# mgaido91/FBK-fairseq-ST

Measured on AMD Instinct MI355X. Metric: audio-frames/sec (train fwd+bwd) s2t_transformer_m, 80-mel, higher is better.
Workload: dtype bf16

## Files before the change

### fbk_fairseq_st_amd/csrc/attention.hip

```cpp
#include "common.hpp"
#include "prof.hpp"
#include <cstdlib>
#include <type_traits>

template <typename T, int DH> struct ACfg {
    static constexpr int E = Elem<T>::PER16;
    static constexpr int ROWB = DH * (int)sizeof(T);
    static constexpr int NCH = ROWB / 16;
    static constexpr int KG = NCH / 4;
    static constexpr int PROWB = 64 * (int)sizeof(T);
    static constexpr int PCH = PROWB / 16;
    static constexpr int PKG = PCH / 4;
    static constexpr int ND = DH / 16;
    static constexpr int TILE = 64 * ROWB;
    static constexpr int TTILE = DH * PROWB;
    static constexpr int PTILE = 16 * PROWB;
};

__device__ __forceinline__ int swz(int row, int c, int nch) { return c ^ (row & ((nch < 8 ? nch : 8) - 1)); }

template <typename T, int DH>
__device__ __forceinline__ void stage_rows(char* lds, const T* g, long stride, int row0, int nvalid) {
    typedef ACfg<T, DH> C;
    for (int cid = threadIdx.x; cid < 64 * C::NCH; cid += 256) {
        const int row = cid / C::NCH, c = cid % C::NCH;
        u32x4 v = {0, 0, 0, 0};
        if (row0 + row < nvalid) v = *reinterpret_cast<const u32x4*>(g + (long)(row0 + row) * stride + c * C::E);
        *reinterpret_cast<u32x4*>(lds + row * C::ROWB + (swz(row, c, C::NCH) << 4)) = v;
    }
}

template <typename T, int DH>
__device__ __forceinline__ void stage_cols(char* lds, const T* g, long stride, int row0, int nvalid) {
    typedef ACfg<T, DH> C;
    if constexpr (sizeof(T) == 2) {
        for (int it = threadIdx.x; it < 32 * C::NCH; it += 256) {
            const int rp = it & 31, dc = it >> 5;
            u32x4 v0 = {0, 0, 0, 0}, v1 = {0, 0, 0, 0};
            const int r0 = row0 + 2 * rp;
            if (r0 < nvalid) v0 = *reinterpret_cast<const u32x4*>(g + (long)r0 * stride + dc * 8);
            if (r0 + 1 < nvalid) v1 = *reinterpret_cast<const u32x4*>(g + (long)(r0 + 1) * stride + dc * 8);
            const uint16_t* a = reinterpret_cast<const uint16_t*>(&v0);
            const uint16_t* b = reinterpret_cast<const uint16_t*>(&v1);
#pragma unroll
            for (int e = 0; e < 8; ++e) {
                const int d = dc * 8 + e;
                const uint32_t w = (uint32_t)a[e] | ((uint32_t)b[e] << 16);
                *reinterpret_cast<uint32_t*>(lds + d * C::PROWB + (swz(d, rp >> 2, C::PCH) << 4) + ((rp & 3) << 2)) = w;
            }
        }
    } else {
        for (int it = threadIdx.x; it < 64 * C::NCH; it += 256) {
            const int r = it & 63, dc = it >> 6;
            u32x4 v = {0, 0, 0, 0};
            if (row0 + r < nvalid) v = *reinterpret_cast<const u32x4*>(g + (long)(row0 + r) * stride + dc * 4);
#pragma unroll
            for (int e = 0; e < 4; ++e) {
                const int d = dc * 4 + e;
                *reinterpret_cast<uint32_t*>(lds + d * C::PROWB + (swz(d, r >> 2, C::PCH) << 4) + ((r & 3) << 2)) = v[e];
            }
        }
    }
}

__device__ __forceinline__ u32x4 frag(const char* lds, int row, int chunk, int rowb, int nch) {
    return *reinterpret_cast<const u32x4*>(lds + row * rowb + (swz(row, chunk, nch) << 4));
}

template <typename T>
__device__ __forceinline__ void put_tile(char* lds, const f32x4 (&acc)[4], int q, int r16) {
    constexpr int PROWB = 64 * (int)sizeof(T), PCH = PROWB / 16;
#pragma unroll
    for (int j = 0; j < 4; ++j)
#pragma unroll
        for (int r = 0; r < 4; ++r) {
            const int row = 4 * q + r, byte = (16 * j + r16) * (int)sizeof(T);
            *reinterpret_cast<T*>(lds + row * PROWB + (swz(row, byte >> 4, PCH) << 4) + (byte & 15)) = from_f32<T>(acc[j][r]);
        }
}

#define S2T_ATTN_V2_MIN_TQ g_s2t_opt_attn_v2_min_tq

struct AttnArgs {
    const void *Q, *K, *V; void* O; float* LSE;
    const void *dO; void *dQ, *dK, *dV; const float* Delta;
    long q_st, q_sb, k_st, k_sb, v_st, v_sb, o_st, o_sb;
    long dq_st, dq_sb, dk_st, dk_sb, dv_st, dv_sb, do_st, do_sb;
    const int* klen;
    int B, H, Tq, Tk, causal;
    int dist_pen;
    float scale, p_drop; unsigned long long seed;
};

__device__ __forceinline__ uint64_t drop_index(const AttnArgs& p, int b, int h, int qrow, int key) {
    return (((uint64_t)b * p.H + h) * p.Tq + qrow) * (uint64_t)((p.Tk + 3) & ~3) + key;
}
__device__ __forceinline__ float drop_scale(const AttnArgs& p, int b, int h, int qrow, int key) {
    if (p.p_drop <= 0.f) return 1.f;
    const uint32_t th = (uint32_t)fminf(p.p_drop * 4294967296.f, 4294967295.f);
    return dropout_keep(p.seed, drop_index(p, b, h, qrow, key), th) ? 1.f / (1.f - p.p_drop) : 0.f;
}

__device__ __forceinline__ uint32_t drop_pair(uint32_t pair, uint32_t fields, uint32_t thm1x2) {
    uint32_t d, k, r;
    asm("v_pk_sub_u16 %0, %1, %2 clamp" : "=v"(d) : "v"(fields), "v"(thm1x2));
    asm("v_pk_min_u16 %0, %1, %2" : "=v"(k) : "v"(d), "v"(0x00010001u));
    asm("v_pk_mul_lo_u16 %0, %1, %2" : "=v"(r) : "v"(pair), "v"(k));
    return r;
}

__device__ __forceinline__ float dist_pen_ln(int qrow, int key) {
    const int d = qrow > key ? qrow - key : key - qrow;
    return d > 1 ? __logf((float)d) : 0.f;
}
__device__ __forceinline__ float dist_pen_log2(int qrow, int key) {
    const int d = qrow > key ? qrow - key : key - qrow;
    return d > 1 ? __builtin_amdgcn_logf((float)d) : 0.f;
}

template <typename T, int DH>
__global__ __launch_bounds__(256) void attn_fwd_kernel(AttnArgs p) {
    typedef ACfg<T, DH> C;
    extern __shared__ __attribute__((aligned(16))) char smem[];
    char* ldsK = smem;
    char* ldsVt = smem + C::TILE;
    const int lane = threadIdx.x & 63, wave = threadIdx.x >> 6, r16 = lane & 15, q = lane >> 4;
    char* ldsP = smem + 2 * C::TILE + wave * C::PTILE;
    const int b = blockIdx.z, h = blockIdx.y, q0 = blockIdx.x * 64 + wave * 16;
    const int klen = p.klen ? min(p.klen[b], p.Tk) : p.Tk;
    const T* Qg = reinterpret_cast<const T*>(p.Q) + (long)b * p.q_sb + (long)h * DH;
    const T* Kg = reinterpret_cast<const T*>(p.K) + (long)b * p.k_sb + (long)h * DH;
    const T* Vg = reinterpret_cast<const T*>(p.V) + (long)b * p.v_sb + (long)h * DH;

    u32x4 qf[C::KG];
#pragma unroll
    for (int g = 0; g < C::KG; ++g) {
        qf[g] = (u32x4){0, 0, 0, 0};
        if (q0 + r16 < p.Tq) qf[g] = *reinterpret_cast<const u32x4*>(Qg + (long)(q0 + r16) * p.q_st + (4 * g + q) * C::E);
    }
    f32x4 o[C::ND];
#pragma unroll
    for (int n = 0; n < C::ND; ++n) o[n] = (f32x4){0.f, 0.f, 0.f, 0.f};
    float m[4] = {-INFINITY, -INFINITY, -INFINITY, -INFINITY}, l[4] = {0.f, 0.f, 0.f, 0.f};

    int kv_end = klen;
    if (p.causal) kv_end = min(kv_end, blockIdx.x * 64 + 64);
    for (int kv0 = 0; kv0 < kv_end; kv0 += 64) {
        __syncthreads();
        stage_rows<T, DH>(ldsK, Kg, p.k_st, kv0, klen);
        stage_cols<T, DH>(ldsVt, Vg, p.v_st, kv0, klen);
        __syncthreads();
        f32x4 s[4];
#pragma unroll
        for (int j = 0; j < 4; ++j) {
            s[j] = (f32x4){0.f, 0.f, 0.f, 0.f};
#pragma unroll
            for (int g = 0; g < C::KG; ++g)
                s[j] = mma16<T>(qf[g], frag(ldsK, 16 * j + r16, 4 * g + q, C::ROWB, C::NCH), s[j]);
        }
        float mx[4] = {-INFINITY, -INFINITY, -INFINITY, -INFINITY};
#pragma unroll
        for (int j = 0; j < 4; ++j) {
            const int key = kv0 + 16 * j + r16;
#pragma unroll
            for (int r = 0; r < 4; ++r) {
                const int qrow = q0 + 4 * q + r;
                const bool ok = key < klen && (!p.causal || key <= qrow);
                s[j][r] = ok ? s[j][r] * p.scale - (p.dist_pen ? dist_pen_ln(qrow, key) : 0.f) : -INFINITY;
                mx[r] = fmaxf(mx[r], s[j][r]);
            }
        }
        float alpha[4], rs[4];
#pragma unroll
        for (int r = 0; r < 4; ++r) {
            float v = mx[r];
            v = fmaxf(v, __shfl_xor(v, 1)); v = fmaxf(v, __shfl_xor(v, 2));
            v = fmaxf(v, __shfl_xor(v, 4)); v = fmaxf(v, __shfl_xor(v, 8));
            const float mn = fmaxf(m[r], v);
            const float mu = (mn == -INFINITY) ? 0.f : mn;
            alpha[r] = __expf(m[r] - mu);
            m[r] = mn;
            mx[r] = mu;
            rs[r] = 0.f;
        }
#pragma unroll
        for (int j = 0; j < 4; ++j)
#pragma unroll
            for (int r = 0; r < 4; ++r) {
                const float pv = __expf(s[j][r] - mx[r]);
                rs[r] += pv;
                s[j][r] = pv * drop_scale(p, b, h, q0 + 4 * q + r, kv0 + 16 * j + r16);
            }
#pragma unroll
        for (int r = 0; r < 4; ++r) {
            float v = rs[r];
            v += __shfl_xor(v, 1); v += __shfl_xor(v, 2); v += __shfl_xor(v, 4); v += __shfl_xor(v, 8);
            l[r] = l[r] * alpha[r] + v;
        }
#pragma unroll
        for (int n = 0; n < C::ND; ++n)
#pragma unroll
            for (int r = 0; r < 4; ++r) o[n][r] *= alpha[r];
        put_tile<T>(ldsP, s, q, r16);
        __builtin_amdgcn_s_waitcnt(0xC07F);
        __builtin_amdgcn_wave_barrier();
#pragma unroll
        for (int g = 0; g < C::PKG; ++g) {
            const u32x4 pa = frag(ldsP, r16, 4 * g + q, C::PROWB, C::PCH);
#pragma unroll
            for (int n = 0; n < C::ND; ++n)
                o[n] = mma16<T>(pa, frag(ldsVt, 16 * n + r16, 4 * g + q, C::PROWB, C::PCH), o[n]);
        }
    }
    T* Og = reinterpret_cast<T*>(p.O) + (long)b * p.o_sb + (long)h * DH;
#pragma unroll
    for (int r = 0; r < 4; ++r) {
        const int qrow = q0 + 4 * q + r;
        if (qrow >= p.Tq) continue;
        const float inv = l[r] > 0.f ? 1.f / l[r] : 0.f;
#pragma unroll
        for (int n = 0; n < C::ND; ++n) Og[(long)qrow * p.o_st + 16 * n + r16] = from_f32<T>(o[n][r] * inv);
        if (r16 == 0 && p.LSE) p.LSE[((long)b * p.H + h) * p.Tq + qrow] = m[r] + logf(l[r]);
    }
}

__device__ __forceinline__ int head_xcd_remap(int& head, int nheads, int ntile) {
    const int L = ((int)blockIdx.z * gridDim.y + blockIdx.y) * gridDim.x + blockIdx.x;
    if (nheads & 7) { head = (int)blockIdx.z * gridDim.y + blockIdx.y; return blockIdx.x; }
    const int slot = L >> 3;
    head = (L & 7) + 8 * (slot / ntile);
    return slot % ntile;
}
typedef short s16x4_t __attribute__((ext_vector_type(4)));
typedef __bf16 bf16x2_t __attribute__((ext_vector_type(2)));
typedef float f32x2_t __attribute__((ext_vector_type(2)));
__device__ __forceinline__ uint32_t pack_bf16(float lo, float hi) {
    return __builtin_bit_cast(uint32_t, __builtin_convertvector((f32x2_t){lo, hi}, bf16x2_t));
}
__device__ __forceinline__ float max_over_rows(float v) {
    uint32_t x = __builtin_bit_cast(uint32_t, v);
    auto r = __builtin_amdgcn_permlane16_swap(x, x, false, false);
    v = fmaxf(__builtin_bit_cast(float, (uint32_t)r[0]), __builtin_bit_cast(float, (uint32_t)r[1]));
    x = __builtin_bit_cast(uint32_t, v);
    r = __builtin_amdgcn_permlane32_swap(x, x, false, false);
    return fmaxf(__builtin_bit_cast(float, (uint32_t)r[0]), __builtin_bit_cast(float, (uint32_t)r[1]));
}
#ifdef S2T_ATTN_STAMPS
__device__ unsigned long long* g_attn_stamps = nullptr;
extern "C" int s2t_dbg_attn_stamps(void* buf) {
    return hipMemcpyToSymbol(HIP_SYMBOL(g_attn_stamps), &buf, sizeof(buf)) == hipSuccess ? 0 : -1;
}
#define ASTAMP_INIT(KID)                                                                                         \
    const int lin_ = ((int)blockIdx.z * gridDim.y + blockIdx.y) * gridDim.x + blockIdx.x;                        \
    const int slot_ = lin_ == 0 ? 0 : (lin_ == 700 ? 1 : (lin_ == 1100 ? 2 : (lin_ == 1500 ? 3 : -1)));                                                    \
    unsigned long long* const stp_ = (g_attn_stamps && slot_ >= 0) ? g_attn_stamps + (((KID) * 4 + slot_) * 4 + (threadIdx.x >> 6)) * 64 : nullptr;
#define ASTAMP(T, K)                                                                                             \
    if (stp_ && (T) < 8) {                                                                                       \
        unsigned long long t_;                                                                                   \
        asm volatile("s_memtime %0\n\ts_waitcnt lgkmcnt(0)" : "=s"(t_) :: "memory");                             \
        if ((threadIdx.x & 63) == 0) stp_[(T) * 8 + (K)] = t_;                                                   \
    }
#define ASTAMP_EARLY(KID)                  \
    ASTAMP_INIT(KID) ASTAMP(7, 0)
#else
#define ASTAMP_INIT(KID)
#define ASTAMP(T, K)
#define ASTAMP_EARLY(KID)
#endif
__global__ __launch_bounds__(256, 3) void attn_fwd2_kernel(AttnArgs p) {
    constexpr int DH = 64;
    ASTAMP_EARLY(0)
    extern __shared__ __attribute__((aligned(16))) char smem[];
    const int lane = threadIdx.x & 63, wave = threadIdx.x >> 6, r16 = lane & 15, q = lane >> 4;
    int head;
    const int bx = head_xcd_remap(head, p.B * p.H, gridDim.x);
    const int b = head / p.H, h = head % p.H, qw = bx * 128 + wave * 32;
    const int klen = p.klen ? min(p.klen[b], p.Tk) : p.Tk;
    const bf16* Qg = reinterpret_cast<const bf16*>(p.Q) + (long)b * p.q_sb + (long)h * DH;
    const bf16* Kg = reinterpret_cast<const bf16*>(p.K) + (long)b * p.k_sb + (long)h * DH;
    const bf16* Vg = reinterpret_cast<const bf16*>(p.V) + (long)b * p.v_sb + (long)h * DH;

    f32x4 o[2][4];
#pragma unroll
    for (int qb = 0; qb < 2; ++qb)
#pragma unroll
        for (int n = 0; n < 4; ++n) o[qb][n] = (f32x4){0.f, 0.f, 0.f, 0.f};
    float m[2] = {-INFINITY, -INFINITY}, l[2] = {0.f, 0.f};

    int kv_end = klen;
    if (p.causal) kv_end = min(kv_end, bx * 128 + 128);
    const int ntile = (kv_end + 63) / 64;

    const uint32_t kst2 = (uint32_t)p.k_st * 2u, vst2 = (uint32_t)p.v_st * 2u;
    auto stage = [&](int kv0, char* st) {
#pragma unroll
        for (int i = 0; i < 2; ++i) {
            const int r8 = 8 * (wave + 4 * i), row = r8 + (lane >> 3), pos = lane & 7;
            const uint32_t r = (uint32_t)min(kv0 + row, p.Tk - 1);
            char* dst = st + __builtin_amdgcn_readfirstlane(r8 * 128);
            const char* ka = reinterpret_cast<const char*>(Kg) + (__umul24(r, kst2) + (uint32_t)((pos ^ (row & 7)) << 4));
            const char* va = reinterpret_cast<const char*>(Vg) + (__umul24(r, vst2) + (uint32_t)((pos ^ (row & 6)) << 4));
            __builtin_amdgcn_global_load_lds((__attribute__((address_space(1))) const void*)ka, (__attribute__((address_space(3))) void*)dst, 16, 0, 0);
            __builtin_amdgcn_global_load_lds((__attribute__((address_space(1))) const void*)va, (__attribute__((address_space(3))) void*)(dst + 8192), 16, 0, 0);
        }
    };
    const uint32_t drop_th16 = (uint32_t)fminf(p.p_drop * 4294967296.f, 4294967295.f) >> 16;
    const uint32_t drop_thm1x2 = (drop_th16 - 1u) * 0x00010001u;
    const bool has_drop = drop_th16 > 0;
    const float drop_inv = 1.f / (1.f - p.p_drop);
    const uint32_t drop_ks = drop_seed_key(p.seed);
    const float sc2 = p.scale * 1.44269504088896f;
    const bool plain = !p.causal && !p.dist_pen && (uint64_t)p.B * p.H * p.Tq * (uint64_t)((p.Tk + 3) & ~3) < (1ull << 34);

    float* sInit = reinterpret_cast<float*>(smem + 32768);
    if (threadIdx.x < 128) {
        const int i = threadIdx.x & 63;
        sInit[threadIdx.x] = (threadIdx.x < 64 || (ntile - 1) * 64 + i < klen) ? 0.f : -INFINITY;
    }
    if (ntile > 0) stage(0, smem);
    char* sQ = smem + 32768 + 512;
#pragma unroll
    for (int i = 0; i < 4; ++i) {
        const int r8 = 8 * (wave + 4 * i), row = r8 + (lane >> 3), pos = lane & 7;
        const long r = min(bx * 128 + row, p.Tq - 1);
        char* dst = sQ + __builtin_amdgcn_readfirstlane(r8 * 128);
        __builtin_amdgcn_global_load_lds((__attribute__((address_space(1))) const void*)(Qg + r * p.q_st + ((pos ^ (row & 7)) << 3)),
                                         (__attribute__((address_space(3))) void*)dst, 16, 0, 0);
    }
    __builtin_amdgcn_s_waitcnt(0x0F70);
    __syncthreads();
    ASTAMP(7, 1)
    for (int t = 0; t < ntile; ++t) {
        const int kv0 = t * 64;
        const char* sK = smem + (t & 1) * 16384;
        const char* sV = sK + 8192;
        ASTAMP(t, 0)
        if (t + 1 < ntile) stage(kv0 + 64, smem + ((t + 1) & 1) * 16384);
        ASTAMP(t, 1)
        f32x4 s[2][4];
        const float* sInit0 = sInit + ((plain && t == ntile - 1) ? 64 : 0) + 4 * q;
        u32x4 qf[2][2];
#pragma unroll
        for (int qb = 0; qb < 2; ++qb)
#pragma unroll
            for (int g = 0; g < 2; ++g) {
                const int row = wave * 32 + 16 * qb + r16;
                qf[qb][g] = *reinterpret_cast<const u32x4*>(sQ + row * 128 + (((4 * g + q) ^ (row & 7)) << 4));
            }
#pragma unroll
        for (int j = 0; j < 4; ++j) {
            u32x4 kf[2];
#pragma unroll
            for (int g = 0; g < 2; ++g) {
                const int row = 16 * j + r16;
                kf[g] = *reinterpret_cast<const u32x4*>(sK + row * 128 + (((4 * g + q) ^ (row & 7)) << 4));
            }
#pragma unroll
            for (int qb = 0; qb < 2; ++qb) {
                s[qb][j] = *reinterpret_cast<const f32x4*>(sInit0 + 16 * j);
#pragma unroll
                for (int g = 0; g < 2; ++g) s[qb][j] = mma16<bf16>(kf[g], qf[qb][g], s[qb][j]);
            }
        }
        u32x4 pf[2][2];
        auto softmax_tile = [&](auto fast_tag, auto drop_tag) {
            constexpr bool FAST = decltype(fast_tag)::value, DROP = decltype(drop_tag)::value;
            const bool pen = !FAST && p.dist_pen;
            const float k2 = pen ? 1.f : sc2;
#pragma unroll
            for (int qb = 0; qb < 2; ++qb) {
                const int qrow = qw + 16 * qb + r16;
                float mx = -INFINITY;
#pragma unroll
                for (int j = 0; j < 4; ++j) {
                    if constexpr (!FAST) {
#pragma unroll
                        for (int r = 0; r < 4; ++r) {
                            float v = s[qb][j][r];
                            const int key = kv0 + 16 * j + 4 * q + r;
                            if (pen) v = v * sc2 - dist_pen_log2(qrow, key);
                            v = (key < klen && (!p.causal || key <= qrow)) ? v : -INFINITY;
                            s[qb][j][r] = v;
                        }
                    }
                    mx = fmaxf(fmaxf(mx, s[qb][j][0]), s[qb][j][1]);
                    mx = fmaxf(fmaxf(mx, s[qb][j][2]), s[qb][j][3]);
                }
                mx = max_over_rows(mx);
                const float mn = fmaxf(m[qb], mx * k2);
                const float mu = (mn == -INFINITY) ? 0.f : mn;
                const float alpha = __builtin_amdgcn_exp2f(m[qb] - mu);
                m[qb] = mn;
                f32x2_t rs2 = {0.f, 0.f};
                const bool drop = FAST ? DROP : has_drop;
                const uint64_t quad0 = drop ? drop_index(p, b, h, qrow, kv0 + 4 * q) >> 2 : 0;
                const uint32_t qlo = (uint32_t)quad0, hwm0 = drop_high_mix(p.seed, quad0);
#pragma unroll
                for (int j = 0; j < 4; ++j) {
                    float pv[4];
#pragma unroll
                    for (int r = 0; r < 4; ++r) pv[r] = __builtin_amdgcn_exp2f(__builtin_fmaf(s[qb][j][r], k2, -mu));
                    rs2 += (f32x2_t){pv[0], pv[1]};
                    rs2 += (f32x2_t){pv[2], pv[3]};
                    uint32_t p01 = pack_bf16(pv[0], pv[1]), p23 = pack_bf16(pv[2], pv[3]);
                    if (drop) {
                        const u32x2 hq = FAST ? drop_hash4_lo(drop_ks, hwm0, qlo + 4u * j) : drop_hash4(p.seed, quad0 + 4 * j);
                        p01 = drop_pair(p01, hq[1], drop_thm1x2); p23 = drop_pair(p23, hq[0], drop_thm1x2);
                    }
                    pf[qb][j >> 1][2 * (j & 1)] = p01;
                    pf[qb][j >> 1][2 * (j & 1) + 1] = p23;
                }
                l[qb] = l[qb] * alpha + (rs2[0] + rs2[1]);
#pragma unroll
                for (int n = 0; n < 4; ++n) o[qb][n] *= alpha;
            }
        };
        if (!plain) softmax_tile(std::false_type{}, std::false_type{});
        else if (has_drop) softmax_tile(std::true_type{}, std::true_type{});
        else softmax_tile(std::true_type{}, std::false_type{});
        ASTAMP(t, 2)
#pragma unroll
        for (int kb = 0; kb < 2; ++kb)
#pragma unroll
            for (int n = 0; n < 4; ++n) {
                u32x4 vf;
#pragma unroll
                for (int hh = 0; hh < 2; ++hh) {
                    const int row = 32 * kb + 16 * hh + 4 * q + (r16 >> 2);
                    const int ch = 2 * n + ((r16 & 3) >> 1);
                    const char* a = sV + row * 128 + ((ch ^ (row & 6)) << 4) + ((r16 & 1) << 3);
                    const s16x4_t v = __builtin_amdgcn_ds_read_tr16_b64_v4i16((__attribute__((address_space(3))) s16x4_t*)a);
                    const u32x2 w = __builtin_bit_cast(u32x2, v);
                    vf[2 * hh] = w[0]; vf[2 * hh + 1] = w[1];
                }
#pragma unroll
                for (int qb = 0; qb < 2; ++qb) o[qb][n] = mma16<bf16>(vf, pf[qb][kb], o[qb][n]);
            }
        ASTAMP(t, 3)
        __builtin_amdgcn_s_waitcnt(0x0F70);
        ASTAMP(t, 4)
        __syncthreads();
        ASTAMP(t, 5)
    }
    ASTAMP(7, 2)
    bf16* Og = reinterpret_cast<bf16*>(p.O) + (long)b * p.o_sb + (long)h * DH;
#pragma unroll
    for (int qb = 0; qb < 2; ++qb) {
        const int qrow = qw + 16 * qb + r16;
        float lt = l[qb];
        lt += __shfl_xor(lt, 16); lt += __shfl_xor(lt, 32);
        if (qrow >= p.Tq) continue;
        const float inv = lt > 0.f ? drop_inv / lt : 0.f;
#pragma unroll
        for (int n = 0; n < 4; ++n) {
            u32x2 w;
            w[0] = pack_bf16(o[qb][n][0] * inv, o[qb][n][1] * inv);
            w[1] = pack_bf16(o[qb][n][2] * inv, o[qb][n][3] * inv);
            *reinterpret_cast<u32x2*>(Og + (long)qrow * p.o_st + 16 * n + 4 * q) = w;
        }
        if (q == 0 && p.LSE) p.LSE[((long)b * p.H + h) * p.Tq + qrow] = m[qb] * 0.693147180559945f + logf(lt);
    }
    ASTAMP(7, 3)
}

template <typename T, int DH>
__global__ __launch_bounds__(256) void attn_delta_kernel(AttnArgs p) {
    const int g = (blockIdx.x * 256 + threadIdx.x) >> 4, li = threadIdx.x & 15;
    const long total = (long)p.B * p.H * p.Tq;
    float s = 0.f;
    if (g < total) {
        const int t = g % p.Tq, h = (g / p.Tq) % p.H, b = g / (p.Tq * p.H);
        const T* o = reinterpret_cast<const T*>(p.O) + (long)t * p.o_st + (long)b * p.o_sb + (long)h * DH;
        const T* d = reinterpret_cast<const T*>(p.dO) + (long)t * p.do_st + (long)b * p.do_sb + (long)h * DH;
        for (int j = li; j < DH; j += 16) s += to_f32(o[j]) * to_f32(d[j]);
    }
    s += __shfl_xor(s, 1); s += __shfl_xor(s, 2); s += __shfl_xor(s, 4); s += __shfl_xor(s, 8);
    if (g < total && li == 0) {
        const int t = g % p.Tq, h = (g / p.Tq) % p.H, b = g / (p.Tq * p.H);
        const_cast<float*>(p.Delta)[((long)b * p.H + h) * p.Tq + t] = s;
    }
}

template <typename T, int DH>
__global__ __launch_bounds__(256) void attn_bwd_dkv_kernel(AttnArgs p) {
    typedef ACfg<T, DH> C;
    extern __shared__ __attribute__((aligned(16))) char smem[];
    char* ldsQ = smem;
    char* ldsDO = smem + C::TILE;
    char* ldsQt = smem + 2 * C::TILE;
    char* ldsDOt = smem + 3 * C::TILE;
    const int lane = threadIdx.x & 63, wave = threadIdx.x >> 6, r16 = lane & 15, q = lane >> 4;
    char* ldsP = smem + 4 * C::TILE + wave * 2 * C::PTILE;
    char* ldsS = ldsP + C::PTILE;
    const int b = blockIdx.z, h = blockIdx.y, k0 = blockIdx.x * 64 + wave * 16;
    const int klen = p.klen ? min(p.klen[b], p.Tk) : p.Tk;
    const T* Qg = reinterpret_cast<const T*>(p.Q) + (long)b * p.q_sb + (long)h * DH;
    const T* Kg = reinterpret_cast<const T*>(p.K) + (long)b * p.k_sb + (long)h * DH;
    const T* Vg = reinterpret_cast<const T*>(p.V) + (long)b * p.v_sb + (long)h * DH;
    const T* dOg = reinterpret_cast<const T*>(p.dO) + (long)b * p.do_sb + (long)h * DH;
    const float* lse = p.LSE + ((long)b * p.H + h) * p.Tq;
    const float* dlt = p.Delta + ((long)b * p.H + h) * p.Tq;

    u32x4 kf[C::KG], vf[C::KG];
#pragma unroll
    for (int g = 0; g < C::KG; ++g) {
        kf[g] = vf[g] = (u32x4){0, 0, 0, 0};
        if (k0 + r16 < klen) {
            kf[g] = *reinterpret_cast<const u32x4*>(Kg + (long)(k0 + r16) * p.k_st + (4 * g + q) * C::E);
            vf[g] = *reinterpret_cast<const u32x4*>(Vg + (long)(k0 + r16) * p.v_st + (4 * g + q) * C::E);
        }
    }
    f32x4 dk[C::ND], dv[C::ND];
#pragma unroll
    for (int n = 0; n < C::ND; ++n) { dk[n] = (f32x4){0.f, 0.f, 0.f, 0.f}; dv[n] = dk[n]; }

    const int qstart = p.causal ? (blockIdx.x * 64) : 0;
    for (int qt = qstart; qt < p.Tq; qt += 64) {
        __syncthreads();
        stage_rows<T, DH>(ldsQ, Qg, p.q_st, qt, p.Tq);
        stage_rows<T, DH>(ldsDO, dOg, p.do_st, qt, p.Tq);
        stage_cols<T, DH>(ldsQt, Qg, p.q_st, qt, p.Tq);
        stage_cols<T, DH>(ldsDOt, dOg, p.do_st, qt, p.Tq);
        __syncthreads();
        f32x4 st[4], dp[4];
#pragma unroll
        for (int j = 0; j < 4; ++j) {
            st[j] = (f32x4){0.f, 0.f, 0.f, 0.f}; dp[j] = st[j];
#pragma unroll
            for (int g = 0; g < C::KG; ++g) {
                st[j] = mma16<T>(kf[g], frag(ldsQ, 16 * j + r16, 4 * g + q, C::ROWB, C::NCH), st[j]);
                dp[j] = mma16<T>(vf[g], frag(ldsDO, 16 * j + r16, 4 * g + q, C::ROWB, C::NCH), dp[j]);
            }
        }
#pragma unroll
        for (int j = 0; j < 4; ++j) {
            const int qrow = qt + 16 * j + r16;
            const bool qok = qrow < p.Tq;
            const float L = qok ? lse[qrow] : 0.f, Dl = qok ? dlt[qrow] : 0.f;
#pragma unroll
            for (int r = 0; r < 4; ++r) {
                const int key = k0 + 4 * q + r;
                const bool ok = qok && key < klen && (!p.causal || key <= qrow);
                const float pv = ok ? __expf(st[j][r] * p.scale - (p.dist_pen ? dist_pen_ln(qrow, key) : 0.f) - L) : 0.f;
                const float ds = ok ? drop_scale(p, b, h, qrow, key) : 0.f;
                st[j][r] = pv * ds;
                dp[j][r] = pv * (ds * dp[j][r] - Dl) * p.scale;
            }
        }
        put_tile<T>(ldsP, st, q, r16);
        put_tile<T>(ldsS, dp, q, r16);
        __builtin_amdgcn_s_waitcnt(0xC07F);
        __builtin_amdgcn_wave_barrier();
#pragma unroll
        for (int g = 0; g < C::PKG; ++g) {
            const u32x4 pa = frag(ldsP, r16, 4 * g + q, C::PROWB, C::PCH);
            const u32x4 sa = frag(ldsS, r16, 4 * g + q, C::PROWB, C::PCH);
#pragma unroll
            for (int n = 0; n < C::ND; ++n) {
                dv[n] = mma16<T>(pa, frag(ldsDOt, 16 * n + r16, 4 * g + q, C::PROWB, C::PCH), dv[n]);
                dk[n] = mma16<T>(sa, frag(ldsQt, 16 * n + r16, 4 * g + q, C::PROWB, C::PCH), dk[n]);
            }
        }
    }
    T* dKg = reinterpret_cast<T*>(p.dK) + (long)b * p.dk_sb + (long)h * DH;
    T* dVg = reinterpret_cast<T*>(p.dV) + (long)b * p.dv_sb + (long)h * DH;
#pragma unroll
    for (int r = 0; r < 4; ++r) {
        const int key = k0 + 4 * q + r;
        if (key >= p.Tk) continue;
#pragma unroll
        for (int n = 0; n < C::ND; ++n) {
            dKg[(long)key * p.dk_st + 16 * n + r16] = from_f32<T>(dk[n][r]);
            dVg[(long)key * p.dv_st + 16 * n + r16] = from_f32<T>(dv[n][r]);
        }
    }
}

template <typename T, int DH>
__global__ __launch_bounds__(256) void attn_bwd_dq_kernel(AttnArgs p) {
    typedef ACfg<T, DH> C;
    extern __shared__ __attribute__((aligned(16))) char smem[];
    char* ldsK = smem;
    char* ldsV = smem + C::TILE;
    char* ldsKt = smem + 2 * C::TILE;
    const int lane = threadIdx.x & 63, wave = threadIdx.x >> 6, r16 = lane & 15, q = lane >> 4;
    char* ldsS = smem + 3 * C::TILE + wave * C::PTILE;
    const int b = blockIdx.z, h = blockIdx.y, q0 = blockIdx.x * 64 + wave * 16;
    const int klen = p.klen ? min(p.klen[b], p.Tk) : p.Tk;
    const T* Qg = reinterpret_cast<const T*>(p.Q) + (long)b * p.q_sb + (long)h * DH;
    const T* Kg = reinterpret_cast<const T*>(p.K) + (long)b * p.k_sb + (long)h * DH;
    const T* Vg = reinterpret_cast<const T*>(p.V) + (long)b * p.v_sb + (long)h * DH;
    const T* dOg = reinterpret_cast<const T*>(p.dO) + (long)b * p.do_sb + (long)h * DH;
    const float* lse = p.LSE + ((long)b * p.H + h) * p.Tq;
    const float* dlt = p.Delta + ((long)b * p.H + h) * p.Tq;

    u32x4 qf[C::KG], dof[C::KG];
#pragma unroll
    for (int g = 0; g < C::KG; ++g) {
        qf[g] = dof[g] = (u32x4){0, 0, 0, 0};
        if (q0 + r16 < p.Tq) {
            qf[g] = *reinterpret_cast<const u32x4*>(Qg + (long)(q0 + r16) * p.q_st + (4 * g + q) * C::E);
            dof[g] = *reinterpret_cast<const u32x4*>(dOg + (long)(q0 + r16) * p.do_st + (4 * g + q) * C::E);
        }
    }
    float L[4], Dl[4];
#pragma unroll
    for (int r = 0; r < 4; ++r) {
        const int qrow = q0 + 4 * q + r;
        L[r] = qrow < p.Tq ? lse[qrow] : 0.f;
        Dl[r] = qrow < p.Tq ? dlt[qrow] : 0.f;
    }
    f32x4 dq[C::ND];
#pragma unroll
    for (int n = 0; n < C::ND; ++n) dq[n] = (f32x4){0.f, 0.f, 0.f, 0.f};

    int kv_end = klen;
    if (p.causal) kv_end = min(kv_end, blockIdx.x * 64 + 64);
    for (int kv0 = 0; kv0 < kv_end; kv0 += 64) {
        __syncthreads();
        stage_rows<T, DH>(ldsK, Kg, p.k_st, kv0, klen);
        stage_rows<T, DH>(ldsV, Vg, p.v_st, kv0, klen);
        stage_cols<T, DH>(ldsKt, Kg, p.k_st, kv0, klen);
        __syncthreads();
        f32x4 s[4], dp[4];
#pragma unroll
        for (int j = 0; j < 4; ++j) {
            s[j] = (f32x4){0.f, 0.f, 0.f, 0.f}; dp[j] = s[j];
#pragma unroll
            for (int g = 0; g < C::KG; ++g) {
                s[j] = mma16<T>(qf[g], frag(ldsK, 16 * j + r16, 4 * g + q, C::ROWB, C::NCH), s[j]);
                dp[j] = mma16<T>(dof[g], frag(ldsV, 16 * j + r16, 4 * g + q, C::ROWB, C::NCH), dp[j]);
            }
        }
#pragma unroll
        for (int j = 0; j < 4; ++j) {
            const int key = kv0 + 16 * j + r16;
#pragma unroll
            for (int r = 0; r < 4; ++r) {
                const int qrow = q0 + 4 * q + r;
                const bool ok = qrow < p.Tq && key < klen && (!p.causal || key <= qrow);
                const float pv = ok ? __expf(s[j][r] * p.scale - (p.dist_pen ? dist_pen_ln(qrow, key) : 0.f) - L[r]) : 0.f;
                const float ds = ok ? drop_scale(p, b, h, qrow, key) : 0.f;
                dp[j][r] = pv * (ds * dp[j][r] - Dl[r]) * p.scale;
            }
        }
        put_tile<T>(ldsS, dp, q, r16);
        __builtin_amdgcn_s_waitcnt(0xC07F);
        __builtin_amdgcn_wave_barrier();
#pragma unroll
        for (int g = 0; g < C::PKG; ++g) {
            const u32x4 sa = frag(ldsS, r16, 4 * g + q, C::PROWB, C::PCH);
#pragma unroll
            for (int n = 0; n < C::ND; ++n)
                dq[n] = mma16<T>(sa, frag(ldsKt, 16 * n + r16, 4 * g + q, C::PROWB, C::PCH), dq[n]);
        }
    }
    T* dQg = reinterpret_cast<T*>(p.dQ) + (long)b * p.dq_sb + (long)h * DH;
#pragma unroll
    for (int r = 0; r < 4; ++r) {
        const int qrow = q0 + 4 * q + r;
        if (qrow >= p.Tq) continue;
#pragma unroll
        for (int n = 0; n < C::ND; ++n) dQg[(long)qrow * p.dq_st + 16 * n + r16] = from_f32<T>(dq[n][r]);
    }
}

__device__ __forceinline__ u32x4 row_frag128(const char* tile, int row, int chunk) {
    return *reinterpret_cast<const u32x4*>(tile + row * 128 + ((chunk ^ (row & 7)) << 4));
}
__device__ __forceinline__ u32x4 tr_frag128(const char* tile, int blk, int n, int r16, int q) {
    u32x4 f;
#pragma unroll
    for (int hh = 0; hh < 2; ++hh) {
        const int row = 32 * blk + 16 * hh + 4 * q + (r16 >> 2);
        const int ch = 2 * n + ((r16 & 3) >> 1);
        const char* a = tile + row * 128 + ((ch ^ (row & 7)) << 4) + ((r16 & 1) << 3);
        const s16x4_t v = __builtin_amdgcn_ds_read_tr16_b64_v4i16((__attribute__((address_space(3))) s16x4_t*)a);
        const u32x2 w = __builtin_bit_cast(u32x2, v);
        f[2 * hh] = w[0]; f[2 * hh + 1] = w[1];
    }
    return f;
}
__device__ __forceinline__ uint32_t quad_bcast(uint32_t v, int r) {
    switch (r) {
        case 0: return (uint32_t)__builtin_amdgcn_mov_dpp((int)v, 0x00, 0xf, 0xf, true);
        case 1: return (uint32_t)__builtin_amdgcn_mov_dpp((int)v, 0x55, 0xf, 0xf, true);
        case 2: return (uint32_t)__builtin_amdgcn_mov_dpp((int)v, 0xAA, 0xf, 0xf, true);
        default: return (uint32_t)__builtin_amdgcn_mov_dpp((int)v, 0xFF, 0xf, 0xf, true);
    }
}
__device__ __forceinline__ void stage2_dma(const bf16* A, long a_st, const bf16* B, long b_st, int r0, int nrows, char* st, int wave, int lane) {
#pragma unroll
    for (int i = 0; i < 2; ++i) {
        const int r8 = 8 * (wave + 4 * i), row = r8 + (lane >> 3), pos = lane & 7;
        const uint32_t r = (uint32_t)min(r0 + row, nrows - 1);
        const uint32_t ch = (uint32_t)((pos ^ (row & 7)) << 4);
        char* dst = st + __builtin_amdgcn_readfirstlane(r8 * 128);
        const char* aa = reinterpret_cast<const char*>(A) + (__umul24(r, (uint32_t)a_st * 2u) + ch);
        const char* ba = reinterpret_cast<const char*>(B) + (__umul24(r, (uint32_t)b_st * 2u) + ch);
        __builtin_amdgcn_global_load_lds((__attribute__((address_space(1))) const void*)aa, (__attribute__((address_space(3))) void*)dst, 16, 0, 0);
        __builtin_amdgcn_global_load_lds((__attribute__((address_space(1))) const void*)ba, (__attribute__((address_space(3))) void*)(dst + 8192), 16, 0, 0);
    }
}
#define S2T_WAIT_VM0() __builtin_amdgcn_s_waitcnt(0x0F70)

__global__ __launch_bounds__(256, 2) void attn_bwd_dkv2_kernel(AttnArgs p) {
    constexpr int DH = 64;
    ASTAMP_EARLY(2)
    extern __shared__ __attribute__((aligned(16))) char smem[];
    const int lane = threadIdx.x & 63, wave = __builtin_amdgcn_readfirstlane(threadIdx.x >> 6), r16 = lane & 15, q = lane >> 4;
    int head;
    const int bx = head_xcd_remap(head, p.B * p.H, gridDim.x);
    const int b = head / p.H, h = head % p.H, kw = bx * 128 + wave * 32;
    const int klen = p.klen ? min(p.klen[b], p.Tk) : p.Tk;
    const bf16* Qg = reinterpret_cast<const bf16*>(p.Q) + (long)b * p.q_sb + (long)h * DH;
    const bf16* Kg = reinterpret_cast<const bf16*>(p.K) + (long)b * p.k_sb + (long)h * DH;
    const bf16* Vg = reinterpret_cast<const bf16*>(p.V) + (long)b * p.v_sb + (long)h * DH;
    const bf16* dOg = reinterpret_cast<const bf16*>(p.dO) + (long)b * p.do_sb + (long)h * DH;
    const float* lse = p.LSE + ((long)b * p.H + h) * p.Tq;
    const float* dlt = p.Delta + ((long)b * p.H + h) * p.Tq;

    char* sKown = smem + 32768 + 1024;
    char* sVown = sKown + 16384;
    f32x4 dkT[2][4], dvT[2][4];
#pragma unroll
    for (int kb = 0; kb < 2; ++kb)
#pragma unroll
        for (int n = 0; n < 4; ++n) { dkT[kb][n] = (f32x4){0.f, 0.f, 0.f, 0.f}; dvT[kb][n] = dkT[kb][n]; }
    const uint32_t drop_th16 = (uint32_t)fminf(p.p_drop * 4294967296.f, 4294967295.f) >> 16;
    const float drop_inv = 1.f / (1.f - p.p_drop);
    const uint32_t drop_ks = drop_seed_key(p.seed), drop_hwm = drop_high_mix(p.seed, 0);
    const uint32_t tkq = (uint32_t)((p.Tk + 3) >> 2);
    const uint32_t drop_thm1x2 = (drop_th16 - 1u) * 0x00010001u;
    const uint32_t own_bit = ((r16 & 1) ? 0x00010000u : 1u) << ((r16 >> 1) & 1);

    const int qstart = p.causal ? bx * 128 : 0;
    const int ntile = qstart < p.Tq ? (p.Tq - qstart + 63) / 64 : 0;
    float* sStat = reinterpret_cast<float*>(smem + 32768);
    auto stage = [&](int qt, int stg) {
        stage2_dma(Qg, p.q_st, dOg, p.do_st, qt, p.Tq, smem + stg * 16384, wave, lane);
        if (wave < 2) {
            float* dst = sStat + stg * 128 + wave * 64;
            if (wave == 1 || qt + lane < p.Tq) {
                const char* sb = reinterpret_cast<const char*>(wave == 0 ? lse : dlt);
                const char* src = sb + (uint32_t)(min(qt + lane, p.Tq - 1) * 4);
                __builtin_amdgcn_global_load_lds((__attribute__((address_space(1))) const void*)src,
                                                 (__attribute__((address_space(3))) void*)dst, 4, 0, 0);
            } else dst[lane] = INFINITY;
        }
    };
    if (ntile > 0) stage(qstart, 0);
    {
        u32x4 kk[4], vv[4];
#pragma unroll
        for (int i = 0; i < 4; ++i) {
            const int cid = threadIdx.x + 256 * i, row = cid >> 3, c = cid & 7;
            const long key = min(bx * 128 + row, p.Tk - 1);
            kk[i] = *reinterpret_cast<const u32x4*>(Kg + key * p.k_st + c * 8);
            vv[i] = *reinterpret_cast<const u32x4*>(Vg + key * p.v_st + c * 8);
        }
#pragma unroll
        for (int i = 0; i < 4; ++i) {
            const int cid = threadIdx.x + 256 * i, row = cid >> 3, c = cid & 7;
            const bool in = bx * 128 + row < klen;
#pragma unroll
            for (int w = 0; w < 4; ++w) { kk[i][w] = in ? kk[i][w] : 0u; vv[i][w] = in ? vv[i][w] : 0u; }
            *reinterpret_cast<u32x4*>(sKown + row * 128 + ((c ^ (row & 7)) << 4)) = kk[i];
            *reinterpret_cast<u32x4*>(sVown + row * 128 + ((c ^ (row & 7)) << 4)) = vv[i];
        }
    }
    S2T_WAIT_VM0();
    __syncthreads();
    const float sc2 = p.scale * 1.44269504088896f;
    const bool generic = p.causal || p.dist_pen;
    ASTAMP(7, 1)
    for (int t = 0; t < ntile; ++t) {
        const int qt = qstart + t * 64;
        const char* sQ = smem + (t & 1) * 16384;
        const char* sDO = sQ + 8192;
        const float* sL = sStat + (t & 1) * 128;
        ASTAMP(t, 0)
        if (t + 1 < ntile) stage(qt + 64, (t + 1) & 1);
        ASTAMP(t, 1)
        auto tile = [&](auto edge_tag, auto drop_tag) {
        constexpr bool EDGE = decltype(edge_tag)::value, DROP = decltype(drop_tag)::value;
#pragma unroll 1
        for (int ib = 0; ib < 2; ++ib) {
        u32x4 pf[2], sf[2];
#pragma unroll
        for (int ii = 0; ii < 2; ++ii) {
            const int i = 2 * ib + ii;
            u32x4 qa[2], da[2];
#pragma unroll
            for (int g = 0; g < 2; ++g) { qa[g] = row_frag128(sQ, 16 * i + r16, 4 * g + q); da[g] = row_frag128(sDO, 16 * i + r16, 4 * g + q); }
            const f32x4 L = *reinterpret_cast<const f32x4*>(sL + 16 * i + 4 * q) * 1.44269504088896f;
            const f32x4 Dl = *reinterpret_cast<const f32x4*>(sL + 64 + 16 * i + 4 * q);
            const uint32_t qrow_quads = DROP ? (uint32_t)(((b * p.H + h) * p.Tq + qt + 16 * i + 4 * q + (r16 & 3))) * tkq : 0u;
#pragma unroll
            for (int kb = 0; kb < 2; ++kb) {
                f32x4 st = {0.f, 0.f, 0.f, 0.f}, dp = {0.f, 0.f, 0.f, 0.f};
#pragma unroll
                for (int g = 0; g < 2; ++g) {
                    const int krow = wave * 32 + 16 * kb + r16;
                    st = mma16<bf16>(qa[g], row_frag128(sKown, krow, 4 * g + q), st);
                    dp = mma16<bf16>(da[g], row_frag128(sVown, krow, 4 * g + q), dp);
                }
                const int key = kw + 16 * kb + r16;
                uint32_t nib = 0u;
                if constexpr (DROP) {
                    const u32x2 hq = drop_hash4_lo(drop_ks, drop_hwm, qrow_quads + ((uint32_t)key >> 2));
                    uint32_t dy, dx, ky, kx;
                    asm("v_pk_sub_u16 %0, %1, %2 clamp" : "=v"(dy) : "v"(hq[1]), "v"(drop_thm1x2));
                    asm("v_pk_sub_u16 %0, %1, %2 clamp" : "=v"(dx) : "v"(hq[0]), "v"(drop_thm1x2));
                    asm("v_pk_min_u16 %0, %1, %2" : "=v"(ky) : "v"(dy), "v"(0x00010001u));
                    asm("v_pk_min_u16 %0, %1, %2" : "=v"(kx) : "v"(dx), "v"(0x00010001u));
                    nib = drop_th16 > 0 ? (ky | (kx << 1)) : 0x00030003u;
                }
                float pv[4], ds[4];
#pragma unroll
                for (int r = 0; r < 4; ++r) {
                    const int qrow = qt + 16 * i + 4 * q + r;
                    float arg = __builtin_fmaf(st[r], sc2, -L[r]);
                    if constexpr (EDGE) { if (p.dist_pen) arg -= dist_pen_log2(qrow, key); }
                    float e = __builtin_amdgcn_exp2f(arg);
                    if constexpr (EDGE) e = (qrow < p.Tq && (!p.causal || key <= qrow)) ? e : 0.f;
                    if constexpr (DROP) {
                        const bool keep = (quad_bcast(nib, r) & own_bit) != 0u;
                        pv[r] = keep ? e : 0.f;
                        ds[r] = e * __builtin_fmaf(keep ? dp[r] : 0.f, drop_inv, -Dl[r]);
                    } else {
                        pv[r] = e;
                        ds[r] = e * (dp[r] - Dl[r]);
                    }
                }
                pf[kb][2 * ii] = pack_bf16(pv[0], pv[1]); pf[kb][2 * ii + 1] = pack_bf16(pv[2], pv[3]);
                sf[kb][2 * ii] = pack_bf16(ds[0], ds[1]); sf[kb][2 * ii + 1] = pack_bf16(ds[2], ds[3]);
            }
        }
#pragma unroll
            for (int n = 0; n < 4; ++n) {
                const u32x4 dot = tr_frag128(sDO, ib, n, r16, q), qtf = tr_frag128(sQ, ib, n, r16, q);
#pragma unroll
                for (int kb = 0; kb < 2; ++kb) {
                    dvT[kb][n] = mma16<bf16>(dot, pf[kb], dvT[kb][n]);
                    dkT[kb][n] = mma16<bf16>(qtf, sf[kb], dkT[kb][n]);
                }
            }
        }
        };
        const bool edge = generic;
        if (p.p_drop > 0.f) { if (edge) tile(std::true_type{}, std::true_type{}); else tile(std::false_type{}, std::true_type{}); }
        else if (edge) tile(std::true_type{}, std::false_type{});
        else tile(std::false_type{}, std::false_type{});
        ASTAMP(t, 3)
        S2T_WAIT_VM0();
        ASTAMP(t, 4)
        __syncthreads();
        ASTAMP(t, 5)
    }
    ASTAMP(7, 2)
    const float dv_scale = p.p_drop > 0.f ? drop_inv : 1.f;
    bf16* dKg = reinterpret_cast<bf16*>(p.dK) + (long)b * p.dk_sb + (long)h * DH;
    bf16* dVg = reinterpret_cast<bf16*>(p.dV) + (long)b * p.dv_sb + (long)h * DH;
#pragma unroll
    for (int kb = 0; kb < 2; ++kb) {
        const int key = kw + 16 * kb + r16;
        if (key >= p.Tk) continue;
        const float kz = key < klen ? 1.f : 0.f;
#pragma unroll
        for (int n = 0; n < 4; ++n) { dkT[kb][n] *= kz * p.scale; dvT[kb][n] *= kz * dv_scale; }
#pragma unroll
        for (int n = 0; n < 4; ++n) {
            u32x2 w;
            w[0] = pack_bf16(dkT[kb][n][0], dkT[kb][n][1]); w[1] = pack_bf16(dkT[kb][n][2], dkT[kb][n][3]);
            *reinterpret_cast<u32x2*>(dKg + (long)key * p.dk_st + 16 * n + 4 * q) = w;
            w[0] = pack_bf16(dvT[kb][n][0], dvT[kb][n][1]); w[1] = pack_bf16(dvT[kb][n][2], dvT[kb][n][3]);
            *reinterpret_cast<u32x2*>(dVg + (long)key * p.dv_st + 16 * n + 4 * q) = w;
        }
    }
    ASTAMP(7, 3)
}

__global__ __launch_bounds__(256, 2) void attn_bwd_dq2_kernel(AttnArgs p) {
    constexpr int DH = 64;
    ASTAMP_EARLY(1)
    extern __shared__ __attribute__((aligned(16))) char smem[];
    const int lane = threadIdx.x & 63, wave = threadIdx.x >> 6, r16 = lane & 15, q = lane >> 4;
    int head;
    const int bx = head_xcd_remap(head, p.B * p.H, gridDim.x);
    const int b = head / p.H, h = head % p.H, qw = bx * 128 + wave * 32;
    const int klen = p.klen ? min(p.klen[b], p.Tk) : p.Tk;
    const bf16* Qg = reinterpret_cast<const bf16*>(p.Q) + (long)b * p.q_sb + (long)h * DH;
    const bf16* Kg = reinterpret_cast<const bf16*>(p.K) + (long)b * p.k_sb + (long)h * DH;
    const bf16* Vg = reinterpret_cast<const bf16*>(p.V) + (long)b * p.v_sb + (long)h * DH;
    const bf16* dOg = reinterpret_cast<const bf16*>(p.dO) + (long)b * p.do_sb + (long)h * DH;
    const float* lse = p.LSE + ((long)b * p.H + h) * p.Tq;
    const float* dlt = p.Delta + ((long)b * p.H + h) * p.Tq;

    int kv_end = klen;
    if (p.causal) kv_end = min(kv_end, bx * 128 + 128);
    const int ntile = (kv_end + 63) / 64;
    if (ntile > 0) stage2_dma(Kg, p.k_st, Vg, p.v_st, 0, p.Tk, smem, wave, lane);
    u32x4 qf[2][2], dof[2][2];
    float L[2], Dl[2];
    const bf16* Og = reinterpret_cast<const bf16*>(p.O) + (long)b * p.o_sb + (long)h * DH;
    u32x4 of[2][2];
#pragma unroll
    for (int qb = 0; qb < 2; ++qb) {
        const long row = min(qw + 16 * qb + r16, p.Tq - 1);
        L[qb] = lse[row] * 1.44269504088896f;
#pragma unroll
        for (int g = 0; g < 2; ++g) {
            qf[qb][g] = *reinterpret_cast<const u32x4*>(Qg + row * p.q_st + (4 * g + q) * 8);
            dof[qb][g] = *reinterpret_cast<const u32x4*>(dOg + row * p.do_st + (4 * g + q) * 8);
            of[qb][g] = *reinterpret_cast<const u32x4*>(Og + row * p.o_st + (4 * g + q) * 8);
        }
    }
#pragma unroll
    for (int qb = 0; qb < 2; ++qb) {
        const int row = qw + 16 * qb + r16;
        const bool in = row < p.Tq;
        float part = 0.f;
#pragma unroll
        for (int g = 0; g < 2; ++g) {
#pragma unroll
            for (int w = 0; w < 4; ++w) { qf[qb][g][w] = in ? qf[qb][g][w] : 0u; dof[qb][g][w] = in ? dof[qb][g][w] : 0u; }
            const bf16* oe = reinterpret_cast<const bf16*>(&of[qb][g]);
            const bf16* de = reinterpret_cast<const bf16*>(&dof[qb][g]);
#pragma unroll
            for (int e = 0; e < 8; ++e) part += (float)oe[e] * (float)de[e];
        }
        L[qb] = in ? L[qb] : 0.f;
        part += __shfl_xor(part, 16); part += __shfl_xor(part, 32);
        Dl[qb] = part;
        if (q == 0 && in) const_cast<float*>(dlt)[row] = part;
    }
    f32x4 dqT[2][4];
#pragma unroll
    for (int qb = 0; qb < 2; ++qb)
#pragma unroll
        for (int n = 0; n < 4; ++n) dqT[qb][n] = (f32x4){0.f, 0.f, 0.f, 0.f};
    const uint32_t drop_th16 = (uint32_t)fminf(p.p_drop * 4294967296.f, 4294967295.f) >> 16;
    const float drop_inv = 1.f / (1.f - p.p_drop);
    const uint32_t drop_ks = drop_seed_key(p.seed), drop_hwm = drop_high_mix(p.seed, 0);
    const uint32_t tkq = (uint32_t)((p.Tk + 3) >> 2);

    const float sc2 = p.scale * 1.44269504088896f;
    const bool generic = p.causal || p.dist_pen;
    S2T_WAIT_VM0();
    __syncthreads();
    ASTAMP(7, 1)
    for (int t = 0; t < ntile; ++t) {
        const int kv0 = t * 64;
        const char* sK = smem + (t & 1) * 16384;
        const char* sV = sK + 8192;
        ASTAMP(t, 0)
        if (t + 1 < ntile) stage2_dma(Kg, p.k_st, Vg, p.v_st, kv0 + 64, p.Tk, smem + ((t + 1) & 1) * 16384, wave, lane);
        ASTAMP(t, 1)
        u32x4 sf[2][2];
        auto ds_tile = [&](auto edge_tag, auto drop_tag, auto tail_tag) {
        constexpr bool EDGE = decltype(edge_tag)::value, DROP = decltype(drop_tag)::value, TAIL = decltype(tail_tag)::value;
        const int tail_thr = klen - kv0 - 4 * q;
#pragma unroll
        for (int j = 0; j < 4; ++j) {
            u32x4 ka[2], va[2];
#pragma unroll
            for (int g = 0; g < 2; ++g) { ka[g] = row_frag128(sK, 16 * j + r16, 4 * g + q); va[g] = row_frag128(sV, 16 * j + r16, 4 * g + q); }
#pragma unroll
            for (int qb = 0; qb < 2; ++qb) {
                f32x4 st = {0.f, 0.f, 0.f, 0.f}, dp = {0.f, 0.f, 0.f, 0.f};
#pragma unroll
                for (int g = 0; g < 2; ++g) { st = mma16<bf16>(ka[g], qf[qb][g], st); dp = mma16<bf16>(va[g], dof[qb][g], dp); }
                const int qrow = qw + 16 * qb + r16;
                const int key0 = kv0 + 16 * j + 4 * q;
                u32x2 hq = {0u, 0u};
                if constexpr (DROP) hq = drop_hash4_lo(drop_ks, drop_hwm, (uint32_t)((b * p.H + h) * p.Tq + qrow) * tkq + ((uint32_t)key0 >> 2));
                float ds[4];
#pragma unroll
                for (int r = 0; r < 4; ++r) {
                    float arg = __builtin_fmaf(st[r], sc2, -L[qb]);
                    if constexpr (EDGE) { if (p.dist_pen) arg -= dist_pen_log2(qrow, key0 + r); }
                    float e = __builtin_amdgcn_exp2f(arg);
                    if constexpr (EDGE) {
                        const int key = key0 + r;
                        e = (key < klen && (!p.causal || key <= qrow)) ? e : 0.f;
                    }
                    if constexpr (TAIL) e = (16 * j + r < tail_thr) ? e : 0.f;
                    if constexpr (DROP) ds[r] = e * __builtin_fmaf(drop_field(hq, r) >= drop_th16 ? dp[r] : 0.f, drop_inv, -Dl[qb]);
                    else ds[r] = e * (dp[r] - Dl[qb]);
                }
                sf[qb][j >> 1][2 * (j & 1)] = pack_bf16(ds[0], ds[1]); sf[qb][j >> 1][2 * (j & 1) + 1] = pack_bf16(ds[2], ds[3]);
            }
        }
        };
        const bool tail = kv0 + 64 > klen;
        if (generic) { if (p.p_drop > 0.f) ds_tile(std::true_type{}, std::true_type{}, std::false_type{}); else ds_tile(std::true_type{}, std::false_type{}, std::false_type{}); }
        else if (p.p_drop > 0.f) { if (tail) ds_tile(std::false_type{}, std::true_type{}, std::true_type{}); else ds_tile(std::false_type{}, std::true_type{}, std::false_type{}); }
        else if (tail) ds_tile(std::false_type{}, std::false_type{}, std::true_type{});
        else ds_tile(std::false_type{}, std::false_type{}, std::false_type{});
        ASTAMP(t, 2)
#pragma unroll
        for (int jb = 0; jb < 2; ++jb)
#pragma unroll
            for (int n = 0; n < 4; ++n) {
                const u32x4 kt = tr_frag128(sK, jb, n, r16, q);
#pragma unroll
                for (int qb = 0; qb < 2; ++qb) dqT[qb][n] = mma16<bf16>(kt, sf[qb][jb], dqT[qb][n]);
            }
        ASTAMP(t, 3)
        S2T_WAIT_VM0();
        ASTAMP(t, 4)
        __syncthreads();
        ASTAMP(t, 5)
    }
    ASTAMP(7, 2)
    bf16* dQg = reinterpret_cast<bf16*>(p.dQ) + (long)b * p.dq_sb + (long)h * DH;
#pragma unroll
    for (int qb = 0; qb < 2; ++qb) {
        const int qrow = qw + 16 * qb + r16;
        if (qrow >= p.Tq) continue;
#pragma unroll
        for (int n = 0; n < 4; ++n) {
            u32x2 w;
            w[0] = pack_bf16(dqT[qb][n][0] * p.scale, dqT[qb][n][1] * p.scale); w[1] = pack_bf16(dqT[qb][n][2] * p.scale, dqT[qb][n][3] * p.scale);
            *reinterpret_cast<u32x2*>(dQg + (long)qrow * p.dq_st + 16 * n + 4 * q) = w;
        }
    }
    ASTAMP(7, 3)
}

__global__ __launch_bounds__(256, 2) void attn_fwd_sq_kernel(AttnArgs p) {
    constexpr int DH = 64;
    extern __shared__ __attribute__((aligned(16))) char smem[];
    const int lane = threadIdx.x & 63, wave = __builtin_amdgcn_readfirstlane(threadIdx.x >> 6), r16 = lane & 15, q = lane >> 4;
    const int head = blockIdx.x, b = head / p.H, h = head % p.H, qw = wave * 16;
    const bool active = qw < p.Tq;
    const int klen = p.klen ? min(p.klen[b], p.Tk) : p.Tk;
    const bf16* Qg = reinterpret_cast<const bf16*>(p.Q) + (long)b * p.q_sb + (long)h * DH;
    const bf16* Kg = reinterpret_cast<const bf16*>(p.K) + (long)b * p.k_sb + (long)h * DH;
    const bf16* Vg = reinterpret_cast<const bf16*>(p.V) + (long)b * p.v_sb + (long)h * DH;

    f32x4 o[4];
#pragma unroll
    for (int n = 0; n < 4; ++n) o[n] = (f32x4){0.f, 0.f, 0.f, 0.f};
    float m = -INFINITY, l = 0.f;
    int kv_end = klen;
    if (p.causal) kv_end = min(kv_end, p.Tq);
    const int ntile = kv_end > 0 ? (kv_end + 63) / 64 : 0;

    const uint32_t kst2 = (uint32_t)p.k_st * 2u, vst2 = (uint32_t)p.v_st * 2u;
    auto stage = [&](int kv0, char* st) {
#pragma unroll
        for (int i = 0; i < 2; ++i) {
            const int r8 = 8 * (wave + 4 * i), row = r8 + (lane >> 3), pos = lane & 7;
            const uint32_t r = (uint32_t)min(kv0 + row, p.Tk - 1);
            char* dst = st + r8 * 128;
            const char* ka = reinterpret_cast<const char*>(Kg) + (__umul24(r, kst2) + (uint32_t)((pos ^ (row & 7)) << 4));
            const char* va = reinterpret_cast<const char*>(Vg) + (__umul24(r, vst2) + (uint32_t)((pos ^ (row & 6)) << 4));
            __builtin_amdgcn_global_load_lds((__attribute__((address_space(1))) const void*)ka, (__attribute__((address_space(3))) void*)dst, 16, 0, 0);
            __builtin_amdgcn_global_load_lds((__attribute__((address_space(1))) const void*)va, (__attribute__((address_space(3))) void*)(dst + 8192), 16, 0, 0);
        }
    };
    const uint32_t drop_th16 = (uint32_t)fminf(p.p_drop * 4294967296.f, 4294967295.f) >> 16;
    const uint32_t drop_thm1x2 = (drop_th16 - 1u) * 0x00010001u;
    const bool has_drop = drop_th16 > 0;
    const float drop_inv = 1.f / (1.f - p.p_drop);
    const uint32_t drop_ks = drop_seed_key(p.seed), drop_hwm = drop_high_mix(p.seed, 0);
    const uint32_t tkq = (uint32_t)((p.Tk + 3) >> 2);
    const float sc2 = p.scale * 1.44269504088896f;

    float* sInit = reinterpret_cast<float*>(smem + 32768);
    if (threadIdx.x < 128) {
        const int i = threadIdx.x & 63;
        sInit[threadIdx.x] = (threadIdx.x < 64 || (ntile - 1) * 64 + i < klen) ? 0.f : -INFINITY;
    }
    if (ntile > 0) stage(0, smem);
    char* sQ = smem + 32768 + 512;
#pragma unroll
    for (int i = 0; i < 2; ++i) {
        const int r8 = 8 * (wave + 4 * i), row = r8 + (lane >> 3), pos = lane & 7;
        const long r = min(row, p.Tq - 1);
        __builtin_amdgcn_global_load_lds((__attribute__((address_space(1))) const void*)(Qg + r * p.q_st + ((pos ^ (row & 7)) << 3)),
                                         (__attribute__((address_space(3))) void*)(sQ + r8 * 128), 16, 0, 0);
    }
    S2T_WAIT_VM0();
    __syncthreads();
    const int qrow = qw + r16;
    const uint32_t qrow_quads = (uint32_t)((b * p.H + h) * p.Tq + qrow) * tkq;
    for (int t = 0; t < ntile; ++t) {
        const int kv0 = t * 64;
        const char* sK = smem + (t & 1) * 16384;
        const char* sV = sK + 8192;
        if (t + 1 < ntile) stage(kv0 + 64, smem + ((t + 1) & 1) * 16384);
        if (active) {
            f32x4 s[4];
            const float* sInit0 = sInit + ((!p.causal && t == ntile - 1) ? 64 : 0) + 4 * q;
            u32x4 qf[2];
#pragma unroll
            for (int g = 0; g < 2; ++g) qf[g] = row_frag128(sQ, qw + r16, 4 * g + q);
#pragma unroll
            for (int j = 0; j < 4; ++j) {
                s[j] = *reinterpret_cast<const f32x4*>(sInit0 + 16 * j);
#pragma unroll
                for (int g = 0; g < 2; ++g) s[j] = mma16<bf16>(row_frag128(sK, 16 * j + r16, 4 * g + q), qf[g], s[j]);
            }
            u32x4 pf[2];
            auto softmax_tile = [&](auto mask_tag, auto drop_tag) {
                constexpr bool MASK = decltype(mask_tag)::value, DROP = decltype(drop_tag)::value;
                float mx = -INFINITY;
#pragma unroll
                for (int j = 0; j < 4; ++j) {
                    if constexpr (MASK) {
#pragma unroll
                        for (int r = 0; r < 4; ++r) {
                            const int key = kv0 + 16 * j + 4 * q + r;
                            s[j][r] = (key < klen && key <= qrow) ? s[j][r] : -INFINITY;
                        }
                    }
                    mx = fmaxf(fmaxf(mx, s[j][0]), s[j][1]);
                    mx = fmaxf(fmaxf(mx, s[j][2]), s[j][3]);
                }
                mx = max_over_rows(mx);
                const float mn = fmaxf(m, mx * sc2);
                const float mu = (mn == -INFINITY) ? 0.f : mn;
                const float alpha = __builtin_amdgcn_exp2f(m - mu);
                m = mn;
                f32x2_t rs2 = {0.f, 0.f};
                const uint32_t qlo = qrow_quads + (uint32_t)((kv0 + 4 * q) >> 2);
#pragma unroll
                for (int j = 0; j < 4; ++j) {
                    float pv[4];
#pragma unroll
                    for (int r = 0; r < 4; ++r) pv[r] = __builtin_amdgcn_exp2f(__builtin_fmaf(s[j][r], sc2, -mu));
                    rs2 += (f32x2_t){pv[0], pv[1]};
                    rs2 += (f32x2_t){pv[2], pv[3]};
                    uint32_t p01 = pack_bf16(pv[0], pv[1]), p23 = pack_bf16(pv[2], pv[3]);
                    if constexpr (DROP) {
                        const u32x2 hq = drop_hash4_lo(drop_ks, drop_hwm, qlo + 4u * j);
                        p01 = drop_pair(p01, hq[1], drop_thm1x2); p23 = drop_pair(p23, hq[0], drop_thm1x2);
                    }
                    pf[j >> 1][2 * (j & 1)] = p01;
                    pf[j >> 1][2 * (j & 1) + 1] = p23;
                }
                l = l * alpha + (rs2[0] + rs2[1]);
#pragma unroll
                for (int n = 0; n < 4; ++n) o[n] *= alpha;
            };
            if (p.causal) { if (has_drop) softmax_tile(std::true_type{}, std::true_type{}); else softmax_tile(std::true_type{}, std::false_type{}); }
            else if (has_drop) softmax_tile(std::false_type{}, std::true_type{});
            else softmax_tile(std::false_type{}, std::false_type{});
#pragma unroll
            for (int kb = 0; kb < 2; ++kb)
#pragma unroll
                for (int n = 0; n < 4; ++n) {
                    u32x4 vf;
#pragma unroll
                    for (int hh = 0; hh < 2; ++hh) {
                        const int row = 32 * kb + 16 * hh + 4 * q + (r16 >> 2);
                        const int ch = 2 * n + ((r16 & 3) >> 1);
                        const char* a = sV + row * 128 + ((ch ^ (row & 6)) << 4) + ((r16 & 1) << 3);
                        const s16x4_t v = __builtin_amdgcn_ds_read_tr16_b64_v4i16((__attribute__((address_space(3))) s16x4_t*)a);
                        const u32x2 w = __builtin_bit_cast(u32x2, v);
                        vf[2 * hh] = w[0]; vf[2 * hh + 1] = w[1];
                    }
                    o[n] = mma16<bf16>(vf, pf[kb], o[n]);
                }
        }
        S2T_WAIT_VM0();
        __syncthreads();
    }
    float lt = l;
    lt += __shfl_xor(lt, 16); lt += __shfl_xor(lt, 32);
    if (qrow >= p.Tq) return;
    bf16* Og = reinterpret_cast<bf16*>(p.O) + (long)b * p.o_sb + (long)h * DH;
    const float inv = lt > 0.f ? drop_inv / lt : 0.f;
#pragma unroll
    for (int n = 0; n < 4; ++n) {
        u32x2 w;
        w[0] = pack_bf16(o[n][0] * inv, o[n][1] * inv);
        w[1] = pack_bf16(o[n][2] * inv, o[n][3] * inv);
        *reinterpret_cast<u32x2*>(Og + (long)qrow * p.o_st + 16 * n + 4 * q) = w;
    }
    if (q == 0 && p.LSE) p.LSE[((long)b * p.H + h) * p.Tq + qrow] = m * 0.693147180559945f + logf(lt);
}

#define S2T_SQ_TPITCH 136
#define S2T_SQ_BWD_LDS (16384 + 512 + 32768 + 4 * 16 * S2T_SQ_TPITCH)
__global__ __launch_bounds__(256, 2) void attn_bwd_sq_kernel(AttnArgs p) {
    constexpr int DH = 64;
    extern __shared__ __attribute__((aligned(16))) char smem[];
    const int lane = threadIdx.x & 63, wave = __builtin_amdgcn_readfirstlane(threadIdx.x >> 6), r16 = lane & 15, q = lane >> 4;
    const int head = blockIdx.x, b = head / p.H, h = head % p.H;
    const int klen = p.klen ? min(p.klen[b], p.Tk) : p.Tk;
    const bf16* Qg = reinterpret_cast<const bf16*>(p.Q) + (long)b * p.q_sb + (long)h * DH;
    const bf16* Kg = reinterpret_cast<const bf16*>(p.K) + (long)b * p.k_sb + (long)h * DH;
    const bf16* Vg = reinterpret_cast<const bf16*>(p.V) + (long)b * p.v_sb + (long)h * DH;
    const bf16* dOg = reinterpret_cast<const bf16*>(p.dO) + (long)b * p.do_sb + (long)h * DH;
    const bf16* Og = reinterpret_cast<const bf16*>(p.O) + (long)b * p.o_sb + (long)h * DH;
    bf16* dKg = reinterpret_cast<bf16*>(p.dK) + (long)b * p.dk_sb + (long)h * DH;
    bf16* dVg = reinterpret_cast<bf16*>(p.dV) + (long)b * p.dv_sb + (long)h * DH;
    const float* lse = p.LSE + ((long)b * p.H + h) * p.Tq;
    float* dlt = const_cast<float*>(p.Delta) + ((long)b * p.H + h) * p.Tq;
    const char* sQ = smem;
    const char* sDO = smem + 8192;
    float* sStat = reinterpret_cast<float*>(smem + 16384);
    char* sKV = smem + 16384 + 512;
    char* sT = sKV + 32768 + wave * (16 * S2T_SQ_TPITCH);

    int kv_end = klen;
    if (p.causal) kv_end = min(kv_end, p.Tq);
    const int ntile = kv_end > 0 ? (kv_end + 63) / 64 : 0;
    const int nq = (p.Tq + 15) >> 4;
    if (ntile > 0) stage2_dma(Kg, p.k_st, Vg, p.v_st, 0, p.Tk, sKV, wave, lane);
    stage2_dma(Qg, p.q_st, dOg, p.do_st, 0, p.Tq, smem, wave, lane);
    {
        const int row = threadIdx.x >> 2, seg = threadIdx.x & 3;
        const long rc = min(row, p.Tq - 1);
        u32x4 of[2], df[2];
#pragma unroll
        for (int g = 0; g < 2; ++g) {
            of[g] = *reinterpret_cast<const u32x4*>(Og + rc * p.o_st + 16 * seg + 8 * g);
            df[g] = *reinterpret_cast<const u32x4*>(dOg + rc * p.do_st + 16 * seg + 8 * g);
        }
        const float L = lse[rc];
        float part = 0.f;
#pragma unroll
        for (int g = 0; g < 2; ++g) {
            const bf16* oe = reinterpret_cast<const bf16*>(&of[g]);
            const bf16* de = reinterpret_cast<const bf16*>(&df[g]);
#pragma unroll
            for (int e = 0; e < 8; ++e) part += (float)oe[e] * (float)de[e];
        }
        part += __shfl_xor(part, 1); part += __shfl_xor(part, 2);
        if (seg == 0) {
            const bool in = row < p.Tq;
            sStat[row] = in ? L * 1.44269504088896f : INFINITY;
            sStat[64 + row] = in ? part : 0.f;
            if (in) dlt[row] = part;
        }
    }
    f32x4 dq[4][4];
#pragma unroll
    for (int i = 0; i < 4; ++i)
#pragma unroll
        for (int n = 0; n < 4; ++n) dq[i][n] = (f32x4){0.f, 0.f, 0.f, 0.f};
    const uint32_t drop_th16 = (uint32_t)fminf(p.p_drop * 4294967296.f, 4294967295.f) >> 16;
    const float drop_inv = 1.f / (1.f - p.p_drop);
    const uint32_t drop_ks = drop_seed_key(p.seed), drop_hwm = drop_high_mix(p.seed, 0);
    const uint32_t tkq = (uint32_t)((p.Tk + 3) >> 2);
    const uint32_t drop_thm1x2 = (drop_th16 - 1u) * 0x00010001u;
    const uint32_t own_bit = ((r16 & 1) ? 0x00010000u : 1u) << ((r16 >> 1) & 1);
    const float sc2 = p.scale * 1.44269504088896f;
    const float dv_scale = p.p_drop > 0.f ? drop_inv : 1.f;
    S2T_WAIT_VM0();
    __syncthreads();
    for (int t = 0; t < ntile; ++t) {
        const int kv0 = t * 64;
        const char* sK = sKV + (t & 1) * 16384;
        const char* sV = sK + 8192;
        if (t + 1 < ntile) stage2_dma(Kg, p.k_st, Vg, p.v_st, kv0 + 64, p.Tk, sKV + ((t + 1) & 1) * 16384, wave, lane);
        const int key = kv0 + 16 * wave + r16;
        f32x4 dkT[4], dvT[4];
#pragma unroll
        for (int n = 0; n < 4; ++n) { dkT[n] = (f32x4){0.f, 0.f, 0.f, 0.f}; dvT[n] = dkT[n]; }
        auto tile = [&](auto mask_tag, auto drop_tag) {
            constexpr bool MASK = decltype(mask_tag)::value, DROP = decltype(drop_tag)::value;
            u32x4 kfr[2], vfr[2];
#pragma unroll
            for (int g = 0; g < 2; ++g) { kfr[g] = row_frag128(sK, 16 * wave + r16, 4 * g + q); vfr[g] = row_frag128(sV, 16 * wave + r16, 4 * g + q); }
#pragma unroll
            for (int ib = 0; ib < 2; ++ib) {
                if (2 * ib >= nq) break;
                u32x4 pf = {0u, 0u, 0u, 0u}, sf = {0u, 0u, 0u, 0u};
#pragma unroll
                for (int ii = 0; ii < 2; ++ii) {
                    const int i = 2 * ib + ii;
                    if (i >= nq) break;
                    u32x4 qa[2], da[2];
#pragma unroll
                    for (int g = 0; g < 2; ++g) { qa[g] = row_frag128(sQ, 16 * i + r16, 4 * g + q); da[g] = row_frag128(sDO, 16 * i + r16, 4 * g + q); }
                    const f32x4 L = *reinterpret_cast<const f32x4*>(sStat + 16 * i + 4 * q);
                    const f32x4 Dl = *reinterpret_cast<const f32x4*>(sStat + 64 + 16 * i + 4 * q);
                    f32x4 st = {0.f, 0.f, 0.f, 0.f}, dp = {0.f, 0.f, 0.f, 0.f};
#pragma unroll
                    for (int g = 0; g < 2; ++g) { st = mma16<bf16>(qa[g], kfr[g], st); dp = mma16<bf16>(da[g], vfr[g], dp); }
                    uint32_t nib = 0u;
                    if constexpr (DROP) {
                        const uint32_t qrow_quads = (uint32_t)((b * p.H + h) * p.Tq + 16 * i + 4 * q + (r16 & 3)) * tkq;
                        const u32x2 hq = drop_hash4_lo(drop_ks, drop_hwm, qrow_quads + ((uint32_t)key >> 2));
                        uint32_t dy, dx, ky, kx;
                        asm("v_pk_sub_u16 %0, %1, %2 clamp" : "=v"(dy) : "v"(hq[1]), "v"(drop_thm1x2));
                        asm("v_pk_sub_u16 %0, %1, %2 clamp" : "=v"(dx) : "v"(hq[0]), "v"(drop_thm1x2));
                        asm("v_pk_min_u16 %0, %1, %2" : "=v"(ky) : "v"(dy), "v"(0x00010001u));
                        asm("v_pk_min_u16 %0, %1, %2" : "=v"(kx) : "v"(dx), "v"(0x00010001u));
                        nib = drop_th16 > 0 ? (ky | (kx << 1)) : 0x00030003u;
                    }
                    float pv[4], ds[4];
#pragma unroll
                    for (int r = 0; r < 4; ++r) {
                        float e = __builtin_amdgcn_exp2f(__builtin_fmaf(st[r], sc2, -L[r]));
                        if constexpr (MASK) e = (key < klen && (!p.causal || key <= 16 * i + 4 * q + r)) ? e : 0.f;
                        if constexpr (DROP) {
                            const bool keep = (quad_bcast(nib, r) & own_bit) != 0u;
                            pv[r] = keep ? e : 0.f;
                            ds[r] = e * __builtin_fmaf(keep ? dp[r] : 0.f, drop_inv, -Dl[r]);
                        } else {
                            pv[r] = e;
                            ds[r] = e * (dp[r] - Dl[r]);
                        }
                    }
                    pf[2 * ii] = pack_bf16(pv[0], pv[1]); pf[2 * ii + 1] = pack_bf16(pv[2], pv[3]);
                    sf[2 * ii] = pack_bf16(ds[0], ds[1]); sf[2 * ii + 1] = pack_bf16(ds[2], ds[3]);
                    *reinterpret_cast<u32x2*>(sT + r16 * S2T_SQ_TPITCH + (16 * i + 4 * q) * 2) = (u32x2){sf[2 * ii], sf[2 * ii + 1]};
                }
#pragma unroll
                for (int n = 0; n < 4; ++n) {
                    const u32x4 dot = tr_frag128(sDO, ib, n, r16, q), qtf = tr_frag128(sQ, ib, n, r16, q);
                    dvT[n] = mma16<bf16>(dot, pf, dvT[n]);
                    dkT[n] = mma16<bf16>(qtf, sf, dkT[n]);
                }
            }
            asm volatile("s_waitcnt lgkmcnt(0)" ::: "memory");
            __builtin_amdgcn_wave_barrier();
            s16x4_t kt[4];
#pragma unroll
            for (int n = 0; n < 4; ++n) {
                const int row = 16 * wave + 4 * q + (r16 >> 2), ch = 2 * n + ((r16 & 3) >> 1);
                kt[n] = __builtin_amdgcn_ds_read_tr16_b64_v4i16((__attribute__((address_space(3))) s16x4_t*)(sK + row * 128 + ((ch ^ (row & 7)) << 4) + ((r16 & 1) << 3)));
            }
#pragma unroll
            for (int i = 0; i < 4; ++i) {
                if (i >= nq) break;
                const s16x4_t a = __builtin_amdgcn_ds_read_tr16_b64_v4i16(
                    (__attribute__((address_space(3))) s16x4_t*)(sT + (4 * q + (r16 >> 2)) * S2T_SQ_TPITCH + (16 * i + 4 * (r16 & 3)) * 2));
#pragma unroll
                for (int n = 0; n < 4; ++n) dq[i][n] = __builtin_amdgcn_mfma_f32_16x16x16bf16_1k(a, kt[n], dq[i][n], 0, 0, 0);
            }
            asm volatile("" ::: "memory");
        };
        if (kv0 + 16 * wave < kv_end) {
            const bool mask = p.causal || kv0 + 64 > klen;
            if (p.p_drop > 0.f) { if (mask) tile(std::true_type{}, std::true_type{}); else tile(std::false_type{}, std::true_type{}); }
            else if (mask) tile(std::true_type{}, std::false_type{});
            else tile(std::false_type{}, std::false_type{});
        }
        S2T_WAIT_VM0();
        __syncthreads();
        if (key < p.Tk) {
#pragma unroll
            for (int n = 0; n < 4; ++n) {
                dkT[n] *= p.scale; dvT[n] *= dv_scale;
                u32x2 w;
                w[0] = pack_bf16(dkT[n][0], dkT[n][1]); w[1] = pack_bf16(dkT[n][2], dkT[n][3]);
                *reinterpret_cast<u32x2*>(dKg + (long)key * p.dk_st + 16 * n + 4 * q) = w;
                w[0] = pack_bf16(dvT[n][0], dvT[n][1]); w[1] = pack_bf16(dvT[n][2], dvT[n][3]);
                *reinterpret_cast<u32x2*>(dVg + (long)key * p.dv_st + 16 * n + 4 * q) = w;
            }
        }
    }
    for (int key = ntile * 64 + (threadIdx.x >> 3); key < p.Tk; key += 32) {
        const int c = (threadIdx.x & 7) * 8;
        *reinterpret_cast<u32x2*>(dKg + (long)key * p.dk_st + c) = (u32x2){0u, 0u};
        *reinterpret_cast<u32x2*>(dKg + (long)key * p.dk_st + c + 4) = (u32x2){0u, 0u};
        *reinterpret_cast<u32x2*>(dVg + (long)key * p.dv_st + c) = (u32x2){0u, 0u};
        *reinterpret_cast<u32x2*>(dVg + (long)key * p.dv_st + c + 4) = (u32x2){0u, 0u};
    }
    float* red = reinterpret_cast<float*>(sKV);
    bf16* dQg = reinterpret_cast<bf16*>(p.dQ) + (long)b * p.dq_sb + (long)h * DH;
#pragma unroll
    for (int half = 0; half < 2; ++half) {
        if (half) __syncthreads();
#pragma unroll
        for (int i = 0; i < 4; ++i) {
            if (i >= nq) break;
#pragma unroll
            for (int nn = 0; nn < 2; ++nn)
#pragma unroll
                for (int r = 0; r < 4; ++r) red[(wave * 64 + 16 * i + 4 * q + r) * 32 + 16 * nn + r16] = dq[i][2 * half + nn][r];
        }
        __syncthreads();
        const int row = threadIdx.x >> 2, c = (threadIdx.x & 3) * 8;
        if (row < p.Tq) {
            f32x4 s0 = {0.f, 0.f, 0.f, 0.f}, s1 = s0;
#pragma unroll
            for (int w = 0; w < 4; ++w) {
                s0 += *reinterpret_cast<const f32x4*>(red + (w * 64 + row) * 32 + c);
                s1 += *reinterpret_cast<const f32x4*>(red + (w * 64 + row) * 32 + c + 4);
            }
            s0 *= p.scale; s1 *= p.scale;
            *reinterpret_cast<u32x2*>(dQg + (long)row * p.dq_st + 32 * half + c) = (u32x2){pack_bf16(s0[0], s0[1]), pack_bf16(s0[2], s0[3])};
            *reinterpret_cast<u32x2*>(dQg + (long)row * p.dq_st + 32 * half + c + 4) = (u32x2){pack_bf16(s1[0], s1[1]), pack_bf16(s1[2], s1[3])};
        }
    }
}

static bool span32(long stride, int rows) {
    return stride >= 0 && stride * 2 < (1l << 24) && (long)rows * stride * 2 + 256 < (1l << 32);
}
static bool strides_ok(int dtype, const long* s, int n) {
    const int e = dtype == S2T_BF16 ? 8 : 4;
    for (int i = 0; i < n; ++i) if (s[i] % e) return false;
    return true;
}

static bool sq_shape(const AttnArgs& a) {
    if (g_s2t_opt_attn_v1 != 0 || a.dist_pen || a.Tq > 64) return false;
    if (!((a.Tq >= S2T_ATTN_V2_MIN_TQ && a.Tk >= 128) || (a.causal && a.Tq == a.Tk))) return false;
    const bool idx32 = (unsigned long long)a.B * a.H * a.Tq * (unsigned long long)((a.Tk + 3) & ~3) < (1ull << 34);
    return idx32 && span32(a.k_st, a.Tk) && span32(a.v_st, a.Tk);
}
static bool sq_fwd_route(const AttnArgs& a) {
    return sq_shape(a) && !(a.o_st % 4) && !(a.o_sb % 4) && !((uintptr_t)a.O & 7);
}
static bool sq_bwd_route(const AttnArgs& a) {
    const bool al = !(a.dk_st % 4) && !(a.dk_sb % 4) && !(a.dv_st % 4) && !(a.dv_sb % 4) && !(a.dq_st % 4) && !(a.dq_sb % 4) &&
                    !((uintptr_t)a.dK & 7) && !((uintptr_t)a.dV & 7) && !((uintptr_t)a.dQ & 7);
    return sq_shape(a) && al && span32(a.q_st, a.Tq) && span32(a.do_st, a.Tq) && !(a.o_st % 8) && !(a.o_sb % 8) && !((uintptr_t)a.O & 15);
}

template <typename T, int DH> static int fwd_launch(const AttnArgs& a, hipStream_t st) {
    typedef ACfg<T, DH> C;
    dim3 grid((a.Tq + 63) / 64, a.H, a.B);
    const size_t lds = 2 * C::TILE + 4 * C::PTILE;
    hipLaunchKernelGGL((attn_fwd_kernel<T, DH>), grid, dim3(256), lds, st, a);
    S2T_LAUNCH_CHECK();
    return S2T_OK;
}
template <typename T, int DH> static int bwd_launch(const AttnArgs& a, hipStream_t st) {
    typedef ACfg<T, DH> C;
    const long rows = (long)a.B * a.H * a.Tq;
    bool dkv2 = false, dq2 = false;
    if constexpr (sizeof(T) == 2 && DH == 64) {
        if (sq_bwd_route(a)) {
            hipLaunchKernelGGL(attn_bwd_sq_kernel, dim3((unsigned)(a.B * a.H)), dim3(256), S2T_SQ_BWD_LDS, st, a);
            S2T_LAUNCH_CHECK();
            return S2T_OK;
        }
        const bool v1 = g_s2t_opt_attn_v1 != 0;
        const bool al = !(a.dk_st % 4) && !(a.dk_sb % 4) && !(a.dv_st % 4) && !(a.dv_sb % 4) && !(a.dq_st % 4) && !(a.dq_sb % 4) &&
                        !((uintptr_t)a.dK & 7) && !((uintptr_t)a.dV & 7) && !((uintptr_t)a.dQ & 7);
        const bool idx32 = (unsigned long long)a.B * a.H * a.Tq * (unsigned long long)((a.Tk + 3) & ~3) < (1ull << 34);
        dkv2 = !v1 && al && idx32 && a.Tk >= 128 && span32(a.q_st, a.Tq) && span32(a.do_st, a.Tq);
        dq2 = !v1 && al && idx32 && span32(a.k_st, a.Tk) && span32(a.v_st, a.Tk) && (a.Tq >= 128 || (a.Tq >= S2T_ATTN_V2_MIN_TQ && a.Tk >= 128)) && !(a.o_st % 8) && !(a.o_sb % 8) && !((uintptr_t)a.O & 15);
        if (dq2) {
            hipLaunchKernelGGL(attn_bwd_dq2_kernel, dim3((a.Tq + 127) / 128, a.H, a.B), dim3(256), 32768, st, a);
            S2T_LAUNCH_CHECK();
        } else {
            hipLaunchKernelGGL((attn_delta_kernel<T, DH>), dim3((unsigned)((rows * 16 + 255) / 256)), dim3(256), 0, st, a);
            S2T_LAUNCH_CHECK();
        }
        if (dkv2) {
            {
                static bool attr = false;
                if (!attr) { (void)hipFuncSetAttribute(reinterpret_cast<const void*>(&attn_bwd_dkv2_kernel), hipFuncAttributeMaxDynamicSharedMemorySize, 32768 + 1024 + 32768); attr = true; }
            }
            hipLaunchKernelGGL(attn_bwd_dkv2_kernel, dim3((a.Tk + 127) / 128, a.H, a.B), dim3(256), 32768 + 1024 + 32768, st, a);
            S2T_LAUNCH_CHECK();
        }
    } else {
        hipLaunchKernelGGL((attn_delta_kernel<T, DH>), dim3((unsigned)((rows * 16 + 255) / 256)), dim3(256), 0, st, a);
        S2T_LAUNCH_CHECK();
    }
    if (!dkv2) {
        static bool attr = false;
        const size_t lds = 4 * C::TILE + 8 * C::PTILE;
        if (!attr && lds > 65536) {
            (void)hipFuncSetAttribute(reinterpret_cast<const void*>(&attn_bwd_dkv_kernel<T, DH>), hipFuncAttributeMaxDynamicSharedMemorySize, (int)lds);
            attr = true;
        }
        hipLaunchKernelGGL((attn_bwd_dkv_kernel<T, DH>), dim3((a.Tk + 63) / 64, a.H, a.B), dim3(256), lds, st, a);
        S2T_LAUNCH_CHECK();
    }
    if (!dq2) {
        static bool attr = false;
        const size_t lds = 3 * C::TILE + 4 * C::PTILE;
        if (!attr && lds > 65536) {
            (void)hipFuncSetAttribute(reinterpret_cast<const void*>(&attn_bwd_dq_kernel<T, DH>), hipFuncAttributeMaxDynamicSharedMemorySize, (int)lds);
            attr = true;
        }
        hipLaunchKernelGGL((attn_bwd_dq_kernel<T, DH>), dim3((a.Tq + 63) / 64, a.H, a.B), dim3(256), lds, st, a);
        S2T_LAUNCH_CHECK();
    }
    return S2T_OK;
}

static int check_common(int dtype, int head_dim, const AttnArgs& a) {
    if (dtype != S2T_F32 && dtype != S2T_BF16) return S2T_ENOTSUP;
    if (head_dim != 64 && head_dim != 32) return S2T_ENOTSUP;
    if (a.B <= 0 || a.H <= 0 || a.Tq <= 0 || a.Tk <= 0) return S2T_EINVAL;
    if (a.p_drop < 0.f || a.p_drop >= 1.f || (a.dist_pen != 0 && a.dist_pen != 1)) return S2T_EINVAL;
    return S2T_OK;
}

extern "C" int s2t_attn_fwd(int dtype, int head_dim, int B, int H, int Tq, int Tk,
                            const void* Q, long q_st, long q_sb, const void* K, long k_st, long k_sb,
                            const void* V, long v_st, long v_sb, void* O, long o_st, long o_sb, float* LSE,
                            const int* klen, int causal, int dist_penalty, float scale, float p_drop, unsigned long long seed,
                            void* stream) {
    AttnArgs a{};
    a.dist_pen = dist_penalty;
    a.Q = Q; a.K = K; a.V = V; a.O = O; a.LSE = LSE;
    a.q_st = q_st; a.q_sb = q_sb; a.k_st = k_st; a.k_sb = k_sb; a.v_st = v_st; a.v_sb = v_sb; a.o_st = o_st; a.o_sb = o_sb;
    a.klen = klen; a.B = B; a.H = H; a.Tq = Tq; a.Tk = Tk; a.causal = causal; a.scale = scale; a.p_drop = p_drop; a.seed = seed;
    if (B == 0 || Tq == 0) return S2T_OK;
    int rc = check_common(dtype, head_dim, a);
    if (rc) return rc;
    if (!Q || !K || !V || !O) return S2T_EINVAL;
    const long s[] = {q_st, q_sb, k_st, k_sb, v_st, v_sb};
    if (!strides_ok(dtype, s, 6)) return S2T_EINVAL;
    hipStream_t st = (hipStream_t)stream;
    ProfScope prof("attn_fwd", st, 4.0 * B * H * (double)Tq * Tk * head_dim * (causal ? 0.5 : 1.0), 0.0);
    if (dtype == S2T_BF16 && head_dim == 64 && sq_fwd_route(a)) {
        hipLaunchKernelGGL(attn_fwd_sq_kernel, dim3((unsigned)(B * H)), dim3(256), 32768 + 512 + 8192, st, a);
        S2T_LAUNCH_CHECK();
        return S2T_OK;
    }
    if (dtype == S2T_BF16 && head_dim == 64 && (Tq >= 128 || (Tq >= S2T_ATTN_V2_MIN_TQ && Tk >= 128)) && (o_st % 4) == 0 && (o_sb % 4) == 0 && ((uintptr_t)O & 7) == 0) {
        const bool v1 = g_s2t_opt_attn_v1 != 0 || !span32(k_st, Tk) || !span32(v_st, Tk);
        if (!v1) {
            hipLaunchKernelGGL(attn_fwd2_kernel, dim3((Tq + 127) / 128, H, B), dim3(256), 32768 + 512 + 16384, st, a);
            S2T_LAUNCH_CHECK();
            return S2T_OK;
        }
    }
    if (dtype == S2T_BF16) return head_dim == 64 ? fwd_launch<bf16, 64>(a, st) : fwd_launch<bf16, 32>(a, st);
    return head_dim == 64 ? fwd_launch<float, 64>(a, st) : fwd_launch<float, 32>(a, st);
}

extern "C" int s2t_attn_bwd(int dtype, int head_dim, int B, int H, int Tq, int Tk,
                            const void* Q, long q_st, long q_sb, const void* K, long k_st, long k_sb,
                            const void* V, long v_st, long v_sb, const void* O, long o_st, long o_sb,
                            const void* dO, long do_st, long do_sb, const float* LSE, float* Delta,
                            void* dQ, long dq_st, long dq_sb, void* dK, long dk_st, long dk_sb,
                            void* dV, long dv_st, long dv_sb,
                            const int* klen, int causal, int dist_penalty, float scale, float p_drop, unsigned long long seed,
                            void* stream) {
    AttnArgs a{};
    a.dist_pen = dist_penalty;
    a.Q = Q; a.K = K; a.V = V; a.O = const_cast<void*>(O); a.LSE = const_cast<float*>(LSE);
    a.dO = dO; a.dQ = dQ; a.dK = dK; a.dV = dV; a.Delta = Delta;
    a.q_st = q_st; a.q_sb = q_sb; a.k_st = k_st; a.k_sb = k_sb; a.v_st = v_st; a.v_sb = v_sb; a.o_st = o_st; a.o_sb = o_sb;
    a.dq_st = dq_st; a.dq_sb = dq_sb; a.dk_st = dk_st; a.dk_sb = dk_sb; a.dv_st = dv_st; a.dv_sb = dv_sb; a.do_st = do_st; a.do_sb = do_sb;
    a.klen = klen; a.B = B; a.H = H; a.Tq = Tq; a.Tk = Tk; a.causal = causal; a.scale = scale; a.p_drop = p_drop; a.seed = seed;
    if (B == 0 || Tq == 0) return S2T_OK;
    int rc = check_common(dtype, head_dim, a);
    if (rc) return rc;
    if (!Q || !K || !V || !O || !dO || !LSE || !Delta || !dQ || !dK || !dV) return S2T_EINVAL;
    const long s[] = {q_st, q_sb, k_st, k_sb, v_st, v_sb, do_st, do_sb};
    if (!strides_ok(dtype, s, 8)) return S2T_EINVAL;
    hipStream_t st = (hipStream_t)stream;
    const bool sq = dtype == S2T_BF16 && head_dim == 64 && sq_bwd_route(a);
    ProfScope prof("attn_bwd", st, (sq ? 10.0 : 14.0) * B * H * (double)Tq * Tk * head_dim * (causal ? 0.5 : 1.0), 0.0);
    if (dtype == S2T_BF16) return head_dim == 64 ? bwd_launch<bf16, 64>(a, st) : bwd_launch<bf16, 32>(a, st);
    return head_dim == 64 ? bwd_launch<float, 64>(a, st) : bwd_launch<float, 32>(a, st);
}

template <typename T>
__global__ __launch_bounds__(256) void attn_probs_avg_kernel(const T* __restrict__ Q, long q_st, long q_sb, const T* __restrict__ Kp, long k_st,
                                                             long k_sb, const int* __restrict__ klen, float* __restrict__ out, int H, int dh,
                                                             int Tq, int Tk, int heads_used, float scale) {
    __shared__ float sh[16];
    __shared__ float qs[128];
    const int tq = blockIdx.x, b = blockIdx.y;
    const int kl = klen ? min(klen[b], Tk) : Tk;
    constexpr int NK = 8;
    float acc[NK];
#pragma unroll
    for (int i = 0; i < NK; ++i) acc[i] = 0.f;
    for (int h = 0; h < heads_used; ++h) {
        __syncthreads();
        if ((int)threadIdx.x < dh) qs[threadIdx.x] = to_f32(Q[tq * q_st + b * q_sb + h * dh + threadIdx.x]) * scale;
        __syncthreads();
        float s[NK];
        float m = -INFINITY;
#pragma unroll
        for (int i = 0; i < NK; ++i) {
            const int tk = threadIdx.x + 256 * i;
            s[i] = -INFINITY;
            if (tk < kl) {
                const T* kr = Kp + (long)tk * k_st + b * k_sb + h * dh;
                float d = 0.f;
                for (int j = 0; j < dh; ++j) d += qs[j] * to_f32(kr[j]);
                s[i] = d;
            }
            m = fmaxf(m, s[i]);
        }
        m = block_max(m, sh);
        float l = 0.f;
#pragma unroll
        for (int i = 0; i < NK; ++i) { s[i] = (s[i] == -INFINITY) ? 0.f : expf(s[i] - m); l += s[i]; }
        l = block_sum(l, sh);
        const float inv = l > 0.f ? 1.f / (l * heads_used) : 0.f;
#pragma unroll
        for (int i = 0; i < NK; ++i) acc[i] += s[i] * inv;
    }
#pragma unroll
    for (int i = 0; i < NK; ++i) {
        const int tk = threadIdx.x + 256 * i;
        if (tk < Tk) out[((long)b * Tq + tq) * Tk + tk] = acc[i];
    }
}

extern "C" int s2t_attn_probs_avg(int dtype, int head_dim, int B, int H, int Tq, int Tk, const void* Q, long q_st, long q_sb,
                                  const void* K, long k_st, long k_sb, const int* klen, int heads_used, float scale, float* out,
                                  void* stream) {
    if (B == 0 || Tq == 0 || Tk == 0) return S2T_OK;
    if (!Q || !K || !out || head_dim <= 0 || head_dim > 128 || H <= 0 || heads_used <= 0 || heads_used > H) return S2T_EINVAL;
    if (Tk > 2048) return S2T_ENOTSUP;
    hipStream_t st = (hipStream_t)stream;
    dim3 grid((unsigned)Tq, (unsigned)B);
    if (dtype == S2T_BF16) hipLaunchKernelGGL(attn_probs_avg_kernel<bf16>, grid, dim3(256), 0, st, (const bf16*)Q, q_st, q_sb, (const bf16*)K, k_st, k_sb,
                                               klen, out, H, head_dim, Tq, Tk, heads_used, scale);
    else if (dtype == S2T_F32) hipLaunchKernelGGL(attn_probs_avg_kernel<float>, grid, dim3(256), 0, st, (const float*)Q, q_st, q_sb, (const float*)K, k_st,
                                                  k_sb, klen, out, H, head_dim, Tq, Tk, heads_used, scale);
    else return S2T_ENOTSUP;
    S2T_LAUNCH_CHECK();
    return S2T_OK;
}
```

### fbk_fairseq_st_amd/csrc/layer.hip

```cpp
#include "common.hpp"
#include "../../include/s2t_hip.h"

namespace {
constexpr size_t AL = 256;
inline size_t up(size_t n) { return (n + AL - 1) / AL * AL; }

struct Ws {
    size_t h1, st1, qkv, ctx, lse, y1;
    size_t h2, st2, q, kv, ctx2, lse2, y2;
    size_t h3, st3, a, pre, amask;
    size_t total, nmask;
};
Ws layout(const S2TLayerDesc& L, int training) {
    Ws w{};
    const size_t M = (size_t)L.T * L.B, D = L.D, e = 2, Ms = (size_t)L.Ts * L.B;
    size_t o = 0;
    auto take = [&](size_t bytes) { const size_t at = o; o += up(bytes); return at; };
    w.h1 = take(M * D * e); w.st1 = take(2 * M * 4); w.qkv = take(M * 3 * D * e); w.ctx = take(M * D * e);
    w.lse = take((size_t)L.B * L.heads * L.T * 4); w.y1 = take(M * D * e);
    if (L.decoder) {
        w.h2 = take(M * D * e); w.st2 = take(2 * M * 4); w.q = take(M * D * e); w.kv = take(Ms * 2 * D * e); w.ctx2 = take(M * D * e);
        w.lse2 = take((size_t)L.B * L.heads * L.T * 4); w.y2 = take(M * D * e);
    }
    w.h3 = take(M * D * e); w.st3 = take(2 * M * 4); w.a = take(M * (size_t)L.ffn * e);
    if (L.gelu) w.pre = take(M * (size_t)L.ffn * e);
    w.nmask = (training && !L.gelu) ? s2t_gemm_relu_mask_bytes((int)M, L.ffn, L.D) : 0;
    if (w.nmask) w.amask = take(w.nmask);
    w.total = o;
    return w;
}
struct Tmp { size_t d3, da, dh3, dx2, dx2d, d2, dctx2, dq, dkv, dh2, dx1, dx1d, d1, dctx, dqkv, dh1, delta, total; };
Tmp tmp_layout(const S2TLayerDesc& L) {
    Tmp t{};
    const size_t M = (size_t)L.T * L.B, D = L.D, e = 2, Ms = (size_t)L.Ts * L.B;
    size_t o = 0;
    auto take = [&](size_t bytes) { const size_t at = o; o += up(bytes); return at; };
    t.d3 = take(M * D * e); t.da = take(M * (size_t)L.ffn * e); t.dh3 = take(M * D * e); t.dx2 = take(M * D * e); t.dx2d = take(M * D * e);
    if (L.decoder) {
        t.d2 = take(M * D * e); t.dctx2 = take(M * D * e); t.dq = take(M * D * e); t.dkv = take(Ms * 2 * D * e); t.dh2 = take(M * D * e);
        t.dx1 = take(M * D * e); t.dx1d = take(M * D * e);
    }
    t.d1 = take(M * D * e); t.dctx = take(M * D * e); t.dqkv = take(M * 3 * D * e); t.dh1 = take(M * D * e);
    t.delta = take((size_t)L.B * L.heads * L.T * 4);
    t.total = o;
    return t;
}

#define TRY(call) do { const int rc_ = (call); if (rc_ != S2T_OK) return rc_; } while (0)

int linear(const S2TLayerDesc& L, int M, int N, int K, const void* x, const void* w, const float* b, void* y, const void* residual,
           const void* aux, void* aux_out, int ldaux, int act, float p_drop, unsigned long long seed, void* st) {
    return s2t_gemm_gather(L.dtype, L.dtype, 0, 0, M, N, K, x, K, w, K, y, N, b, residual, residual ? N : 0, aux, aux_out, ldaux, act, 0, 1, 1.f,
                           nullptr, 0, nullptr, nullptr, p_drop, seed, st);
}
int linear_dx(const S2TLayerDesc& L, int M, int n_out, int n_in, const void* dy, const void* w, void* dx, const void* aux, int ldaux, int act,
              float alpha, int accumulate, void* st) {
    return s2t_gemm_gather(L.dtype, L.dtype, 0, 1, M, n_in, n_out, dy, n_out, w, n_in, dx, n_in, nullptr, nullptr, 0, aux, nullptr, ldaux, act,
                           accumulate, 1, alpha, nullptr, 0, nullptr, nullptr, 0.f, 0ull, st);
}
int queue_dw(S2TLayerCall& c, const void* dy, const void* x, float* dw, float* db, int n_out, int n_in, int tokens) {
    if (c.n_items >= c.max_items || !c.items) return S2T_EINVAL;
    S2TWgradProblem& p = c.items[c.n_items++];
    p.dY = dy; p.X = x; p.dW = dw; p.db = db; p.n_out = n_out; p.n_in = n_in; p.tokens = tokens; p.ldy = n_out; p.ldx = n_in; p.ldw = n_in;
    return S2T_OK;
}
bool bad(const S2TLayerDesc* L) {
    return !L || L->dtype != S2T_BF16 || L->T <= 0 || L->B <= 0 || L->D <= 0 || L->heads <= 0 || L->D % L->heads || L->ffn <= 0 ||
           (L->decoder && L->Ts <= 0) || (L->D & 7) || (L->ffn & 7);
}
}

extern "C" size_t s2t_layer_ws_bytes(const S2TLayerDesc* L, int training) { return bad(L) ? 0 : layout(*L, training).total; }
extern "C" size_t s2t_layer_bwd_tmp_bytes(const S2TLayerDesc* L) { return bad(L) ? 0 : tmp_layout(*L).total; }

extern "C" int s2t_layer_fwd(const S2TLayerDesc* Lp, S2TLayerCall* c, void* st) {
    if (bad(Lp) || !c || !c->x || !c->y || !c->ws || (Lp->decoder && !c->enc)) return S2T_EINVAL;
    const S2TLayerDesc& L = *Lp;
    const Ws w = layout(L, c->training);
    char* ws = static_cast<char*>(c->ws);
    const int M = L.T * L.B, D = L.D, Ff = L.ffn, H = L.heads, d = D / H;
    const float scale = (float)pow((double)d, -0.5);
    const float pa = c->training ? L.p_attn : 0.f, p = c->training ? L.p_drop : 0.f, pact = c->training ? L.p_act : 0.f;
    float* st1 = reinterpret_cast<float*>(ws + w.st1);
    TRY(s2t_layernorm_fwd(L.dtype, c->x, L.ln1_g, L.ln1_b, ws + w.h1, st1, st1 + M, M, D, L.ln_eps, st));
    TRY(linear(L, M, 3 * D, D, ws + w.h1, L.w_qkv, L.b_qkv, ws + w.qkv, nullptr, nullptr, nullptr, 0, S2T_ACT_NONE, 0.f, 0, st));
    const char* qkv = ws + w.qkv;
    const long ts3 = (long)L.B * 3 * D, bs3 = 3 * D, ts1 = (long)L.B * D, bs1 = D;
    TRY(s2t_attn_fwd(L.dtype, d, L.B, H, L.T, L.T, qkv, ts3, bs3, qkv + (size_t)D * 2, ts3, bs3, qkv + (size_t)2 * D * 2, ts3, bs3, ws + w.ctx, ts1, bs1,
                     reinterpret_cast<float*>(ws + w.lse), c->self_klen, L.causal, L.dist_penalty, scale, pa, c->seed_sa_attn, st));
    TRY(linear(L, M, D, D, ws + w.ctx, L.w_o, L.b_o, ws + w.y1, c->x, nullptr, nullptr, 0, S2T_ACT_NONE, p, c->seed_sa_out, st));
    const char* xin = ws + w.y1;
    if (L.decoder) {
        const int Ms = L.Ts * L.B;
        float* st2 = reinterpret_cast<float*>(ws + w.st2);
        TRY(s2t_layernorm_fwd(L.dtype, xin, L.lnx_g, L.lnx_b, ws + w.h2, st2, st2 + M, M, D, L.ln_eps, st));
        TRY(linear(L, M, D, D, ws + w.h2, L.w_xq, L.b_xq, ws + w.q, nullptr, nullptr, nullptr, 0, S2T_ACT_NONE, 0.f, 0, st));
        TRY(linear(L, Ms, 2 * D, D, c->enc, L.w_xkv, L.b_xkv, ws + w.kv, nullptr, nullptr, nullptr, 0, S2T_ACT_NONE, 0.f, 0, st));
        const char* kv = ws + w.kv;
        const long ts2 = (long)L.B * 2 * D, bs2 = 2 * D;
        TRY(s2t_attn_fwd(L.dtype, d, L.B, H, L.T, L.Ts, ws + w.q, ts1, bs1, kv, ts2, bs2, kv + (size_t)D * 2, ts2, bs2, ws + w.ctx2, ts1, bs1,
                         reinterpret_cast<float*>(ws + w.lse2), c->enc_klen, 0, 0, scale, pa, c->seed_xa_attn, st));
        TRY(linear(L, M, D, D, ws + w.ctx2, L.w_xo, L.b_xo, ws + w.y2, xin, nullptr, nullptr, 0, S2T_ACT_NONE, p, c->seed_xa_out, st));
        xin = ws + w.y2;
    }
    float* st3 = reinterpret_cast<float*>(ws + w.st3);
    TRY(s2t_layernorm_fwd(L.dtype, xin, L.ln2_g, L.ln2_b, ws + w.h3, st3, st3 + M, M, D, L.ln_eps, st));
    if (L.gelu) {
        TRY(linear(L, M, Ff, D, ws + w.h3, L.w_fc1, L.b_fc1, ws + w.a, nullptr, nullptr, ws + w.pre, Ff, S2T_ACT_GELU, pact, c->seed_ffn_act, st));
    } else if (w.nmask) {
        TRY(linear(L, M, Ff, D, ws + w.h3, L.w_fc1, L.b_fc1, ws + w.a, nullptr, nullptr, ws + w.amask, 0, S2T_ACT_RELU_MASK, pact, c->seed_ffn_act, st));
    } else {
        TRY(linear(L, M, Ff, D, ws + w.h3, L.w_fc1, L.b_fc1, ws + w.a, nullptr, nullptr, nullptr, 0, S2T_ACT_RELU, pact, c->seed_ffn_act, st));
    }
    TRY(linear(L, M, D, Ff, ws + w.a, L.w_fc2, L.b_fc2, c->y, xin, nullptr, nullptr, 0, S2T_ACT_NONE, p, c->seed_ffn_out, st));
    return S2T_OK;
}

extern "C" int s2t_layer_bwd(const S2TLayerDesc* Lp, S2TLayerCall* c, void* st) {
    if (bad(Lp) || !c || !c->x || !c->ws || !c->dy || !c->dx || !c->tmp || (Lp->decoder && (!c->enc || !c->denc))) return S2T_EINVAL;
    if (c->nxt_p > 0.f && !c->dx_drop) return S2T_EINVAL;
    const S2TLayerDesc& L = *Lp;
    const Ws w = layout(L, c->training);
    const Tmp t = tmp_layout(L);
    const char* ws = static_cast<const char*>(c->ws);
    char* tm = static_cast<char*>(c->tmp);
    const int M = L.T * L.B, D = L.D, Ff = L.ffn, H = L.heads, d = D / H;
    const float scale = (float)pow((double)d, -0.5);
    const float pa = c->training ? L.p_attn : 0.f, p = c->training ? L.p_drop : 0.f, pact = c->training ? L.p_act : 0.f;
    const size_t nMD = (size_t)M * D;
    const long ts3 = (long)L.B * 3 * D, bs3 = 3 * D, ts1 = (long)L.B * D, bs1 = D;
    const char* x3 = L.decoder ? ws + w.y2 : ws + w.y1;
    const void* d3 = c->dy_drop;
    if (!d3) {
        if (p > 0.f) { TRY(s2t_dropout(L.dtype, c->dy, tm + t.d3, nMD, p, c->seed_ffn_out, st)); d3 = tm + t.d3; }
        else d3 = c->dy;
    }
    TRY(queue_dw(*c, d3, ws + w.a, L.g_w_fc2, L.g_b_fc2, D, Ff, M));
    if (!L.gelu) {
        const float alpha = 1.f / (1.f - pact);
        if (w.nmask) TRY(linear_dx(L, M, D, Ff, d3, L.w_fc2, tm + t.da, ws + w.amask, 0, S2T_ACT_RELU_BWD_MASK, alpha, 0, st));
        else TRY(linear_dx(L, M, D, Ff, d3, L.w_fc2, tm + t.da, ws + w.a, Ff, S2T_ACT_RELU_BWD, alpha, 0, st));
    } else {
        TRY(linear_dx(L, M, D, Ff, d3, L.w_fc2, tm + t.da, ws + w.pre, Ff, S2T_ACT_GELU_BWD, 1.f, 0, st));
        if (pact > 0.f) TRY(s2t_dropout(L.dtype, tm + t.da, tm + t.da, (size_t)M * Ff, pact, c->seed_ffn_act, st));
    }
    TRY(queue_dw(*c, tm + t.da, ws + w.h3, L.g_w_fc1, L.g_b_fc1, Ff, D, M));
    TRY(linear_dx(L, M, Ff, D, tm + t.da, L.w_fc1, tm + t.dh3, nullptr, 0, S2T_ACT_NONE, 1.f, 0, st));
    const float* st3 = reinterpret_cast<const float*>(ws + w.st3);
    const unsigned long long seed_up = L.decoder ? c->seed_xa_out : c->seed_sa_out;
    TRY(s2t_layernorm_bwd(L.dtype, tm + t.dh3, x3, st3, st3 + M, L.ln2_g, c->dy, tm + t.dx2, L.g_ln2_g, L.g_ln2_b, M, D,
                          p > 0.f ? tm + t.dx2d : nullptr, p, seed_up, st));
    const char* dcur = tm + t.dx2;
    const char* dcur_d = p > 0.f ? tm + t.dx2d : tm + t.dx2;
    if (L.decoder) {
        const int Ms = L.Ts * L.B;
        TRY(queue_dw(*c, dcur_d, ws + w.ctx2, L.g_w_xo, L.g_b_xo, D, D, M));
        TRY(linear_dx(L, M, D, D, dcur_d, L.w_xo, tm + t.dctx2, nullptr, 0, S2T_ACT_NONE, 1.f, 0, st));
        const char* kv = ws + w.kv;
        char* dkv = tm + t.dkv;
        const long ts2 = (long)L.B * 2 * D, bs2 = 2 * D;
        TRY(s2t_attn_bwd(L.dtype, d, L.B, H, L.T, L.Ts, ws + w.q, ts1, bs1, kv, ts2, bs2, kv + (size_t)D * 2, ts2, bs2, ws + w.ctx2, ts1, bs1,
                         tm + t.dctx2, ts1, bs1, reinterpret_cast<const float*>(ws + w.lse2), reinterpret_cast<float*>(tm + t.delta),
                         tm + t.dq, ts1, bs1, dkv, ts2, bs2, dkv + (size_t)D * 2, ts2, bs2, c->enc_klen, 0, 0, scale, pa, c->seed_xa_attn, st));
        TRY(queue_dw(*c, dkv, c->enc, L.g_w_xkv, L.g_b_xkv, 2 * D, D, Ms));
        TRY(linear_dx(L, Ms, 2 * D, D, dkv, L.w_xkv, c->denc, nullptr, 0, S2T_ACT_NONE, 1.f, c->denc_accumulate, st));
        TRY(queue_dw(*c, tm + t.dq, ws + w.h2, L.g_w_xq, L.g_b_xq, D, D, M));
        TRY(linear_dx(L, M, D, D, tm + t.dq, L.w_xq, tm + t.dh2, nullptr, 0, S2T_ACT_NONE, 1.f, 0, st));
        const float* st2 = reinterpret_cast<const float*>(ws + w.st2);
        TRY(s2t_layernorm_bwd(L.dtype, tm + t.dh2, ws + w.y1, st2, st2 + M, L.lnx_g, dcur, tm + t.dx1, L.g_lnx_g, L.g_lnx_b, M, D,
                              p > 0.f ? tm + t.dx1d : nullptr, p, c->seed_sa_out, st));
        dcur = tm + t.dx1;
        dcur_d = p > 0.f ? tm + t.dx1d : tm + t.dx1;
    }
    TRY(queue_dw(*c, dcur_d, ws + w.ctx, L.g_w_o, L.g_b_o, D, D, M));
    TRY(linear_dx(L, M, D, D, dcur_d, L.w_o, tm + t.dctx, nullptr, 0, S2T_ACT_NONE, 1.f, 0, st));
    const char* qkv = ws + w.qkv;
    char* dqkv = tm + t.dqkv;
    TRY(s2t_attn_bwd(L.dtype, d, L.B, H, L.T, L.T, qkv, ts3, bs3, qkv + (size_t)D * 2, ts3, bs3, qkv + (size_t)2 * D * 2, ts3, bs3, ws + w.ctx, ts1, bs1,
                     tm + t.dctx, ts1, bs1, reinterpret_cast<const float*>(ws + w.lse), reinterpret_cast<float*>(tm + t.delta),
                     dqkv, ts3, bs3, dqkv + (size_t)D * 2, ts3, bs3, dqkv + (size_t)2 * D * 2, ts3, bs3, c->self_klen, L.causal, L.dist_penalty, scale, pa,
                     c->seed_sa_attn, st));
    TRY(queue_dw(*c, dqkv, ws + w.h1, L.g_w_qkv, L.g_b_qkv, 3 * D, D, M));
    TRY(linear_dx(L, M, 3 * D, D, dqkv, L.w_qkv, tm + t.dh1, nullptr, 0, S2T_ACT_NONE, 1.f, 0, st));
    const float* st1 = reinterpret_cast<const float*>(ws + w.st1);
    TRY(s2t_layernorm_bwd(L.dtype, tm + t.dh1, c->x, st1, st1 + M, L.ln1_g, dcur, c->dx, L.g_ln1_g, L.g_ln1_b, M, D,
                          c->nxt_p > 0.f ? c->dx_drop : nullptr, c->nxt_p, c->nxt_seed, st));
    return S2T_OK;
}
```

### fbk_fairseq_st_amd/kernels.py

```python
import ctypes

import torch

from . import lib as L
from .lib import ACT_NONE, ACT_RELU, ACT_GELU, ACT_RELU_BWD, ACT_GELU_BWD, ACT_RELU_MASK, ACT_RELU_BWD_MASK


def _lib():
    return L.load()


_GEMM = None
_DT = {torch.float32: L.F32, torch.bfloat16: L.BF16}
_RAW_STREAM = torch._C._cuda_getCurrentRawStream


def gemm(a, b, trans_a=False, trans_b=False, bias=None, residual=None, act=ACT_NONE, aux=None, aux_out=None,
         out=None, out_dtype=None, accumulate=False, splitk=1, alpha=1.0, M=None, N=None, K=None,
         map_a=None, period_a=0, map_b=None, map_c=None, out_rows=None, p_drop=0.0, seed=0):
    global _GEMM
    if _GEMM is None:
        _GEMM = _lib().s2t_gemm_gather
    if not (a.is_cuda and b.is_cuda):
        raise L.S2THipError("S2T kernels need device tensors: the hot path has no CPU fallback")
    sa0, sb0 = a.stride(0), b.stride(0)
    assert a.stride(1) == 1 and b.stride(1) == 1
    if M is None:
        M = a.shape[1] if trans_a else a.shape[0]
    if K is None:
        K = a.shape[0] if trans_a else a.shape[1]
    if N is None:
        N = b.shape[1] if trans_b else b.shape[0]
    if out is None:
        odt = out_dtype or a.dtype
        rows = out_rows if out_rows is not None else M
        out = (torch.zeros if (accumulate or splitk > 1 or map_c is not None) else torch.empty)(
            (rows, N), dtype=odt, device=a.device)
    ldaux = 0
    if act >= ACT_RELU_MASK:
        t = aux_out if act == ACT_RELU_MASK else aux
        assert t is not None and t.is_cuda and t.dtype == torch.uint8 and t.numel() == relu_mask_bytes(M, N, K) > 0
    elif residual is not None or aux is not None or aux_out is not None:
        for t in (residual, aux, aux_out):
            assert t is None or (t.dtype == out.dtype and t.stride(-1) == 1 and t.is_cuda)
        ldaux = aux.stride(0) if aux is not None else (aux_out.stride(0) if aux_out is not None else 0)
    rc = _GEMM(
        _DT[a.dtype], _DT[out.dtype], int(trans_a), int(trans_b), M, N, K, a.data_ptr(), sa0, b.data_ptr(), sb0,
        out.data_ptr(), out.stride(0), bias.data_ptr() if bias is not None else 0,
        residual.data_ptr() if residual is not None else 0, residual.stride(0) if residual is not None else 0,
        aux.data_ptr() if aux is not None else 0, aux_out.data_ptr() if aux_out is not None else 0, ldaux, act,
        int(accumulate), splitk, alpha,
        L.ptr(map_a), period_a, L.ptr(map_b), L.ptr(map_c), p_drop, seed, _RAW_STREAM(L.device_index()))
    if rc:
        L.check(rc, "s2t_gemm")
    return out


_MASK_BYTES = {}


def relu_mask_bytes(M, N, K):
    key = (M, N, K, OPTION_EPOCH)
    n = _MASK_BYTES.get(key)
    if n is None:
        if len(_MASK_BYTES) > 4096:
            _MASK_BYTES.clear()
        n = _MASK_BYTES[key] = int(_lib().s2t_gemm_relu_mask_bytes(M, N, K))
    return n


def linear_wgrad(dy, x, dw, db=None, splitk=1):
    L.require_cuda(dy, x)
    assert dy.dim() == 2 and x.dim() == 2 and dy.stride(1) == 1 and x.stride(1) == 1 and dy.shape[0] == x.shape[0]
    assert dw.dtype == torch.float32 and dw.stride(1) == 1 and (db is None or db.dtype == torch.float32)
    L.check(_lib().s2t_linear_wgrad(L.dt(dy), dy.shape[1], x.shape[1], dy.shape[0], L.ptr(dy), dy.stride(0), L.ptr(x), x.stride(0),
                                    L.ptr(dw), dw.stride(0), L.ptr(db), int(splitk), L.stream()), "s2t_linear_wgrad")
    return dw


WGRAD_GROUP_MAX = 4096


def wgrad_group(items):
    if not items:
        return
    fn = _lib().s2t_wgrad_group if items[0][0].dtype == torch.bfloat16 else _lib().s2t_wgrad_group_f32
    for i in range(0, len(items), WGRAD_GROUP_MAX):
        chunk = items[i:i + WGRAD_GROUP_MAX]
        arr = (L.WgradProblem * len(chunk))()
        for k, (dy, x, dw, db) in enumerate(chunk):
            if not (dy.is_cuda and x.is_cuda and dw.is_cuda and dw.dtype == torch.float32 and dy.shape[0] == x.shape[0]
                    and dw.shape[0] == dy.shape[1] and dw.shape[1] == x.shape[1] and dy.dtype == x.dtype == items[0][0].dtype):
                raise L.S2THipError("wgrad_group: item %d is not a (dy [tokens, n_out], x [tokens, n_in], f32 dw [n_out, n_in]) device triple" % k)
            p = arr[k]
            p.dY = dy.data_ptr(); p.X = x.data_ptr(); p.dW = dw.data_ptr(); p.db = db.data_ptr() if db is not None else None
            p.n_out = dy.shape[1]; p.n_in = x.shape[1]; p.tokens = dy.shape[0]
            p.ldy = dy.stride(0); p.ldx = x.stride(0); p.ldw = dw.stride(0)
        L.check(fn(len(chunk), ctypes.addressof(arr), L.stream()), "s2t_wgrad_group")


def wgrad_group_raw(n, items_addr):
    if n:
        L.check(_lib().s2t_wgrad_group(int(n), int(items_addr), L.stream()), "s2t_wgrad_group")


def layer_ws_bytes(desc, training):
    return int(_lib().s2t_layer_ws_bytes(ctypes.addressof(desc), int(training)))


def layer_tmp_bytes(desc):
    return int(_lib().s2t_layer_bwd_tmp_bytes(ctypes.addressof(desc)))


def layer_fwd(desc_addr, call_addr):
    rc = _lib().s2t_layer_fwd(desc_addr, call_addr, L.stream())
    if rc:
        L.check(rc, "s2t_layer_fwd")


def layer_bwd(desc_addr, call_addr):
    rc = _lib().s2t_layer_bwd(desc_addr, call_addr, L.stream())
    if rc:
        L.check(rc, "s2t_layer_bwd")


def wgrad_group_ok(dy, x):
    if dy.dtype == torch.float32 and x.dtype == torch.float32:
        return (dy.stride(1) == 1 and x.stride(1) == 1 and dy.stride(0) % 4 == 0 and x.stride(0) % 4 == 0
                and dy.data_ptr() % 16 == 0 and x.data_ptr() % 16 == 0
                and (dy.shape[1] + 3) // 4 * 4 <= dy.stride(0) and (x.shape[1] + 3) // 4 * 4 <= x.stride(0))
    return (dy.dtype == torch.bfloat16 and x.dtype == torch.bfloat16 and dy.stride(1) == 1 and x.stride(1) == 1
            and dy.stride(0) % 8 == 0 and x.stride(0) % 8 == 0 and dy.data_ptr() % 16 == 0 and x.data_ptr() % 16 == 0
            and dy.shape[1] >= 8 and x.shape[1] >= 8
            and (dy.shape[1] + 7) // 8 * 8 <= dy.stride(0) and (x.shape[1] + 7) // 8 * 8 <= x.stride(0))


def colsum(x, out):
    assert x.dim() == 2 and x.stride(1) == 1 and out.dtype == torch.float32
    L.check(_lib().s2t_colsum(L.dt(x), L.ptr(x), x.stride(0), x.shape[0], x.shape[1], L.ptr(out), L.stream()), "s2t_colsum")
    return out


def _tb(x):
    return x.stride(0), x.stride(1)


def attn_fwd(q, k, v, heads, klen=None, causal=False, scale=None, p_drop=0.0, seed=0, out=None, dist_penalty=False):
    Tq, B, D = q.shape
    Tk = k.shape[0]
    d = D // heads
    if scale is None:
        scale = d ** -0.5
    if out is None:
        out = torch.empty((Tq, B, D), dtype=q.dtype, device=q.device)
    lse = torch.empty((B, heads, Tq), dtype=torch.float32, device=q.device)
    rc = _lib().s2t_attn_fwd(L.dt(q), d, B, heads, Tq, Tk, L.ptr(q), *_tb(q), L.ptr(k), *_tb(k), L.ptr(v), *_tb(v),
                             L.ptr(out), *_tb(out), L.ptr(lse), L.ptr(klen), int(causal), int(bool(dist_penalty)), float(scale), float(p_drop),
                             int(seed), L.stream())
    L.check(rc, "s2t_attn_fwd")
    return out, lse


def attn_probs_avg(q, k, heads, klen=None, scale=None, heads_used=None):
    Tq, B, D = q.shape
    Tk = k.shape[0]
    d = D // heads
    out = torch.empty((B, Tq, Tk), dtype=torch.float32, device=q.device)
    L.check(_lib().s2t_attn_probs_avg(L.dt(q), d, B, heads, Tq, Tk, L.ptr(q), *_tb(q), L.ptr(k), *_tb(k), L.ptr(klen),
                                      int(heads_used or heads), float(d ** -0.5 if scale is None else scale), L.ptr(out), L.stream()),
            "s2t_attn_probs_avg")
    return out


def attn_bwd(q, k, v, o, do, lse, heads, dq, dk, dv, klen=None, causal=False, scale=None, p_drop=0.0, seed=0, dist_penalty=False):
    Tq, B, D = q.shape
    Tk = k.shape[0]
    d = D // heads
    if scale is None:
        scale = d ** -0.5
    delta = torch.empty((B, heads, Tq), dtype=torch.float32, device=q.device)
    rc = _lib().s2t_attn_bwd(L.dt(q), d, B, heads, Tq, Tk, L.ptr(q), *_tb(q), L.ptr(k), *_tb(k), L.ptr(v), *_tb(v),
                             L.ptr(o), *_tb(o), L.ptr(do), *_tb(do), L.ptr(lse), L.ptr(delta),
                             L.ptr(dq), *_tb(dq), L.ptr(dk), *_tb(dk), L.ptr(dv), *_tb(dv),
                             L.ptr(klen), int(causal), int(bool(dist_penalty)), float(scale), float(p_drop), int(seed), L.stream())
    L.check(rc, "s2t_attn_bwd")
    return dq, dk, dv


_LN_FWD = _LN_BWD = None


def layernorm_fwd(x, gamma, beta, eps=1e-5):
    global _LN_FWD
    if _LN_FWD is None:
        _LN_FWD = _lib().s2t_layernorm_fwd
    if not (x.is_cuda and gamma.is_cuda and beta.is_cuda):
        raise L.S2THipError("S2T kernels need device tensors: the hot path has no CPU fallback")
    D = x.shape[-1]
    M = x.numel() // D
    assert x.is_contiguous()
    y = torch.empty_like(x)
    st = torch.empty((2, M), dtype=torch.float32, device=x.device)
    mean, rstd = st[0], st[1]
    rc = _LN_FWD(_DT[x.dtype], x.data_ptr(), gamma.data_ptr(), beta.data_ptr(), y.data_ptr(), mean.data_ptr(), rstd.data_ptr(),
                 M, D, float(eps), _RAW_STREAM(L.device_index()))
    if rc:
        L.check(rc, "s2t_layernorm_fwd")
    return y, mean, rstd


def layernorm_bwd(dy, x, mean, rstd, gamma, dgamma, dbeta, dres=None, drop=None):
    global _LN_BWD
    if _LN_BWD is None:
        _LN_BWD = _lib().s2t_layernorm_bwd
    if not (dy.is_cuda and x.is_cuda and mean.is_cuda and rstd.is_cuda and gamma.is_cuda and dgamma.is_cuda and dbeta.is_cuda
            and (dres is None or dres.is_cuda)):
        raise L.S2THipError("S2T kernels need device tensors: the hot path has no CPU fallback")
    D = x.shape[-1]
    M = x.numel() // D
    assert dy.is_contiguous() and x.is_contiguous() and (dres is None or dres.is_contiguous())
    dx = torch.empty_like(x)
    dxd = torch.empty_like(x) if drop is not None else None
    p, seed = drop if drop is not None else (0.0, 0)
    rc = _LN_BWD(_DT[x.dtype], dy.data_ptr(), x.data_ptr(), mean.data_ptr(), rstd.data_ptr(), gamma.data_ptr(),
                 dres.data_ptr() if dres is not None else 0, dx.data_ptr(), dgamma.data_ptr(), dbeta.data_ptr(), M, D,
                 dxd.data_ptr() if dxd is not None else 0, float(p), int(seed), _RAW_STREAM(L.device_index()))
    if rc:
        L.check(rc, "s2t_layernorm_bwd")
    return dx if drop is None else (dx, dxd)


def conv1_fwd(x, w, bias, C, dtype, act=ACT_RELU):
    B, T, F = x.shape
    T2, F2 = (T + 1) // 2, (F + 1) // 2
    y = torch.empty((B, T2, F2, C), dtype=dtype, device=x.device)
    pre = torch.empty_like(y) if act == ACT_GELU else None
    sums = torch.zeros((2 * C,), dtype=torch.float64, device=x.device)
    L.check(_lib().s2t_conv1_fwd(L.dt(y), L.ptr(x), L.ptr(w), L.ptr(bias), L.ptr(y), L.ptr(pre), L.ptr(sums), B, T, F, C, act,
                                 L.stream()), "s2t_conv1_fwd")
    return y, sums, pre


def conv1_bwd(x, dpre, dw, db):
    B, T, F = x.shape
    C = dpre.shape[-1]
    L.check(_lib().s2t_conv1_bwd(L.dt(dpre), L.ptr(x), L.ptr(dpre), L.ptr(dw), L.ptr(db), B, T, F, C, L.stream()),
            "s2t_conv1_bwd")


def chan_sums(y, C, dyn=None, mean=None, rstd=None):
    P = y.numel() // C
    sums = torch.zeros((2 * C,), dtype=torch.float64, device=y.device)
    L.check(_lib().s2t_chan_sums(L.dt(y), L.ptr(y), L.ptr(dyn), L.ptr(mean), L.ptr(rstd), L.ptr(sums), P, C,
                                 0 if dyn is None else 1, L.stream()), "s2t_chan_sums")
    return sums


def conv1_bwd_bn(x, dyn, y, mean, rstd, gamma, sums, dw, db, dgamma, dbeta, count, training=True, pre=None):
    B, T, F = x.shape
    C = y.shape[-1]
    L.check(_lib().s2t_conv1_bwd_bn(L.dt(y), L.ptr(x), L.ptr(dyn), L.ptr(y), L.ptr(pre), L.ptr(mean), L.ptr(rstd), L.ptr(gamma), L.ptr(sums),
                                    L.ptr(dw), L.ptr(db), L.ptr(dgamma), L.ptr(dbeta), B, T, F, C, float(count), int(training), L.stream()),
            "s2t_conv1_bwd_bn")


def bn_finalize(sums, gamma, beta, run_mean, run_var, num_batches, count, training, momentum=0.1, eps=1e-5):
    C = gamma.numel()
    o = torch.empty((4, C), dtype=torch.float32, device=gamma.device)
    L.check(_lib().s2t_bn_finalize(L.ptr(sums), L.ptr(gamma), L.ptr(beta), L.ptr(run_mean), L.ptr(run_var),
                                   L.ptr(num_batches), L.ptr(o[0]), L.ptr(o[1]), L.ptr(o[2]), L.ptr(o[3]),
                                   float(count), C, int(training), float(momentum), float(eps), L.stream()), "s2t_bn_finalize")
    return o[0], o[1], o[2], o[3]


def bn_apply(y, scale, shift, p_drop=0.0, seed=0):
    yn = torch.empty_like(y)
    L.check(_lib().s2t_bn_apply(L.dt(y), L.ptr(y), L.ptr(scale), L.ptr(shift), L.ptr(yn), y.numel(), scale.numel(), float(p_drop),
                                int(seed), L.stream()), "s2t_bn_apply")
    return yn


def bn_bwd_apply(dyn, y, mean, rstd, gamma, sums, dgamma, dbeta, count, training=True, pre=None):
    dpre = torch.empty_like(y)
    L.check(_lib().s2t_bn_bwd_apply(L.dt(y), L.ptr(dyn), L.ptr(y), L.ptr(pre), L.ptr(mean), L.ptr(rstd), L.ptr(gamma), L.ptr(sums),
                                    L.ptr(dpre), L.ptr(dgamma), L.ptr(dbeta), y.numel(), gamma.numel(), float(count),
                                    int(training), L.stream()), "s2t_bn_bwd_apply")
    return dpre


def permute_cf(src, dst, N, C, F, mode):
    L.check(_lib().s2t_permute_cf(L.dt(dst), L.ptr(src), L.ptr(dst), N, C, F, mode, L.stream()), "s2t_permute_cf")
    return dst


def permute_conv_w(src, dst, Co, Ci, mode):
    L.check(_lib().s2t_permute_conv_w(L.dt(dst), L.ptr(src), L.ptr(dst), Co, Ci, mode, L.stream()), "s2t_permute_conv_w")
    return dst


def add_pos(x, table, len32, out=None, p_drop=0.0, seed=0):
    T, B, D = x.shape
    out = x if out is None else out
    assert x.is_contiguous() and out.is_contiguous() and out.shape == x.shape and out.dtype == x.dtype
    assert table.shape[0] >= T + 1 and table.shape[1] == D
    L.check(_lib().s2t_add_pos(L.dt(x), L.ptr(x), L.ptr(out), L.ptr(table), L.ptr(len32), T, B, D, float(p_drop), int(seed), L.stream()),
            "s2t_add_pos")
    return out


def padded_cols(V, dtype):
    e = 8 if dtype == torch.bfloat16 else 4
    return (V + e - 1) // e * e


def alloc_rows(rows_shape, V, dtype, device, zero=False):
    ld = padded_cols(V, dtype)
    buf = (torch.zeros if zero else torch.empty)(tuple(rows_shape) + (ld,), dtype=dtype, device=device)
    return buf[..., :V]


def _row_ld(x):
    assert x.stride(-1) == 1
    ld = x.stride(-2)
    if x.dim() == 3:
        if x.shape[1] == 1:
            return x.stride(0) if x.shape[0] > 1 else max(ld, x.shape[2])
        assert x.shape[0] == 1 or x.stride(0) == x.shape[1] * ld
    return ld


def ctc_argmax(logits, want_lse=False):
    T, B, V = logits.shape
    pred = torch.empty((B, T), dtype=torch.int32, device=logits.device)
    pmax = torch.empty((B, T), dtype=torch.float32, device=logits.device)
    lse = torch.empty((T * B,), dtype=torch.float32, device=logits.device) if want_lse else None
    L.check(_lib().s2t_ctc_argmax(L.dt(logits), L.ptr(logits), L.ptr(pred), L.ptr(pmax), L.ptr(lse), T, B, V, _row_ld(logits), L.stream()),
            "s2t_ctc_argmax")
    return (pred, pmax, lse) if want_lse else (pred, pmax)


def ctc_rle(pred, pmax, len64, strategy=0):
    B, T = pred.shape
    dev = pred.device
    seg = torch.empty((B, T), dtype=torch.int32, device=dev)
    rs = torch.empty((B, T), dtype=torch.int32, device=dev)
    rl = torch.empty((B, T), dtype=torch.int32, device=dev)
    new_len = torch.empty((B,), dtype=torch.int64, device=dev)
    w = torch.empty((B, T), dtype=torch.float32, device=dev)
    L.check(_lib().s2t_ctc_rle(L.ptr(pred), L.ptr(pmax), L.ptr(len64), L.ptr(seg), L.ptr(rs), L.ptr(rl), L.ptr(new_len),
                               L.ptr(w), T, B, strategy, L.stream()), "s2t_ctc_rle")
    return seg, rs, rl, new_len, w


def ctc_compress_fwd(x, w, rs, rl, new_len, Tout):
    T, B, D = x.shape
    out = torch.empty((Tout, B, D), dtype=x.dtype, device=x.device)
    L.check(_lib().s2t_ctc_compress_fwd(L.dt(x), L.ptr(x), L.ptr(w), L.ptr(rs), L.ptr(rl), L.ptr(new_len), L.ptr(out),
                                        T, B, D, Tout, L.stream()), "s2t_ctc_compress_fwd")
    return out


def ctc_compress_bwd(dout, w, seg, dx, accumulate=False):
    T, B, D = dx.shape
    L.check(_lib().s2t_ctc_compress_bwd(L.dt(dx), L.ptr(dout), L.ptr(w), L.ptr(seg), L.ptr(dx), T, B, D, int(accumulate),
                                        L.stream()), "s2t_ctc_compress_bwd")
    return dx


CTC_MAX_TARGET, CTC_MAX_VOCAB = 511, 40704


def ctc_loss(logits, targets, tgt_len, in_len32, blank, grad_scale=1.0, defer_grad=False, lse=None, route="auto"):
    T, B, V = logits.shape
    Lmax = targets.shape[1]
    if route not in ("auto", "any"):
        raise ValueError("ctc_loss route must be 'auto' or 'any', got %r" % (route,))
    if route == "auto":
        route = "fixed" if Lmax <= CTC_MAX_TARGET and V <= CTC_MAX_VOCAB else "any"
    dev = logits.device
    lse_given = lse is not None
    if lse is None:
        lse = torch.empty((T * B,), dtype=torch.float32, device=dev)
    assert lse.numel() == T * B and lse.dtype == torch.float32
    nll = torch.empty((B,), dtype=torch.float32, device=dev)
    ld = _row_ld(logits)
    grad = None if defer_grad else torch.empty((T, B, ld), dtype=logits.dtype, device=dev)[..., :V]
    loss = torch.zeros((1,), dtype=torch.float32, device=dev)
    phase = (1 if defer_grad else 0) | (4 if lse_given else 0)
    if route == "fixed":
        S = next(r for r in (64, 128, 256, 512, 1024) if 2 * Lmax + 1 <= r)
        la = torch.empty((B * T * S,), dtype=torch.float32, device=dev)
        lb = torch.empty((B * T * S,), dtype=torch.float32, device=dev)
        L.check(_lib().s2t_ctc_loss(L.dt(logits), L.ptr(logits), L.ptr(targets), L.ptr(tgt_len), L.ptr(in_len32), L.ptr(lse),
                                    L.ptr(la), L.ptr(lb), L.ptr(nll), L.ptr(grad), L.ptr(loss), T, B, V, ld, Lmax, blank,
                                    float(grad_scale), phase, 0, L.stream()), "s2t_ctc_loss")
    else:
        nbytes = _lib().s2t_ctc_loss_any_workspace(T, B, Lmax, V)
        la = torch.empty(((nbytes + 3) // 4,), dtype=torch.float32, device=dev)
        lb = None
        L.check(_lib().s2t_ctc_loss_any(L.dt(logits), L.ptr(logits), L.ptr(targets), L.ptr(tgt_len), L.ptr(in_len32), L.ptr(lse),
                                        L.ptr(la), L.ptr(nll), L.ptr(grad), L.ptr(loss), T, B, V, ld, Lmax, blank,
                                        float(grad_scale), phase, 0, L.stream()), "s2t_ctc_loss_any")
    if defer_grad:
        return loss, (logits, targets, tgt_len, in_len32, lse, la, lb, nll, blank, float(grad_scale), route), nll
    return loss, grad, nll


def ctc_loss_grad(ws, upstream):
    logits, targets, tgt_len, in_len32, lse, la, lb, nll, blank, grad_scale, route = ws
    T, B, V = logits.shape
    ld = _row_ld(logits)
    grad = torch.empty((T, B, ld), dtype=logits.dtype, device=logits.device)[..., :V]
    assert upstream.dtype == torch.float32 and upstream.numel() == 1
    if route == "fixed":
        L.check(_lib().s2t_ctc_loss(L.dt(logits), L.ptr(logits), L.ptr(targets), L.ptr(tgt_len), L.ptr(in_len32), L.ptr(lse),
                                    L.ptr(la), L.ptr(lb), L.ptr(nll), L.ptr(grad), 0, T, B, V, ld, targets.shape[1], blank,
                                    grad_scale, 2, L.ptr(upstream), L.stream()), "s2t_ctc_loss")
    else:
        L.check(_lib().s2t_ctc_loss_any(L.dt(logits), L.ptr(logits), L.ptr(targets), L.ptr(tgt_len), L.ptr(in_len32), L.ptr(lse),
                                        L.ptr(la), L.ptr(nll), L.ptr(grad), 0, T, B, V, ld, targets.shape[1], blank,
                                        grad_scale, 2, L.ptr(upstream), L.stream()), "s2t_ctc_loss_any")
    return grad


def lsce(logits, target, eps, pad, want_grad=True, grad_scale=1.0):
    rows, V = logits.shape
    assert target.numel() == rows
    ld = _row_ld(logits)
    sums = torch.zeros((2,), dtype=torch.float32, device=logits.device)
    dl = torch.empty((rows, ld), dtype=logits.dtype, device=logits.device)[:, :V] if want_grad else None
    L.check(_lib().s2t_lsce(L.dt(logits), L.ptr(logits), L.ptr(target), L.ptr(dl), L.ptr(sums), rows, V, ld, float(eps), pad,
                            float(grad_scale), L.stream()), "s2t_lsce")
    return sums, dl


def kd_loss(logits, target, teacher_idx, teacher_logits, lam, tau, pad, want_grad=True, grad_scale=1.0):
    rows, V = logits.shape
    ld = _row_ld(logits)
    s = torch.zeros((1,), dtype=torch.float32, device=logits.device)
    dl = torch.empty((rows, ld), dtype=logits.dtype, device=logits.device)[:, :V] if want_grad else None
    Kt = teacher_idx.shape[-1] if teacher_idx is not None else 0
    L.check(_lib().s2t_kd_loss(L.dt(logits), L.ptr(logits), L.ptr(target), L.ptr(teacher_idx), L.ptr(teacher_logits), L.ptr(dl),
                               L.ptr(s), rows, V, ld, Kt, float(lam), float(tau), pad, float(grad_scale), L.stream()), "s2t_kd_loss")
    return s, dl


def embed_fwd(tokens, W, table, scale, pad, pos_offset=0):
    B, Ln = tokens.shape
    D = W.shape[1]
    out = torch.empty((Ln, B, D), dtype=W.dtype, device=W.device)
    L.check(_lib().s2t_embed_fwd(L.dt(W), L.ptr(tokens), L.ptr(W), L.ptr(table), L.ptr(out), B, Ln, D, float(scale), pad,
                                 int(pos_offset), L.stream()), "s2t_embed_fwd")
    return out


def conv2_wgrad(dpre, y1n, gw, B, T2, F2, C):
    rc = _lib().s2t_conv2_wgrad(L.dt(dpre), L.ptr(dpre), L.ptr(y1n), L.ptr(gw), B, T2, F2, C, L.stream())
    if rc == -95:
        return False
    L.check(rc, "s2t_conv2_wgrad")
    return True


def conv2_fwd(y1n, w2p, bias, B, T2, F2, C, act=ACT_RELU):
    T4, F4 = (T2 + 1) // 2, (F2 + 1) // 2
# ... 297 lines not shown
```

### fbk_fairseq_st_amd/lib.py

```python
import ctypes
import os
import subprocess

import torch

_HERE = os.path.dirname(os.path.abspath(__file__))
LIB_PATH = os.environ.get("S2T_HIP_LIB") or os.path.join(_HERE, "libs2t_hip.so")
CSRC = os.path.join(_HERE, "csrc")

F32, BF16 = 0, 1
ABI_VERSION = 9
ACT_NONE, ACT_RELU, ACT_GELU, ACT_RELU_BWD, ACT_GELU_BWD, ACT_RELU_MASK, ACT_RELU_BWD_MASK = 0, 1, 2, 3, 4, 5, 6

c_int, c_long, c_float, c_double, c_void_p, c_size_t = (ctypes.c_int, ctypes.c_long, ctypes.c_float,
                                                        ctypes.c_double, ctypes.c_void_p, ctypes.c_size_t)
c_ull = ctypes.c_ulonglong
c_longlong = ctypes.c_longlong
P = c_void_p

SIGNATURES = {
    "s2t_abi_version": [],
    "s2t_gemm": [c_int] * 7 + [P, c_int, P, c_int, P, c_int, P, P, c_int, P, P, c_int, c_int, c_int, c_int, c_float, P],
    "s2t_gemm_gather": [c_int] * 7 + [P, c_int, P, c_int, P, c_int, P, P, c_int, P, P, c_int, c_int, c_int, c_int,
                                       c_float, P, c_int, P, P, c_float, c_ull, P],
    "s2t_gemm_relu_mask_bytes": [c_int, c_int, c_int],
    "s2t_linear_wgrad": [c_int, c_int, c_int, c_int, P, c_int, P, c_int, P, c_int, P, c_int, P],
    "s2t_wgrad_group": [c_int, P, P],
    "s2t_wgrad_group_f32": [c_int, P, P],
    "s2t_colsum": [c_int, P, c_int, c_int, c_int, P, P],
    "s2t_attn_fwd": [c_int] * 6 + [P, c_long, c_long] * 4 + [P, P, c_int, c_int, c_float, c_float, c_ull, P],
    "s2t_attn_bwd": [c_int] * 6 + [P, c_long, c_long] * 5 + [P, P] + [P, c_long, c_long] * 3 +
                    [P, c_int, c_int, c_float, c_float, c_ull, P],
    "s2t_attn_probs_avg": [c_int] * 6 + [P, c_long, c_long] * 2 + [P, c_int, c_float, P, P],
    "s2t_layernorm_fwd": [c_int, P, P, P, P, P, P, c_int, c_int, c_float, P],
    "s2t_layernorm_bwd": [c_int, P, P, P, P, P, P, P, P, P, c_int, c_int, P, c_float, c_ull, P],
    "s2t_conv1_fwd": [c_int, P, P, P, P, P, P, c_int, c_int, c_int, c_int, c_int, P],
    "s2t_conv1_bwd": [c_int, P, P, P, P, c_int, c_int, c_int, c_int, P],
    "s2t_conv1_bwd_bn": [c_int] + [P] * 12 + [c_int, c_int, c_int, c_int, c_double, c_int, P],
    "s2t_chan_sums": [c_int, P, P, P, P, P, c_long, c_int, c_int, P],
    "s2t_bn_finalize": [P] * 10 + [c_double, c_int, c_int, c_float, c_float, P],
    "s2t_bn_apply": [c_int, P, P, P, P, c_long, c_int, c_float, c_ull, P],
    "s2t_bn_bwd_apply": [c_int, P, P, P, P, P, P, P, P, P, P, c_long, c_int, c_double, c_int, P],
    "s2t_permute_cf": [c_int, P, P, c_int, c_int, c_int, c_int, P],
    "s2t_permute_conv_w": [c_int, P, P, c_int, c_int, c_int, P],
    "s2t_add_pos": [c_int, P, P, P, P, c_int, c_int, c_int, c_float, c_ull, P],
    "s2t_ctc_argmax": [c_int, P, P, P, P, c_int, c_int, c_int, c_int, P],
    "s2t_ctc_rle": [P] * 8 + [c_int, c_int, c_int, P],
    "s2t_ctc_compress_fwd": [c_int, P, P, P, P, P, P, c_int, c_int, c_int, c_int, P],
    "s2t_ctc_compress_bwd": [c_int, P, P, P, P, c_int, c_int, c_int, c_int, P],
    "s2t_ctc_loss": [c_int, P, P, P, P, P, P, P, P, P, P, c_int, c_int, c_int, c_int, c_int, c_int, c_float, c_int, P, P],
    "s2t_ctc_loss_any_workspace": [c_int, c_int, c_int, c_int],
    "s2t_ctc_loss_any": [c_int, P, P, P, P, P, P, P, P, P, c_int, c_int, c_int, c_int, c_int, c_int, c_float, c_int, P, P],
    "s2t_lsce": [c_int, P, P, P, P, c_long, c_int, c_int, c_float, c_int, c_float, P],
    "s2t_kd_loss": [c_int, P, P, P, P, P, P, c_long, c_int, c_int, c_int, c_float, c_float, c_int, c_float, P],
    "s2t_embed_fwd": [c_int, P, P, P, P, c_int, c_int, c_int, c_float, c_int, c_int, P],
    "s2t_log_softmax": [c_int, P, P, c_long, c_int, c_int, c_float, P],
    "s2t_softmax_probs": [c_int, P, P, c_long, c_int, c_int, c_float, P],
    "s2t_softmax_bwd": [c_int, P, P, P, c_long, c_int, c_int, c_float, c_int, P],
    "s2t_ensemble_lse": [c_int, P, P, c_size_t, P],
    "s2t_score_targets": [c_int, c_int, P, P, P, P, c_int, c_int, c_int, P],
    "s2t_embed_bwd": [c_int, P, P, P, c_int, c_int, c_int, c_float, c_int, P],
    "s2t_act_bwd": [c_int, P, P, P, c_size_t, c_int, c_float, c_ull, P],
    "s2t_add_inplace": [c_int, P, P, c_size_t, P],
    "s2t_dropout": [c_int, P, P, c_size_t, c_float, c_ull, P],
    "s2t_grad_norm_clip": [P, c_size_t, P, c_float, c_float, P, P],
    "s2t_grad_norm_clip_div": [P, c_size_t, P, c_float, P, c_float, P, P],
    "s2t_adam_step": [P, P, P, P, P, c_size_t, P, c_float, c_float, c_float, c_float, c_float, c_int, P],
    "s2t_cast": [c_int, c_int, P, P, c_size_t, P],
    "s2t_scale_by_device_scalar": [c_int, P, c_size_t, P, P],
    "s2t_set_option": [ctypes.c_char_p, c_int],
    "s2t_comm_standin": [P, P, c_size_t, c_int, c_int, c_float, P],
    "s2t_prof_enable": [c_int],
    "s2t_prof_reset": [],
    "s2t_prof_read": [ctypes.c_char_p, P, P, P, P],
    "s2t_conv2_wgrad": [c_int, P, P, P, c_int, c_int, c_int, c_int, P],
    "s2t_conv2_fwd": [c_int, P, P, P, P, P, c_int, c_int, c_int, c_int, c_int, P],
    "s2t_conv2_dgrad": [c_int, P, P, P, c_int, c_int, c_int, c_int, c_float, c_ull, P],
    "s2t_topk": [c_int, P, P, P, c_long, c_int, c_int, c_int, P],
    "s2t_augment": [P, P, P, P, P, c_int, c_int, c_int, c_int, c_int, c_int, P],
    "s2t_a2d_chan_stats": [c_int, P, P, P, P, P, P, P, P, c_long, c_int, c_int, c_int, c_int, c_int, P],
    "s2t_a2d_bn_act": [c_int, P, P, P, P, P, P, c_long, c_int, c_int, c_int, P],
    "s2t_a2d_bn_bwd": [c_int, P, P, P, P, P, P, P, P, P, c_long, c_int, c_int, c_int, c_int, c_double, c_int, P],
    "s2t_a2d_param_grads": [P, P, P, c_int, P],
    "s2t_a2d_pack_w": [c_int, P, P, P, c_int, c_int, c_int, c_int, c_int, P],
    "s2t_a2d_conv_wgrad": [c_int, P, c_int, P, c_int, P, P, c_int, c_int, c_int, c_int, c_int, P],
    "s2t_a2d_planes": [c_int, P, P, c_int, c_int, c_int, c_int, c_int, c_int, c_int, P],
    "s2t_a2d_time_fwd": [c_int, P, P, P, c_int, c_int, c_int, c_float, c_ull, P],
    "s2t_a2d_time_bwd": [c_int, P, P, P, P, P, P, c_int, c_int, c_int, c_float, c_ull, P],
    "s2t_a2d_freq_fwd": [c_int, P, P, P, c_int, c_int, c_int, c_float, c_ull, P],
    "s2t_a2d_freq_bwd": [c_int, P, P, P, P, c_int, c_int, c_int, c_float, c_ull, P],
    "s2t_layer_ws_bytes": [P, c_int],
    "s2t_layer_bwd_tmp_bytes": [P],
    "s2t_layer_fwd": [P, P, P],
    "s2t_layer_bwd": [P, P, P],
    "s2t_decode_prepare_enc": [c_int, P, P, P, c_int, c_int, c_int, c_int, c_int, P],
    "s2t_decode_pack_weight": [c_int, P, c_int, c_int, c_int, P, P],
    "s2t_decode_begin": [P, c_int, P],
    "s2t_decode_step": [P, P],
    "s2t_decode_step_rules": [P, P, P],
    "s2t_decode_lds_bytes": [P],
    "s2t_decode_graph_create": [P, c_int, P],
    "s2t_decode_graph_create_rules": [P, P, c_int, P],
    "s2t_decode_begin_ensemble": [P, c_int, c_int, P],
    "s2t_decode_step_ensemble": [P, c_int, P, P],
    "s2t_decode_graph_create_ensemble": [P, c_int, P, c_int, P],
    "s2t_decode_step_sample": [P, c_int, P, P, P],
    "s2t_decode_graph_create_sample": [P, c_int, P, P, c_int, P],
    "s2t_decode_begin_ex": [P, c_int, P, P, P, c_int, P],
    "s2t_decode_step_ex": [P, c_int, P, P, P, P],
    "s2t_decode_graph_create_ex": [P, c_int, P, P, P, c_int, P],
    "s2t_sample_rows": [P, c_long, c_int, c_int, c_int, c_int, c_float, c_ull, c_int, P, P, P, P],
    "s2t_decode_graph_launch": [P, P],
    "s2t_decode_graph_destroy": [P],
    "s2t_host_batch_by_size": [P, c_longlong, P, c_longlong, c_longlong, c_int, P, P, P],
    "s2t_host_ctc_uer": [P, P, c_int, c_int, P, P, c_int, c_int, P, P],
}

class WgradProblem(ctypes.Structure):
    _fields_ = [("dY", c_void_p), ("X", c_void_p), ("dW", c_void_p), ("db", c_void_p),
                ("n_out", c_int), ("n_in", c_int), ("tokens", c_int), ("ldy", c_int), ("ldx", c_int), ("ldw", c_int)]


_LAYER_W = ("qkv", "o", "xq", "xkv", "xo", "fc1", "fc2")
_LAYER_LN = ("ln1_g", "ln1_b", "lnx_g", "lnx_b", "ln2_g", "ln2_b")


class LayerDesc(ctypes.Structure):
    _fields_ = ([(n, c_int) for n in ("dtype", "decoder", "T", "B", "D", "heads", "ffn", "Ts", "gelu", "causal", "dist_penalty")] +
                [(n, c_float) for n in ("ln_eps", "p_drop", "p_attn", "p_act")] +
                [("w_" + n, c_void_p) for n in _LAYER_W] + [("b_" + n, c_void_p) for n in _LAYER_W] + [(n, c_void_p) for n in _LAYER_LN] +
                [("g_w_" + n, c_void_p) for n in _LAYER_W] + [("g_b_" + n, c_void_p) for n in _LAYER_W] + [("g_" + n, c_void_p) for n in _LAYER_LN])


class LayerCall(ctypes.Structure):
    _fields_ = [("training", c_int), ("self_klen", c_void_p), ("enc_klen", c_void_p),
                ("seed_sa_attn", c_ull), ("seed_sa_out", c_ull), ("seed_xa_attn", c_ull), ("seed_xa_out", c_ull), ("seed_ffn_act", c_ull),
                ("seed_ffn_out", c_ull), ("x", c_void_p), ("enc", c_void_p), ("y", c_void_p), ("ws", c_void_p),
                ("dy", c_void_p), ("dy_drop", c_void_p), ("dx", c_void_p), ("dx_drop", c_void_p), ("nxt_p", c_float), ("nxt_seed", c_ull),
                ("denc", c_void_p), ("denc_accumulate", c_int), ("tmp", c_void_p), ("items", c_void_p), ("max_items", c_int), ("n_items", c_int)]


_DEC_LAYER = ("ln1_g", "ln1_b", "w_qkv", "b_qkv", "w_o", "b_o", "lnx_g", "lnx_b", "w_xq", "b_xq", "w_xo", "b_xo", "ln2_g", "ln2_b",
              "w_fc1", "b_fc1", "w_fc2", "b_fc2", "kv_enc", "vt_enc", "kv_cache")


class DecodeLayer(ctypes.Structure):
    _fields_ = [(n, c_void_p) for n in _DEC_LAYER]


class DecodeDesc(ctypes.Structure):
    _fields_ = ([(n, c_int) for n in ("dtype", "B", "beam", "D", "heads", "ffn", "layers", "V", "ldv", "Ts", "Tsp", "max_len", "min_len",
                                      "ffn_slices", "gelu", "pad", "unk", "eos", "step0_all_slots")] +
                [(n, c_float) for n in ("ln_eps", "embed_scale", "unk_penalty", "inv_temperature")] +
                [(n, c_void_p) for n in ("layer", "lnf_g", "lnf_b", "w_out", "embed", "pos_table", "enc_klen", "init_scores",
                                         "x0", "x1", "part0", "part1", "xn", "logits", "steps", "anc", "cand_val", "cand_idx",
                                         "tok_hist", "par_hist", "cum_hist", "blacklist", "nfin", "finished", "fin_step", "fin_row",
                                         "fin_score")] +
                [("diverse_groups", c_int), ("diverse_strength", c_float)])


class DecodeRules(ctypes.Structure):
    _fields_ = [("no_repeat_ngram", c_int), ("prefix_len", c_int), ("prefix", c_void_p)]


class DecodeSample(ctypes.Structure):
    _fields_ = [("topk", c_int), ("topp", c_float), ("key", c_ull)]


class DecodeExtras(ctypes.Structure):
    _fields_ = [("lne_g", c_void_p * 8), ("lne_b", c_void_p * 8), ("attn_part", c_void_p), ("attn_hist", c_void_p)]


_lib = None


def build(verbose=False):
    cmd = ["make", "-C", CSRC, "-j", str(min(8, os.cpu_count() or 4)), "all"]
    res = subprocess.run(cmd, stdout=subprocess.PIPE, stderr=subprocess.STDOUT, text=True)
    if res.returncode != 0:
        raise RuntimeError("building libs2t_hip.so failed:\n" + res.stdout[-4000:])
    if verbose:
        print(res.stdout[-2000:])
    build_fastcall()
    return LIB_PATH


FAST_PATH = os.path.join(_HERE, "_s2t_fastcall.so")
_HOST_SIDE = ("s2t_host_batch_by_size", "s2t_host_ctc_uer")
_SIZE_T_RESULT = ("s2t_gemm_relu_mask_bytes", "s2t_layer_ws_bytes", "s2t_layer_bwd_tmp_bytes", "s2t_decode_lds_bytes",
                  "s2t_ctc_loss_any_workspace")


def signature_hash():
    import hashlib
    text = ";".join("%s(%s)%s" % (n, ",".join(t.__name__ for t in SIGNATURES[n]), "z" if n in _SIZE_T_RESULT else "i") for n in sorted(SIGNATURES))
    return int(hashlib.sha256(text.encode()).hexdigest()[:15], 16)


def _fastcall_source():
    out = ['#define PY_SSIZE_T_CLEAN', '#include <Python.h>', '#include "s2t_hip.h"', '',
           'static inline unsigned long long as_ptr(PyObject* o) { return o == Py_None ? 0ull : PyLong_AsUnsignedLongLongMask(o); }', '']
    names = sorted(SIGNATURES)
    for name in names:
        at = SIGNATURES[name]
        n = len(at)
        decl, call = [], []
        for i, t in enumerate(at):
            if t in (c_float, c_double):
                decl.append("    const double a%d = PyFloat_AsDouble(args[%d]);" % (i, i))
                call.append("(%s)a%d" % ("float" if t is c_float else "double", i))
            elif t is P:
                decl.append("    const unsigned long long a%d = as_ptr(args[%d]);" % (i, i))
                call.append("(void*)a%d" % i)
            elif t is ctypes.c_char_p:
                decl.append("    const char* a%d = PyBytes_AsString(args[%d]);" % (i, i))
                call.append("a%d" % i)
            elif t is c_ull:
                decl.append("    const unsigned long long a%d = PyLong_AsUnsignedLongLongMask(args[%d]);" % (i, i))
                call.append("a%d" % i)
            else:
                decl.append("    const long long a%d = PyLong_AsLongLong(args[%d]);" % (i, i))
                call.append({c_int: "(int)a%d", c_long: "(long)a%d", c_longlong: "(long long)a%d", c_size_t: "(size_t)a%d"}[t] % i)
        out.append("static PyObject* w_%s(PyObject* self, PyObject* const* args, Py_ssize_t nargs) {" % name)
        out.append('    if (nargs != %d) { PyErr_SetString(PyExc_TypeError, "%s takes %d arguments"); return NULL; }' % (n, name, n))
        out += decl
        out.append("    if (PyErr_Occurred()) return NULL;")
        proto = ", ".join({c_float: "float", c_double: "double", P: "void*", ctypes.c_char_p: "const char*", c_ull: "unsigned long long",
                           c_int: "int", c_long: "long", c_longlong: "long long", c_size_t: "size_t"}[t] for t in at) or "void"
        ret = "size_t" if name in _SIZE_T_RESULT else "int"
        out.append("    %s (*fn)(%s) = (%s (*)(%s))%s;" % (ret, proto, ret, proto, name))
        if name in _HOST_SIDE:
            out.append("    %s r;" % ret)
            out.append("    Py_BEGIN_ALLOW_THREADS")
            out.append("    r = fn(%s);" % ", ".join(call))
            out.append("    Py_END_ALLOW_THREADS")
        else:
            out.append("    const %s r = fn(%s);" % (ret, ", ".join(call)))
        out.append("    return %s;" % ("PyLong_FromSize_t(r)" if ret == "size_t" else "PyLong_FromLong((long)r)"))
        out.append("}")
    out.append("static PyObject* w_s2t_build_info(PyObject* self, PyObject* const* args, Py_ssize_t nargs) { return PyBytes_FromString(s2t_build_info()); }")
    out.append("static PyObject* w_s2t_signature_hash(PyObject* self, PyObject* const* args, Py_ssize_t nargs) { return PyLong_FromLongLong(%dLL); }" % signature_hash())
    out.append("static PyMethodDef methods[] = {")
    for name in names + ["s2t_build_info", "s2t_signature_hash"]:
        out.append('    {"%s", (PyCFunction)(void (*)(void))w_%s, METH_FASTCALL, ""},' % (name, name))
    out.append("    {NULL, NULL, 0, NULL}};")
    out.append('static struct PyModuleDef moddef = {PyModuleDef_HEAD_INIT, "_s2t_fastcall", "generated binding of include/s2t_hip.h", -1, methods};')
    out.append("PyMODINIT_FUNC PyInit__s2t_fastcall(void) { return PyModule_Create(&moddef); }")
    return "\n".join(out) + "\n"


def build_fastcall():
    import sysconfig
    obj = os.path.join(CSRC, "_obj")
    os.makedirs(obj, exist_ok=True)
    src = os.path.join(obj, "s2t_fastcall.c")
    text = _fastcall_source()
    if not (os.path.exists(src) and open(src).read() == text and os.path.exists(FAST_PATH)
            and os.path.getmtime(FAST_PATH) >= os.path.getmtime(os.path.join(_HERE, "libs2t_hip.so"))):
        with open(src, "w") as f:
            f.write(text)
        cmd = ["gcc", "-O2", "-shared", "-fPIC", "-I" + sysconfig.get_paths()["include"], "-I" + os.path.join(os.path.dirname(_HERE), "include"),
               src, "-o", FAST_PATH, "-L" + _HERE, "-l:libs2t_hip.so", "-Wl,-rpath,$ORIGIN"]
        res = subprocess.run(cmd, stdout=subprocess.PIPE, stderr=subprocess.STDOUT, text=True)
        if res.returncode != 0:
            raise RuntimeError("building the CPython binding failed:\n" + res.stdout[-4000:])
    return FAST_PATH


def load():
    global _lib
    if _lib is not None:
        return _lib
    if not os.path.exists(LIB_PATH):
        raise ImportError("libs2t_hip.so not found at %s -- run `python -c 'import __graft_entry__ as g; g.build()'` "
                          "(there is no CPU or PyTorch fallback for the S2T hot path)" % LIB_PATH)
    lib = ctypes.CDLL(LIB_PATH)
    for name, argtypes in SIGNATURES.items():
        fn = getattr(lib, name)
        fn.argtypes = argtypes
        fn.restype = c_int
    lib.s2t_build_info.restype = ctypes.c_char_p
    for name in _SIZE_T_RESULT:
        getattr(lib, name).restype = c_size_t
    lib.s2t_build_info.argtypes = []
    if lib.s2t_abi_version() != ABI_VERSION:
        raise ImportError("libs2t_hip.so at %s has ABI version %d, this package binds version %d -- rebuild it (make -C %s)"
                          % (LIB_PATH, lib.s2t_abi_version(), ABI_VERSION, CSRC))
    global _ctypes_lib
    _ctypes_lib = lib
    _lib = _load_fastcall(lib) or lib
    return _lib


def _load_fastcall(ctypes_lib):
    if os.environ.get("S2T_HIP_LIB") or os.environ.get("S2T_HIP_CTYPES") or not os.path.exists(FAST_PATH):
        return None
    import importlib.util
    try:
        spec = importlib.util.spec_from_file_location("_s2t_fastcall", FAST_PATH)
        mod = importlib.util.module_from_spec(spec)
        spec.loader.exec_module(mod)
    except Exception:
        return None
    if any(not hasattr(mod, n) for n in SIGNATURES) or mod.s2t_abi_version() != ABI_VERSION:
        return None
    if getattr(mod, "s2t_signature_hash", lambda: None)() != signature_hash():
        import warnings
        warnings.warn("fbk_fairseq_st_amd: the generated binding %s was built from another signature table; falling back to ctypes "
                      "(~4 us per launch instead of 0.3) -- run __graft_entry__.build()" % FAST_PATH)
        return None
    return mod


_ctypes_lib = None


def load_ctypes():
    load()
    return _ctypes_lib


class S2THipError(RuntimeError):
    pass


def check(rc, what):
    if rc != 0:
        if rc <= -1000:
            raise S2THipError("%s: HIP error %d" % (what, -rc - 1000))
        raise S2THipError("%s: error %d (%s)" % (what, rc, {-22: "invalid argument", -95: "not supported"}.get(rc, "?")))


def dt(t):
    if t.dtype == torch.float32:
        return F32
    if t.dtype == torch.bfloat16:
        return BF16
    raise TypeError("S2T kernels take float32 or bfloat16 tensors, got %s" % t.dtype)


def ptr(t):
    if t is None:
        return 0
    if not t.is_cuda:
        raise S2THipError("S2T kernels need device tensors: the hot path has no CPU fallback")
    return t.data_ptr()


_GET_DEVICE = torch._C._cuda_getDevice


def device_index():
    return _GET_DEVICE()


def stream():
    return torch._C._cuda_getCurrentRawStream(_GET_DEVICE())


def require_cuda(*ts):
    for t in ts:
        if t is not None and not t.is_cuda:
            raise S2THipError("S2T kernels need device tensors: the hot path has no CPU fallback")
```

### include/s2t_hip.h

```cpp
#ifndef S2T_HIP_H
#define S2T_HIP_H
#include <stddef.h>
#ifdef __cplusplus
extern "C" {
#endif

#define S2T_F32 0
#define S2T_BF16 1

#define S2T_ACT_NONE 0
#define S2T_ACT_RELU 1
#define S2T_ACT_GELU 2
#define S2T_ACT_RELU_BWD 3
#define S2T_ACT_GELU_BWD 4
#define S2T_ACT_RELU_MASK 5
#define S2T_ACT_RELU_BWD_MASK 6

int s2t_conv2_wgrad(int dtype, const void* dpre, const void* y1n, float* gw, int B, int T2, int F2, int C, void* stream);
int s2t_conv2_fwd(int dtype, const void* y1n, const void* w2p, const float* bias, void* z2, void* pre, int B, int T2, int F2, int C,
                  int act, void* stream);
int s2t_conv2_dgrad(int dtype, const void* dpre, const void* w2q, void* dy1n, int B, int T2, int F2, int C, float p_drop,
                    unsigned long long seed, void* stream);
int s2t_topk(int dtype, const void* x, float* vals, int* idx, long rows, int V, int ld, int K, void* stream);
int s2t_augment(const float* x, float* out, const int* row_map, const int* fmask, const int* tmask, int B, int T, int To, int F,
                int nF, int nT, void* stream);
int s2t_host_batch_by_size(const long long* indices, long long n, const long long* lens, long long max_tokens,
                           long long max_sentences, int bsz_mult, long long* out_flat, long long* out_offsets,
                           long long* n_batches);
int s2t_abi_version(void);
const char* s2t_build_info(void);

int s2t_gemm(int in_dtype, int out_dtype, int trans_a, int trans_b, int M, int N, int K,
             const void* A, int lda, const void* B, int ldb, void* C, int ldc,
             const float* bias, const void* residual, int ldr, const void* aux, void* aux_out, int ldaux,
             int act, int accumulate, int splitk, float alpha, void* stream);

int s2t_gemm_gather(int in_dtype, int out_dtype, int trans_a, int trans_b, int M, int N, int K,
                    const void* A, int lda, const void* B, int ldb, void* C, int ldc,
                    const float* bias, const void* residual, int ldr, const void* aux, void* aux_out, int ldaux,
                    int act, int accumulate, int splitk, float alpha,
                    const int* mapA, int periodA, const int* mapB, const int* mapC,
                    float p_drop, unsigned long long seed, void* stream);
size_t s2t_gemm_relu_mask_bytes(int M, int N, int K);

typedef struct S2TWgradProblem {
    const void* dY; const void* X; float* dW; float* db;
    int n_out, n_in, tokens, ldy, ldx, ldw;
} S2TWgradProblem;
int s2t_wgrad_group(int n, const S2TWgradProblem* probs, void* stream);
int s2t_wgrad_group_f32(int n, const S2TWgradProblem* probs, void* stream);

int s2t_linear_wgrad(int in_dtype, int n_out, int n_in, int tokens, const void* dY, int ldy, const void* X, int ldx,
                     float* dW, int ldw, float* db, int splitk, void* stream);
int s2t_colsum(int dtype, const void* X, int ld, int M, int N, float* out, void* stream);

int s2t_attn_fwd(int dtype, int head_dim, int B, int H, int Tq, int Tk,
                 const void* Q, long q_st, long q_sb, const void* K, long k_st, long k_sb,
                 const void* V, long v_st, long v_sb, void* O, long o_st, long o_sb, float* LSE,
                 const int* klen, int causal, int dist_penalty, float scale, float p_drop, unsigned long long seed, void* stream);
int s2t_attn_probs_avg(int dtype, int head_dim, int B, int H, int Tq, int Tk, const void* Q, long q_st, long q_sb,
                       const void* K, long k_st, long k_sb, const int* klen, int heads_used, float scale, float* out, void* stream);
int s2t_attn_bwd(int dtype, int head_dim, int B, int H, int Tq, int Tk,
                 const void* Q, long q_st, long q_sb, const void* K, long k_st, long k_sb,
                 const void* V, long v_st, long v_sb, const void* O, long o_st, long o_sb,
                 const void* dO, long do_st, long do_sb, const float* LSE, float* Delta,
                 void* dQ, long dq_st, long dq_sb, void* dK, long dk_st, long dk_sb, void* dV, long dv_st, long dv_sb,
                 const int* klen, int causal, int dist_penalty, float scale, float p_drop, unsigned long long seed, void* stream);

int s2t_layernorm_fwd(int dtype, const void* x, const float* gamma, const float* beta, void* y,
                      float* mean, float* rstd, int M, int D, float eps, void* stream);
int s2t_layernorm_bwd(int dtype, const void* dy, const void* x, const float* mean, const float* rstd,
                      const float* gamma, const void* dres, void* dx, float* dgamma, float* dbeta,
                      int M, int D, void* dx_drop, float p_drop, unsigned long long seed, void* stream);

typedef struct S2TLayerDesc {
    int dtype, decoder;
    int T, B, D, heads, ffn, Ts;
    int gelu, causal, dist_penalty;
    float ln_eps, p_drop, p_attn, p_act;
    const void *w_qkv, *w_o, *w_xq, *w_xkv, *w_xo, *w_fc1, *w_fc2;
    const float *b_qkv, *b_o, *b_xq, *b_xkv, *b_xo, *b_fc1, *b_fc2;
    const float *ln1_g, *ln1_b, *lnx_g, *lnx_b, *ln2_g, *ln2_b;
    float *g_w_qkv, *g_w_o, *g_w_xq, *g_w_xkv, *g_w_xo, *g_w_fc1, *g_w_fc2;
    float *g_b_qkv, *g_b_o, *g_b_xq, *g_b_xkv, *g_b_xo, *g_b_fc1, *g_b_fc2;
    float *g_ln1_g, *g_ln1_b, *g_lnx_g, *g_lnx_b, *g_ln2_g, *g_ln2_b;
} S2TLayerDesc;
typedef struct S2TLayerCall {
    int training;
    const int* self_klen; const int* enc_klen;
    unsigned long long seed_sa_attn, seed_sa_out, seed_xa_attn, seed_xa_out, seed_ffn_act, seed_ffn_out;
    const void* x; const void* enc; void* y; void* ws;
    const void* dy; const void* dy_drop; void* dx; void* dx_drop; float nxt_p; unsigned long long nxt_seed;
    void* denc; int denc_accumulate; void* tmp;
    S2TWgradProblem* items; int max_items; int n_items;
} S2TLayerCall;
size_t s2t_layer_ws_bytes(const S2TLayerDesc* L, int training);
size_t s2t_layer_bwd_tmp_bytes(const S2TLayerDesc* L);
int s2t_layer_fwd(const S2TLayerDesc* L, S2TLayerCall* c, void* stream);
int s2t_layer_bwd(const S2TLayerDesc* L, S2TLayerCall* c, void* stream);

int s2t_conv1_fwd(int dtype, const float* x, const float* w, const float* bias, void* y, void* pre, double* sums,
                  int B, int T, int F, int C, int act, void* stream);
int s2t_conv1_bwd(int dtype, const float* x, const void* dpre, float* dw, float* db, int B, int T, int F, int C, void* stream);
int s2t_conv1_bwd_bn(int dtype, const float* x, const void* dyn, const void* y, const void* pre, const float* mean, const float* rstd,
                     const float* gamma, const double* sums, float* dw, float* db, float* dgamma, float* dbeta, int B, int T, int F,
                     int C, double count, int training, void* stream);
int s2t_chan_sums(int dtype, const void* y, const void* dyn, const float* mean, const float* rstd,
                  double* sums, long P, int C, int mode, void* stream);
int s2t_bn_finalize(const double* sums, const float* gamma, const float* beta, float* run_mean, float* run_var,
                    long long* num_batches, float* mean, float* rstd, float* scale, float* shift,
                    double count, int C, int training, float momentum, float eps, void* stream);
int s2t_bn_apply(int dtype, const void* y, const float* scale, const float* shift, void* yn, long n, int C,
                 float p_drop, unsigned long long seed, void* stream);
int s2t_bn_bwd_apply(int dtype, const void* dyn, const void* y, const void* pre, const float* mean, const float* rstd,
                     const float* gamma, const double* sums, void* dpre, float* dgamma, float* dbeta,
                     long n, int C, double count, int training, void* stream);
int s2t_permute_cf(int dst_dtype, const float* src, void* dst, int N, int C, int F, int mode, void* stream);
int s2t_permute_conv_w(int dst_dtype, const float* src, void* dst, int Co, int Ci, int mode, void* stream);
int s2t_add_pos(int dtype, const void* src, void* dst, const float* table, const int* len, int T, int B, int D,
                float p_drop, unsigned long long seed, void* stream);

int s2t_ctc_argmax(int dtype, const void* logits, int* pred, float* pmax, float* lse, int T, int B, int V, int ld, void* stream);
int s2t_ctc_rle(const int* pred, const float* pmax, const long long* len, int* seg, int* run_start, int* run_len,
                long long* new_len, float* w, int T, int B, int strategy, void* stream);
int s2t_ctc_compress_fwd(int dtype, const void* x, const float* w, const int* run_start, const int* run_len,
                         const long long* new_len, void* out, int T, int B, int D, int Tout, void* stream);
int s2t_ctc_compress_bwd(int dtype, const void* dout, const float* w, const int* seg, void* dx, int T, int B, int D,
                         int accumulate, void* stream);

#define S2T_CTC_MAX_TARGET 511
#define S2T_CTC_MAX_VOCAB 40704
#define S2T_CTC_ROW(Lmax) (2 * (Lmax) + 1 <= 64 ? 64 : 2 * (Lmax) + 1 <= 128 ? 128 : 2 * (Lmax) + 1 <= 256 ? 256 : 2 * (Lmax) + 1 <= 512 ? 512 : 1024)
int s2t_ctc_loss(int dtype, const void* logits, const long long* targets, const long long* tgt_len, const int* in_len,
                 float* lse, float* la, float* lb, float* nll, void* grad, float* loss_sum,
                 int T, int B, int V, int ld, int Lmax, int blank, float grad_scale, int phase, const float* grad_scale_dev,
                 void* stream);
size_t s2t_ctc_loss_any_workspace(int T, int B, int Lmax, int V);
int s2t_ctc_loss_any(int dtype, const void* logits, const long long* targets, const long long* tgt_len, const int* in_len,
                     float* lse, void* ws, float* nll, void* grad, float* loss_sum,
                     int T, int B, int V, int ld, int Lmax, int blank, float grad_scale, int phase, const float* grad_scale_dev,
                     void* stream);
int s2t_lsce(int dtype, const void* logits, const long long* target, void* dlogits, float* sums2,
             long rows, int V, int ld, float eps, int pad, float grad_scale, void* stream);

int s2t_kd_loss(int dtype, const void* logits, const long long* target, const long long* teacher_idx,
                const float* teacher_logits, void* dlogits, float* sum1, long rows, int V, int ld, int Kt,
                float lambda, float tau, int pad, float grad_scale, void* stream);

int s2t_embed_fwd(int dtype, const long long* tokens, const void* W, const float* table, void* out,
                  int B, int L, int D, float scale, int pad, int pos_offset, void* stream);
int s2t_log_softmax(int dtype, const void* logits, float* out, long rows, int V, int ld, float inv_temperature, void* stream);
int s2t_softmax_probs(int dtype, const void* logits, float* out, long rows, int V, int ld, float inv_temperature, void* stream);
int s2t_softmax_bwd(int dtype, const float* out, const float* dout, void* dlogits, long rows, int V, int ld, float inv_temperature,
                    int log_probs, void* stream);
int s2t_ensemble_lse(int n, const float* const* lprobs, float* out, size_t numel, void* stream);
int s2t_score_targets(int dtype, int n, const void* const* logits, const int* ld, const long long* target, float* out,
                      int B, int L, int V, void* stream);
int s2t_embed_bwd(int dtype, const long long* tokens, const void* dout, float* dW, int B, int L, int D,
                  float scale, int pad, void* stream);
int s2t_act_bwd(int dtype, const void* dy, const void* y, void* out, size_t n, int act, float p_drop, unsigned long long seed,
                void* stream);
int s2t_add_inplace(int dtype, const void* x, void* y, size_t n, void* stream);
int s2t_dropout(int dtype, const void* x, void* y, size_t n, float p, unsigned long long seed, void* stream);

int s2t_a2d_chan_stats(int dtype, const void* z, const void* dy, const float* prescale, const float* mean, const float* rstd,
                       const float* scale, const float* shift, double* sums, long M, int C, int ld_z, int ld_dy, int Cg,
                       int mode, void* stream);
int s2t_a2d_bn_act(int dtype, const void* z, const float* prescale, const float* scale, const float* shift, const void* res,
                   void* y, long M, int C, int ld_z, int ld_y, void* stream);
int s2t_a2d_bn_bwd(int dtype, const void* dy, const void* z, const float* prescale, const float* mean, const float* rstd,
                   const float* scale, const float* shift, const double* sums, void* dz, long M, int C, int ld_dy, int ld_z,
                   int Cg, double count, int training, void* stream);
int s2t_a2d_param_grads(const double* sums, float* dgamma, float* dbeta, int Cg, void* stream);
int s2t_a2d_pack_w(int dst_dtype, const float* src, void* dst, float* grad, int Co, int Ci, int CP, int ld, int mode, void* stream);
#define S2T_A2D_WGRAD_GROUPS 512
int s2t_a2d_conv_wgrad(int dtype, const void* dY, int ld_dy, const void* X, int ld_x, float* dW, float* ws, int CO, int CI,
                       int B, int T, int F, void* stream);
int s2t_a2d_planes(int dtype, void* chl, void* planes, int G, int ch0, int ld, int B, int T, int F, int dir, void* stream);
int s2t_a2d_time_fwd(int dtype, const void* qkv, void* cat, float* lse, int B, int T, int F, float p_drop,
                     unsigned long long seed, void* stream);
int s2t_a2d_time_bwd(int dtype, const void* qkv, const void* cat, const void* dcat, const float* lse, float* delta, void* dqkv,
                     int B, int T, int F, float p_drop, unsigned long long seed, void* stream);
int s2t_a2d_freq_fwd(int dtype, const void* qkv, void* cat, float* A, int B, int T, int F, float p_drop,
                     unsigned long long seed, void* stream);
int s2t_a2d_freq_bwd(int dtype, const void* qkv, const void* dcat, const float* A, void* dqkv, int B, int T, int F,
                     float p_drop, unsigned long long seed, void* stream);

int s2t_grad_norm_clip(const float* g, size_t n, double* acc_ws, float scale, float max_norm, float* out2, void* stream);
int s2t_grad_norm_clip_div(const float* g, size_t n, double* acc_ws, float scale, const double* divisor_dev, float max_norm,
                           float* out2, void* stream);
int s2t_adam_step(float* p, const float* g, float* m, float* v, void* shadow_bf16, size_t n, const float* mult2,
                  float lr, float beta1, float beta2, float eps, float wd, int step, void* stream);
int s2t_cast(int src_dtype, int dst_dtype, const void* src, void* dst, size_t n, void* stream);
int s2t_scale_by_device_scalar(int dtype, void* x, size_t n, const float* scalar, void* stream);

typedef struct S2TDecodeLayer {
    const void *ln1_g, *ln1_b;
    const void *w_qkv, *b_qkv;
    const void *w_o, *b_o;
    const void *lnx_g, *lnx_b;
    const void *w_xq, *b_xq, *w_xo, *b_xo;
    const void *ln2_g, *ln2_b;
    const void *w_fc1, *b_fc1;
    const void *w_fc2, *b_fc2;
    const void* kv_enc;
    const void* vt_enc;
    void* kv_cache;
} S2TDecodeLayer;

typedef struct S2TDecodeDesc {
    int dtype, B, beam, D, heads, ffn, layers, V, ldv, Ts, Tsp, max_len, min_len, ffn_slices, gelu;
    int pad, unk, eos, step0_all_slots;
    float ln_eps, embed_scale, unk_penalty, inv_temperature;
    const S2TDecodeLayer* layer;
    const void *lnf_g, *lnf_b;
    const void* w_out;
    const void* embed;
    const float* pos_table;
    const int* enc_klen;
    const float* init_scores;
    float *x0, *x1;
    void *part0, *part1;
    void* xn;
    float* logits;
    int* steps;
    int* anc;
    float* cand_val; int* cand_idx;
    int* tok_hist; int* par_hist; float* cum_hist;
    int* blacklist;
    int* nfin; int* finished;
    int* fin_step; int* fin_row; float* fin_score;
    int diverse_groups; float diverse_strength;
} S2TDecodeDesc;

int s2t_decode_pack_weight(int dtype, const void* W, int ldw, int N, int K, void* Wp, void* stream);
int s2t_decode_prepare_enc(int dtype, const void* kv, void* kv_enc, void* vt_enc, int Ts, int Tsp, int B, int D, int heads, void* stream);
int s2t_decode_begin(const S2TDecodeDesc* d, int bos, void* stream);
int s2t_decode_step(const S2TDecodeDesc* d, void* stream);
typedef struct S2TDecodeRules { int no_repeat_ngram, prefix_len; const int* prefix; } S2TDecodeRules;
int s2t_decode_step_rules(const S2TDecodeDesc* d, const S2TDecodeRules* r, void* stream);
size_t s2t_decode_lds_bytes(const S2TDecodeDesc* d);
int s2t_decode_graph_create(const S2TDecodeDesc* d, int n_steps, void** graph_exec);
int s2t_decode_graph_create_rules(const S2TDecodeDesc* d, const S2TDecodeRules* r, int n_steps, void** graph_exec);
int s2t_decode_begin_ensemble(const S2TDecodeDesc* const* d, int n, int bos, void* stream);
int s2t_decode_step_ensemble(const S2TDecodeDesc* const* d, int n, const S2TDecodeRules* r, void* stream);
int s2t_decode_graph_create_ensemble(const S2TDecodeDesc* const* d, int n, const S2TDecodeRules* r, int n_steps, void** graph_exec);
int s2t_decode_graph_launch(void* graph_exec, void* stream);
int s2t_decode_graph_destroy(void* graph_exec);
int s2t_sample_rows(const float* lprobs, long rows, int V, int ld, int draws, int topk, float topp, unsigned long long key, int step,
                    int* tok, float* lp_out, int* n_kept, void* stream);
typedef struct S2TDecodeSample { int topk; float topp; unsigned long long key; } S2TDecodeSample;
int s2t_decode_step_sample(const S2TDecodeDesc* const* d, int n, const S2TDecodeRules* r, const S2TDecodeSample* s, void* stream);
int s2t_decode_graph_create_sample(const S2TDecodeDesc* const* d, int n, const S2TDecodeRules* r, const S2TDecodeSample* s, int n_steps,
                                   void** graph_exec);

typedef struct S2TDecodeExtras { const float* lne_g[8]; const float* lne_b[8]; float* attn_part; float* attn_hist; } S2TDecodeExtras;
int s2t_decode_begin_ex(const S2TDecodeDesc* const* d, int n, const S2TDecodeRules* r, const S2TDecodeSample* s, const S2TDecodeExtras* x,
                        int bos, void* stream);
int s2t_decode_step_ex(const S2TDecodeDesc* const* d, int n, const S2TDecodeRules* r, const S2TDecodeSample* s, const S2TDecodeExtras* x,
                       void* stream);
int s2t_decode_graph_create_ex(const S2TDecodeDesc* const* d, int n, const S2TDecodeRules* r, const S2TDecodeSample* s,
                               const S2TDecodeExtras* x, int n_steps, void** graph_exec);

int s2t_comm_standin(const void* src, void* dst, size_t bytes, int workgroups, int ranks, float bus_gbps, void* stream);

int s2t_prof_enable(int on);
int s2t_set_option(const char* key, int value);
int s2t_prof_read(const char* family, double* ms, long long* launches, double* flops, double* bytes);
int s2t_prof_reset(void);

int s2t_host_ctc_uer(const int* pred, const long long* input_len, int B, int T, const long long* targets,
                     const long long* target_len, int L, int blank, double* errors, double* total);

#ifdef __cplusplus
}
#endif
#endif
```

Baseline: 6.641 million.

## Save attention dropout keep bitmask in forward and reuse it in backward

The forward flash-attention kernel gets a KEEP variant that packs the per-element dropout keep decisions into a bitmask written to a workspace buffer. The backward dQ and dK/dV kernels read that bitmask instead of regenerating the dropout hash: dq2 loads it straight from global memory, and dkv2 copies it into LDS through global_load_lds. The layer code allocates the buffer and routes non-causal encoder self-attention through the new path. This swaps the hash arithmetic repeated in both backward kernels for extra global writes and reads plus 2 KB more LDS in dkv2, which may affect occupancy.

```diff
diff --git a/fbk_fairseq_st_amd/csrc/attention.hip b/fbk_fairseq_st_amd/csrc/attention.hip
--- a/fbk_fairseq_st_amd/csrc/attention.hip
+++ b/fbk_fairseq_st_amd/csrc/attention.hip
@@ -90,7 +90,12 @@
     int B, H, Tq, Tk, causal;
     int dist_pen;
     float scale, p_drop; unsigned long long seed;
+    uint32_t* keep;
 };
+
+__device__ __forceinline__ size_t keep_block(const AttnArgs& p, int head, int bx, int t) {
+    return (((size_t)head * ((p.Tq + 127) >> 7) + bx) * ((p.Tk + 63) >> 6) + t) * 256;
+}
 
 __device__ __forceinline__ uint64_t drop_index(const AttnArgs& p, int b, int h, int qrow, int key) {
     return (((uint64_t)b * p.H + h) * p.Tq + qrow) * (uint64_t)((p.Tk + 3) & ~3) + key;
@@ -103,6 +108,13 @@
 
 __device__ __forceinline__ uint32_t drop_pair(uint32_t pair, uint32_t fields, uint32_t thm1x2) {
     uint32_t d, k, r;
+    asm("v_pk_sub_u16 %0, %1, %2 clamp" : "=v"(d) : "v"(fields), "v"(thm1x2));
+    asm("v_pk_min_u16 %0, %1, %2" : "=v"(k) : "v"(d), "v"(0x00010001u));
+    asm("v_pk_mul_lo_u16 %0, %1, %2" : "=v"(r) : "v"(pair), "v"(k));
+    return r;
+}
+__device__ __forceinline__ uint32_t drop_pair_k(uint32_t pair, uint32_t fields, uint32_t thm1x2, uint32_t& k) {
+    uint32_t d, r;
     asm("v_pk_sub_u16 %0, %1, %2 clamp" : "=v"(d) : "v"(fields), "v"(thm1x2));
     asm("v_pk_min_u16 %0, %1, %2" : "=v"(k) : "v"(d), "v"(0x00010001u));
     asm("v_pk_mul_lo_u16 %0, %1, %2" : "=v"(r) : "v"(pair), "v"(k));
@@ -267,6 +279,7 @@
 #define ASTAMP(T, K)
 #define ASTAMP_EARLY(KID)
 #endif
+template <bool KEEP>
 __global__ __launch_bounds__(256, 3) void attn_fwd2_kernel(AttnArgs p) {
     constexpr int DH = 64;
     ASTAMP_EARLY(0)
@@ -363,6 +376,7 @@
             }
         }
         u32x4 pf[2][2];
+        uint32_t keepw = 0u;
         auto softmax_tile = [&](auto fast_tag, auto drop_tag) {
             constexpr bool FAST = decltype(fast_tag)::value, DROP = decltype(drop_tag)::value;
             const bool pen = !FAST && p.dist_pen;
@@ -395,6 +409,7 @@
                 const bool drop = FAST ? DROP : has_drop;
                 const uint64_t quad0 = drop ? drop_index(p, b, h, qrow, kv0 + 4 * q) >> 2 : 0;
                 const uint32_t qlo = (uint32_t)quad0, hwm0 = drop_high_mix(p.seed, quad0);
+                uint32_t k01s = 0u, k23s = 0u;
 #pragma unroll
                 for (int j = 0; j < 4; ++j) {
                     float pv[4];
@@ -403,21 +418,35 @@
                     rs2 += (f32x2_t){pv[0], pv[1]};
                     rs2 += (f32x2_t){pv[2], pv[3]};
                     uint32_t p01 = pack_bf16(pv[0], pv[1]), p23 = pack_bf16(pv[2], pv[3]);
-                    if (drop) {
+                    if constexpr (KEEP && FAST && DROP) {
+                        const u32x2 hq = drop_hash4_lo(drop_ks, hwm0, qlo + 4u * j);
+                        uint32_t k01, k23;
+                        p01 = drop_pair_k(p01, hq[1], drop_thm1x2, k01); p23 = drop_pair_k(p23, hq[0], drop_thm1x2, k23);
+                        k01s |= k01 << (4 * j); k23s |= k23 << (4 * j);
+                    } else if (drop) {
                         const u32x2 hq = FAST ? drop_hash4_lo(drop_ks, hwm0, qlo + 4u * j) : drop_hash4(p.seed, quad0 + 4 * j);
                         p01 = drop_pair(p01, hq[1], drop_thm1x2); p23 = drop_pair(p23, hq[0], drop_thm1x2);
                     }
                     pf[qb][j >> 1][2 * (j & 1)] = p01;
                     pf[qb][j >> 1][2 * (j & 1) + 1] = p23;
                 }
+                if constexpr (KEEP && FAST && DROP) {
+                    const uint32_t tw = k01s | (k23s << 2), hw = tw | (tw >> 15);
+                    keepw |= qb == 0 ? (hw & 0xffffu) : (hw << 16);
+                }
                 l[qb] = l[qb] * alpha + (rs2[0] + rs2[1]);
 #pragma unroll
                 for (int n = 0; n < 4; ++n) o[qb][n] *= alpha;
             }
         };
-        if (!plain) softmax_tile(std::false_type{}, std::false_type{});
-        else if (has_drop) softmax_tile(std::true_type{}, std::true_type{});
-        else softmax_tile(std::true_type{}, std::false_type{});
+        if constexpr (KEEP) {
+            softmax_tile(std::true_type{}, std::true_type{});
+            *reinterpret_cast<uint32_t*>(reinterpret_cast<char*>(p.keep + keep_block(p, head, bx, t)) + threadIdx.x * 4u) = keepw;
+        } else {
+            if (!plain) softmax_tile(std::false_type{}, std::false_type{});
+            else if (has_drop) softmax_tile(std::true_type{}, std::true_type{});
+            else softmax_tile(std::true_type{}, std::false_type{});
+        }
         ASTAMP(t, 2)
 #pragma unroll
         for (int kb = 0; kb < 2; ++kb)
@@ -704,6 +733,7 @@
 }
 #define S2T_WAIT_VM0() __builtin_amdgcn_s_waitcnt(0x0F70)
 
+template <bool KEEP>
 __global__ __launch_bounds__(256, 2) void attn_bwd_dkv2_kernel(AttnArgs p) {
     constexpr int DH = 64;
     ASTAMP_EARLY(2)
@@ -737,8 +767,17 @@
     const int qstart = p.causal ? bx * 128 : 0;
     const int ntile = qstart < p.Tq ? (p.Tq - qstart + 63) / 64 : 0;
     float* sStat = reinterpret_cast<float*>(smem + 32768);
+    char* sKeep = smem + 32768 + 1024 + 32768;
+    const int nkt = (p.Tk + 63) >> 6;
+    const uint32_t keep_sh = 8 * (wave & 1) + (r16 & 3);
     auto stage = [&](int qt, int stg) {
         stage2_dma(Qg, p.q_st, dOg, p.do_st, qt, p.Tq, smem + stg * 16384, wave, lane);
+        if constexpr (KEEP) {
+            const uint32_t* blk = p.keep + keep_block(p, head, qt >> 7, min(2 * bx + (wave >> 1), nkt - 1)) + ((qt >> 6) & 1) * 128;
+            const char* src = reinterpret_cast<const char*>(blk) + (uint32_t)(((wave & 1) * 64 + lane) * 4);
+            __builtin_amdgcn_global_load_lds((__attribute__((address_space(1))) const void*)src,
+                                             (__attribute__((address_space(3))) void*)(sKeep + stg * 1024 + wave * 256), 4, 0, 0);
+        }
         if (wave < 2) {
             float* dst = sStat + stg * 128 + wave * 64;
             if (wave == 1 || qt + lane < p.Tq) {
@@ -779,6 +818,7 @@
         const char* sQ = smem + (t & 1) * 16384;
         const char* sDO = sQ + 8192;
         const float* sL = sStat + (t & 1) * 128;
+        const char* sKp = sKeep + (t & 1) * 1024 + (wave >> 1) * 512 + ((r16 >> 2) * 16 + 4 * q) * 4;
         ASTAMP(t, 0)
         if (t + 1 < ntile) stage(qt + 64, (t + 1) & 1);
         ASTAMP(t, 1)
@@ -795,7 +835,13 @@
             for (int g = 0; g < 2; ++g) { qa[g] = row_frag128(sQ, 16 * i + r16, 4 * g + q); da[g] = row_frag128(sDO, 16 * i + r16, 4 * g + q); }
             const f32x4 L = *reinterpret_cast<const f32x4*>(sL + 16 * i + 4 * q) * 1.44269504088896f;
             const f32x4 Dl = *reinterpret_cast<const f32x4*>(sL + 64 + 16 * i + 4 * q);
-            const uint32_t qrow_quads = DROP ? (uint32_t)(((b * p.H + h) * p.Tq + qt + 16 * i + 4 * q + (r16 & 3))) * tkq : 0u;
+            const uint32_t qrow_quads = (DROP && !KEEP) ? (uint32_t)(((b * p.H + h) * p.Tq + qt + 16 * i + 4 * q + (r16 & 3))) * tkq : 0u;
+            u32x4 kws = {0u, 0u, 0u, 0u};
+            if constexpr (KEEP) {
+                kws = *reinterpret_cast<const u32x4*>(sKp + (i >> 1) * 256);
+#pragma unroll
+                for (int r = 0; r < 4; ++r) kws[r] >>= keep_sh;
+            }
 #pragma unroll
             for (int kb = 0; kb < 2; ++kb) {
                 f32x4 st = {0.f, 0.f, 0.f, 0.f}, dp = {0.f, 0.f, 0.f, 0.f};
@@ -807,7 +853,7 @@
                 }
                 const int key = kw + 16 * kb + r16;
                 uint32_t nib = 0u;
-                if constexpr (DROP) {
+                if constexpr (DROP && !KEEP) {
                     const u32x2 hq = drop_hash4_lo(drop_ks, drop_hwm, qrow_quads + ((uint32_t)key >> 2));
                     uint32_t dy, dx, ky, kx;
                     asm("v_pk_sub_u16 %0, %1, %2 clamp" : "=v"(dy) : "v"(hq[1]), "v"(drop_thm1x2));
@@ -825,7 +871,9 @@
                     float e = __builtin_amdgcn_exp2f(arg);
                     if constexpr (EDGE) e = (qrow < p.Tq && (!p.causal || key <= qrow)) ? e : 0.f;
                     if constexpr (DROP) {
-                        const bool keep = (quad_bcast(nib, r) & own_bit) != 0u;
+                        bool keep;
+                        if constexpr (KEEP) keep = (kws[r] & (1u << (16 * (i & 1) + 4 * kb))) != 0u;
+                        else keep = (quad_bcast(nib, r) & own_bit) != 0u;
                         pv[r] = keep ? e : 0.f;
                         ds[r] = e * __builtin_fmaf(keep ? dp[r] : 0.f, drop_inv, -Dl[r]);
                     } else {
@@ -849,7 +897,8 @@
         }
         };
         const bool edge = generic;
-        if (p.p_drop > 0.f) { if (edge) tile(std::true_type{}, std::true_type{}); else tile(std::false_type{}, std::true_type{}); }
+        if constexpr (KEEP) tile(std::false_type{}, std::true_type{});
+        else if (p.p_drop > 0.f) { if (edge) tile(std::true_type{}, std::true_type{}); else tile(std::false_type{}, std::true_type{}); }
         else if (edge) tile(std::true_type{}, std::false_type{});
         else tile(std::false_type{}, std::false_type{});
         ASTAMP(t, 3)
@@ -881,6 +930,7 @@
     ASTAMP(7, 3)
 }
 
+template <bool KEEP>
 __global__ __launch_bounds__(256, 2) void attn_bwd_dq2_kernel(AttnArgs p) {
     constexpr int DH = 64;
     ASTAMP_EARLY(1)
@@ -947,6 +997,12 @@
 
     const float sc2 = p.scale * 1.44269504088896f;
     const bool generic = p.causal || p.dist_pen;
+    const char* keep_w = nullptr;
+    uint32_t kw_next = 0u;
+    if constexpr (KEEP) {
+        keep_w = reinterpret_cast<const char*>(p.keep + keep_block(p, head, bx, 0));
+        if (ntile > 0) kw_next = *reinterpret_cast<const uint32_t*>(keep_w + threadIdx.x * 4u);
+    }
     S2T_WAIT_VM0();
     __syncthreads();
     ASTAMP(7, 1)
@@ -956,6 +1012,8 @@
         const char* sV = sK + 8192;
         ASTAMP(t, 0)
         if (t + 1 < ntile) stage2_dma(Kg, p.k_st, Vg, p.v_st, kv0 + 64, p.Tk, smem + ((t + 1) & 1) * 16384, wave, lane);
+        const uint32_t kw = kw_next;
+        if constexpr (KEEP) { if (t + 1 < ntile) kw_next = *reinterpret_cast<const uint32_t*>(keep_w + ((uint32_t)(t + 1) * 1024u + threadIdx.x * 4u)); }
         ASTAMP(t, 1)
         u32x4 sf[2][2];
         auto ds_tile = [&](auto edge_tag, auto drop_tag, auto tail_tag) {
@@ -974,7 +1032,7 @@
                 const int qrow = qw + 16 * qb + r16;
                 const int key0 = kv0 + 16 * j + 4 * q;
                 u32x2 hq = {0u, 0u};
-                if constexpr (DROP) hq = drop_hash4_lo(drop_ks, drop_hwm, (uint32_t)((b * p.H + h) * p.Tq + qrow) * tkq + ((uint32_t)key0 >> 2));
+                if constexpr (DROP && !KEEP) hq = drop_hash4_lo(drop_ks, drop_hwm, (uint32_t)((b * p.H + h) * p.Tq + qrow) * tkq + ((uint32_t)key0 >> 2));
                 float ds[4];
 #pragma unroll
                 for (int r = 0; r < 4; ++r) {
@@ -986,7 +1044,8 @@
                         e = (key < klen && (!p.causal || key <= qrow)) ? e : 0.f;
                     }
                     if constexpr (TAIL) e = (16 * j + r < tail_thr) ? e : 0.f;
-                    if constexpr (DROP) ds[r] = e * __builtin_fmaf(drop_field(hq, r) >= drop_th16 ? dp[r] : 0.f, drop_inv, -Dl[qb]);
+                    if constexpr (DROP && KEEP) ds[r] = e * __builtin_fmaf((kw & (1u << (16 * qb + 4 * j + r))) != 0u ? dp[r] : 0.f, drop_inv, -Dl[qb]);
+                    else if constexpr (DROP) ds[r] = e * __builtin_fmaf(drop_field(hq, r) >= drop_th16 ? dp[r] : 0.f, drop_inv, -Dl[qb]);
                     else ds[r] = e * (dp[r] - Dl[qb]);
                 }
                 sf[qb][j >> 1][2 * (j & 1)] = pack_bf16(ds[0], ds[1]); sf[qb][j >> 1][2 * (j & 1) + 1] = pack_bf16(ds[2], ds[3]);
@@ -994,7 +1053,8 @@
         }
         };
         const bool tail = kv0 + 64 > klen;
-        if (generic) { if (p.p_drop > 0.f) ds_tile(std::true_type{}, std::true_type{}, std::false_type{}); else ds_tile(std::true_type{}, std::false_type{}, std::false_type{}); }
+        if constexpr (KEEP) { if (tail) ds_tile(std::false_type{}, std::true_type{}, std::true_type{}); else ds_tile(std::false_type{}, std::true_type{}, std::false_type{}); }
+        else if (generic) { if (p.p_drop > 0.f) ds_tile(std::true_type{}, std::true_type{}, std::false_type{}); else ds_tile(std::true_type{}, std::false_type{}, std::false_type{}); }
         else if (p.p_drop > 0.f) { if (tail) ds_tile(std::false_type{}, std::true_type{}, std::true_type{}); else ds_tile(std::false_type{}, std::true_type{}, std::false_type{}); }
         else if (tail) ds_tile(std::false_type{}, std::false_type{}, std::true_type{});
         else ds_tile(std::false_type{}, std::false_type{}, std::false_type{});
@@ -1443,18 +1503,25 @@
         dkv2 = !v1 && al && idx32 && a.Tk >= 128 && span32(a.q_st, a.Tq) && span32(a.do_st, a.Tq);
         dq2 = !v1 && al && idx32 && span32(a.k_st, a.Tk) && span32(a.v_st, a.Tk) && (a.Tq >= 128 || (a.Tq >= S2T_ATTN_V2_MIN_TQ && a.Tk >= 128)) && !(a.o_st % 8) && !(a.o_sb % 8) && !((uintptr_t)a.O & 15);
         if (dq2) {
-            hipLaunchKernelGGL(attn_bwd_dq2_kernel, dim3((a.Tq + 127) / 128, a.H, a.B), dim3(256), 32768, st, a);
+            if (a.keep) hipLaunchKernelGGL(attn_bwd_dq2_kernel<true>, dim3((a.Tq + 127) / 128, a.H, a.B), dim3(256), 32768, st, a);
+            else hipLaunchKernelGGL(attn_bwd_dq2_kernel<false>, dim3((a.Tq + 127) / 128, a.H, a.B), dim3(256), 32768, st, a);
             S2T_LAUNCH_CHECK();
         } else {
             hipLaunchKernelGGL((attn_delta_kernel<T, DH>), dim3((unsigned)((rows * 16 + 255) / 256)), dim3(256), 0, st, a);
             S2T_LAUNCH_CHECK();
         }
         if (dkv2) {
+            constexpr int lds = 32768 + 1024 + 32768, lds_keep = lds + 2048;
             {
                 static bool attr = false;
-                if (!attr) { (void)hipFuncSetAttribute(reinterpret_cast<const void*>(&attn_bwd_dkv2_kernel), hipFuncAttributeMaxDynamicSharedMemorySize, 32768 + 1024 + 32768); attr = true; }
-            }
-            hipLaunchKernelGGL(attn_bwd_dkv2_kernel, dim3((a.Tk + 127) / 128, a.H, a.B), dim3(256), 32768 + 1024 + 32768, st, a);
+                if (!attr) {
+                    (void)hipFuncSetAttribute(reinterpret_cast<const void*>(&attn_bwd_dkv2_kernel<false>), hipFuncAttributeMaxDynamicSharedMemorySize, lds);
+                    (void)hipFuncSetAttribute(reinterpret_cast<const void*>(&attn_bwd_dkv2_kernel<true>), hipFuncAttributeMaxDynamicSharedMemorySize, lds_keep);
+                    attr = true;
+                }
+            }
+            if (a.keep) hipLaunchKernelGGL(attn_bwd_dkv2_kernel<true>, dim3((a.Tk + 127) / 128, a.H, a.B), dim3(256), lds_keep, st, a);
+            else hipLaunchKernelGGL(attn_bwd_dkv2_kernel<false>, dim3((a.Tk + 127) / 128, a.H, a.B), dim3(256), lds, st, a);
             S2T_LAUNCH_CHECK();
         }
     } else {
@@ -1492,12 +1559,26 @@
     return S2T_OK;
 }
 
-extern "C" int s2t_attn_fwd(int dtype, int head_dim, int B, int H, int Tq, int Tk,
+extern "C" size_t s2t_attn_keep_bytes(int head_dim, int B, int H, int Tq, int Tk, int causal, int dist_penalty, float p_drop) {
+    if (head_dim != 64 || B <= 0 || H <= 0 || Tq <= 0 || Tk <= 0 || causal || dist_penalty || !(p_drop < 1.f)) return 0;
+    if (((uint32_t)fminf(p_drop * 4294967296.f, 4294967295.f) >> 16) == 0) return 0;
+    if (g_s2t_opt_attn_v1 != 0 || Tq <= 64 || !(Tq >= 128 || (Tq >= S2T_ATTN_V2_MIN_TQ && Tk >= 128))) return 0;
+    if (!((unsigned long long)B * H * Tq * (unsigned long long)((Tk + 3) & ~3) < (1ull << 34))) return 0;
+    return (size_t)B * H * ((Tq + 127) / 128) * ((Tk + 63) / 64) * 256 * sizeof(uint32_t);
+}
+static bool keep_route(int dtype, int head_dim, const AttnArgs& a) {
+    return dtype == S2T_BF16 && s2t_attn_keep_bytes(head_dim, a.B, a.H, a.Tq, a.Tk, a.causal, a.dist_pen, a.p_drop) > 0 &&
+           (a.o_st % 4) == 0 && (a.o_sb % 4) == 0 && ((uintptr_t)a.O & 7) == 0 && span32(a.k_st, a.Tk) && span32(a.v_st, a.Tk) &&
+           ((uintptr_t)a.keep & 3) == 0;
+}
+
+static int attn_fwd_impl(int dtype, int head_dim, int B, int H, int Tq, int Tk,
                             const void* Q, long q_st, long q_sb, const void* K, long k_st, long k_sb,
                             const void* V, long v_st, long v_sb, void* O, long o_st, long o_sb, float* LSE,
                             const int* klen, int causal, int dist_penalty, float scale, float p_drop, unsigned long long seed,
-                            void* stream) {
+                            void* keep, void* stream) {
     AttnArgs a{};
+    a.keep = static_cast<uint32_t*>(keep);
     a.dist_pen = dist_penalty;
     a.Q = Q; a.K = K; a.V = V; a.O = O; a.LSE = LSE;
     a.q_st = q_st; a.q_sb = q_sb; a.k_st = k_st; a.k_sb = k_sb; a.v_st = v_st; a.v_sb = v_sb; a.o_st = o_st; a.o_sb = o_sb;
@@ -1508,6 +1589,7 @@
     if (!Q || !K || !V || !O) return S2T_EINVAL;
     const long s[] = {q_st, q_sb, k_st, k_sb, v_st, v_sb};
     if (!strides_ok(dtype, s, 6)) return S2T_EINVAL;
+    if (a.keep && !keep_route(dtype, head_dim, a)) return S2T_ENOTSUP;
     hipStream_t st = (hipStream_t)stream;
     ProfScope prof("attn_fwd", st, 4.0 * B * H * (double)Tq * Tk * head_dim * (causal ? 0.5 : 1.0), 0.0);
     if (dtype == S2T_BF16 && head_dim == 64 && sq_fwd_route(a)) {
@@ -1518,24 +1600,43 @@
     if (dtype == S2T_BF16 && head_dim == 64 && (Tq >= 128 || (Tq >= S2T_ATTN_V2_MIN_TQ && Tk >= 128)) && (o_st % 4) == 0 && (o_sb % 4) == 0 && ((uintptr_t)O & 7) == 0) {
         const bool v1 = g_s2t_opt_attn_v1 != 0 || !span32(k_st, Tk) || !span32(v_st, Tk);
         if (!v1) {
-            hipLaunchKernelGGL(attn_fwd2_kernel, dim3((Tq + 127) / 128, H, B), dim3(256), 32768 + 512 + 16384, st, a);
+            if (a.keep) hipLaunchKernelGGL(attn_fwd2_kernel<true>, dim3((Tq + 127) / 128, H, B), dim3(256), 32768 + 512 + 16384, st, a);
+            else hipLaunchKernelGGL(attn_fwd2_kernel<false>, dim3((Tq + 127) / 128, H, B), dim3(256), 32768 + 512 + 16384, st, a);
             S2T_LAUNCH_CHECK();
             return S2T_OK;
         }
     }
+    if (a.keep) return S2T_ENOTSUP;
     if (dtype == S2T_BF16) return head_dim == 64 ? fwd_launch<bf16, 64>(a, st) : fwd_launch<bf16, 32>(a, st);
     return head_dim == 64 ? fwd_launch<float, 64>(a, st) : fwd_launch<float, 32>(a, st);
 }
-
-extern "C" int s2t_attn_bwd(int dtype, int head_dim, int B, int H, int Tq, int Tk,
+extern "C" int s2t_attn_fwd(int dtype, int head_dim, int B, int H, int Tq, int Tk,
+                            const void* Q, long q_st, long q_sb, const void* K, long k_st, long k_sb,
+                            const void* V, long v_st, long v_sb, void* O, long o_st, long o_sb, float* LSE,
+                            const int* klen, int causal, int dist_penalty, float scale, float p_drop, unsigned long long seed,
+                            void* stream) {
+    return attn_fwd_impl(dtype, head_dim, B, H, Tq, Tk, Q, q_st, q_sb, K, k_st, k_sb, V, v_st, v_sb, O, o_st, o_sb, LSE, klen, causal, dist_penalty,
+                         scale, p_drop, seed, nullptr, stream);
+}
+extern "C" int s2t_attn_fwd_keep(int dtype, int head_dim, int B, int H, int Tq, int Tk,
+                                 const void* Q, long q_st, long q_sb, const void* K, long k_st, long k_sb,
+                                 const void* V, long v_st, long v_sb, void* O, long o_st, long o_sb, float* LSE,
+                                 const int* klen, int causal, int dist_penalty, float scale, float p_drop, unsigned long long seed,
+                                 void* keep, void* stream) {
+    return attn_fwd_impl(dtype, head_dim, B, H, Tq, Tk, Q, q_st, q_sb, K, k_st, k_sb, V, v_st, v_sb, O, o_st, o_sb, LSE, klen, causal, dist_penalty,
+                         scale, p_drop, seed, keep, stream);
+}
+
+static int attn_bwd_impl(int dtype, int head_dim, int B, int H, int Tq, int Tk,
                             const void* Q, long q_st, long q_sb, const void* K, long k_st, long k_sb,
                             const void* V, long v_st, long v_sb, const void* O, long o_st, long o_sb,
                             const void* dO, long do_st, long do_sb, const float* LSE, float* Delta,
                             void* dQ, long dq_st, long dq_sb, void* dK, long dk_st, long dk_sb,
                             void* dV, long dv_st, long dv_sb,
                             const int* klen, int causal, int dist_penalty, float scale, float p_drop, unsigned long long seed,
-                            void* stream) {
+                            const void* keep, void* stream) {
     AttnArgs a{};
+    a.keep = static_cast<uint32_t*>(const_cast<void*>(keep));
     a.dist_pen = dist_penalty;
     a.Q = Q; a.K = K; a.V = V; a.O = const_cast<void*>(O); a.LSE = const_cast<float*>(LSE);
     a.dO = dO; a.dQ = dQ; a.dK = dK; a.dV = dV; a.Delta = Delta;
@@ -1548,11 +1649,34 @@
     if (!Q || !K || !V || !O || !dO || !LSE || !Delta || !dQ || !dK || !dV) return S2T_EINVAL;
     const long s[] = {q_st, q_sb, k_st, k_sb, v_st, v_sb, do_st, do_sb};
     if (!strides_ok(dtype, s, 8)) return S2T_EINVAL;
+    if (a.keep && !keep_route(dtype, head_dim, a)) return S2T_ENOTSUP;
     hipStream_t st = (hipStream_t)stream;
     const bool sq = dtype == S2T_BF16 && head_dim == 64 && sq_bwd_route(a);
     ProfScope prof("attn_bwd", st, (sq ? 10.0 : 14.0) * B * H * (double)Tq * Tk * head_dim * (causal ? 0.5 : 1.0), 0.0);
     if (dtype == S2T_BF16) return head_dim == 64 ? bwd_launch<bf16, 64>(a, st) : bwd_launch<bf16, 32>(a, st);
     return head_dim == 64 ? bwd_launch<float, 64>(a, st) : bwd_launch<float, 32>(a, st);
+}
+extern "C" int s2t_attn_bwd(int dtype, int head_dim, int B, int H, int Tq, int Tk,
+                            const void* Q, long q_st, long q_sb, const void* K, long k_st, long k_sb,
+                            const void* V, long v_st, long v_sb, const void* O, long o_st, long o_sb,
+                            const void* dO, long do_st, long do_sb, const float* LSE, float* Delta,
+                            void* dQ, long dq_st, long dq_sb, void* dK, long dk_st, long dk_sb,
+                            void* dV, long dv_st, long dv_sb,
+                            const int* klen, int causal, int dist_penalty, float scale, float p_drop, unsigned long long seed,
+                            void* stream) {
+    return attn_bwd_impl(dtype, head_dim, B, H, Tq, Tk, Q, q_st, q_sb, K, k_st, k_sb, V, v_st, v_sb, O, o_st, o_sb, dO, do_st, do_sb, LSE, Delta,
+                         dQ, dq_st, dq_sb, dK, dk_st, dk_sb, dV, dv_st, dv_sb, klen, causal, dist_penalty, scale, p_drop, seed, nullptr, stream);
+}
+extern "C" int s2t_attn_bwd_keep(int dtype, int head_dim, int B, int H, int Tq, int Tk,
+                                 const void* Q, long q_st, long q_sb, const void* K, long k_st, long k_sb,
+                                 const void* V, long v_st, long v_sb, const void* O, long o_st, long o_sb,
+                                 const void* dO, long do_st, long do_sb, const float* LSE, float* Delta,
+                                 void* dQ, long dq_st, long dq_sb, void* dK, long dk_st, long dk_sb,
+                                 void* dV, long dv_st, long dv_sb,
+                                 const int* klen, int causal, int dist_penalty, float scale, float p_drop, unsigned long long seed,
+                                 const void* keep, void* stream) {
+    return attn_bwd_impl(dtype, head_dim, B, H, Tq, Tk, Q, q_st, q_sb, K, k_st, k_sb, V, v_st, v_sb, O, o_st, o_sb, dO, do_st, do_sb, LSE, Delta,
+                         dQ, dq_st, dq_sb, dK, dk_st, dk_sb, dV, dv_st, dv_sb, klen, causal, dist_penalty, scale, p_drop, seed, keep, stream);
 }
 
 template <typename T>
diff --git a/fbk_fairseq_st_amd/csrc/layer.hip b/fbk_fairseq_st_amd/csrc/layer.hip
--- a/fbk_fairseq_st_amd/csrc/layer.hip
+++ b/fbk_fairseq_st_amd/csrc/layer.hip
@@ -9,6 +9,7 @@
     size_t h1, st1, qkv, ctx, lse, y1;
     size_t h2, st2, q, kv, ctx2, lse2, y2;
     size_t h3, st3, a, pre, amask;
+    size_t keep, nkeep;
     size_t total, nmask;
 };
 Ws layout(const S2TLayerDesc& L, int training) {
@@ -26,6 +27,8 @@
     if (L.gelu) w.pre = take(M * (size_t)L.ffn * e);
     w.nmask = (training && !L.gelu) ? s2t_gemm_relu_mask_bytes((int)M, L.ffn, L.D) : 0;
     if (w.nmask) w.amask = take(w.nmask);
+    w.nkeep = (training && L.p_attn > 0.f) ? s2t_attn_keep_bytes(L.D / L.heads, L.B, L.heads, L.T, L.T, L.causal, L.dist_penalty, L.p_attn) : 0;
+    if (w.nkeep) w.keep = take(w.nkeep);
     w.total = o;
     return w;
 }
@@ -86,8 +89,13 @@
     TRY(linear(L, M, 3 * D, D, ws + w.h1, L.w_qkv, L.b_qkv, ws + w.qkv, nullptr, nullptr, nullptr, 0, S2T_ACT_NONE, 0.f, 0, st));
     const char* qkv = ws + w.qkv;
     const long ts3 = (long)L.B * 3 * D, bs3 = 3 * D, ts1 = (long)L.B * D, bs1 = D;
-    TRY(s2t_attn_fwd(L.dtype, d, L.B, H, L.T, L.T, qkv, ts3, bs3, qkv + (size_t)D * 2, ts3, bs3, qkv + (size_t)2 * D * 2, ts3, bs3, ws + w.ctx, ts1, bs1,
-                     reinterpret_cast<float*>(ws + w.lse), c->self_klen, L.causal, L.dist_penalty, scale, pa, c->seed_sa_attn, st));
+    if (w.nkeep) {
+        TRY(s2t_attn_fwd_keep(L.dtype, d, L.B, H, L.T, L.T, qkv, ts3, bs3, qkv + (size_t)D * 2, ts3, bs3, qkv + (size_t)2 * D * 2, ts3, bs3, ws + w.ctx, ts1, bs1,
+                              reinterpret_cast<float*>(ws + w.lse), c->self_klen, L.causal, L.dist_penalty, scale, pa, c->seed_sa_attn, ws + w.keep, st));
+    } else {
+        TRY(s2t_attn_fwd(L.dtype, d, L.B, H, L.T, L.T, qkv, ts3, bs3, qkv + (size_t)D * 2, ts3, bs3, qkv + (size_t)2 * D * 2, ts3, bs3, ws + w.ctx, ts1, bs1,
+                         reinterpret_cast<float*>(ws + w.lse), c->self_klen, L.causal, L.dist_penalty, scale, pa, c->seed_sa_attn, st));
+    }
     TRY(linear(L, M, D, D, ws + w.ctx, L.w_o, L.b_o, ws + w.y1, c->x, nullptr, nullptr, 0, S2T_ACT_NONE, p, c->seed_sa_out, st));
     const char* xin = ws + w.y1;
     if (L.decoder) {
@@ -176,10 +184,17 @@
     TRY(linear_dx(L, M, D, D, dcur_d, L.w_o, tm + t.dctx, nullptr, 0, S2T_ACT_NONE, 1.f, 0, st));
     const char* qkv = ws + w.qkv;
     char* dqkv = tm + t.dqkv;
-    TRY(s2t_attn_bwd(L.dtype, d, L.B, H, L.T, L.T, qkv, ts3, bs3, qkv + (size_t)D * 2, ts3, bs3, qkv + (size_t)2 * D * 2, ts3, bs3, ws + w.ctx, ts1, bs1,
-                     tm + t.dctx, ts1, bs1, reinterpret_cast<const float*>(ws + w.lse), reinterpret_cast<float*>(tm + t.delta),
-                     dqkv, ts3, bs3, dqkv + (size_t)D * 2, ts3, bs3, dqkv + (size_t)2 * D * 2, ts3, bs3, c->self_klen, L.causal, L.dist_penalty, scale, pa,
-                     c->seed_sa_attn, st));
+    if (w.nkeep) {
+        TRY(s2t_attn_bwd_keep(L.dtype, d, L.B, H, L.T, L.T, qkv, ts3, bs3, qkv + (size_t)D * 2, ts3, bs3, qkv + (size_t)2 * D * 2, ts3, bs3, ws + w.ctx, ts1, bs1,
+                              tm + t.dctx, ts1, bs1, reinterpret_cast<const float*>(ws + w.lse), reinterpret_cast<float*>(tm + t.delta),
+                              dqkv, ts3, bs3, dqkv + (size_t)D * 2, ts3, bs3, dqkv + (size_t)2 * D * 2, ts3, bs3, c->self_klen, L.causal, L.dist_penalty, scale, pa,
+                              c->seed_sa_attn, ws + w.keep, st));
+    } else {
+        TRY(s2t_attn_bwd(L.dtype, d, L.B, H, L.T, L.T, qkv, ts3, bs3, qkv + (size_t)D * 2, ts3, bs3, qkv + (size_t)2 * D * 2, ts3, bs3, ws + w.ctx, ts1, bs1,
+                         tm + t.dctx, ts1, bs1, reinterpret_cast<const float*>(ws + w.lse), reinterpret_cast<float*>(tm + t.delta),
+                         dqkv, ts3, bs3, dqkv + (size_t)D * 2, ts3, bs3, dqkv + (size_t)2 * D * 2, ts3, bs3, c->self_klen, L.causal, L.dist_penalty, scale, pa,
+                         c->seed_sa_attn, st));
+    }
     TRY(queue_dw(*c, dqkv, ws + w.h1, L.g_w_qkv, L.g_b_qkv, 3 * D, D, M));
     TRY(linear_dx(L, M, 3 * D, D, dqkv, L.w_qkv, tm + t.dh1, nullptr, 0, S2T_ACT_NONE, 1.f, 0, st));
     const float* st1 = reinterpret_cast<const float*>(ws + w.st1);
diff --git a/fbk_fairseq_st_amd/kernels.py b/fbk_fairseq_st_amd/kernels.py
--- a/fbk_fairseq_st_amd/kernels.py
+++ b/fbk_fairseq_st_amd/kernels.py
@@ -161,6 +161,47 @@
     return out, lse
 
 
+def attn_keep_bytes(d, B, heads, Tq, Tk, causal=False, dist_penalty=False, p_drop=0.0):
+    return int(_lib().s2t_attn_keep_bytes(d, B, heads, Tq, Tk, int(causal), int(bool(dist_penalty)), float(p_drop)))
+
+
+def attn_fwd_keep(q, k, v, heads, keep, klen=None, causal=False, scale=None, p_drop=0.0, seed=0, out=None, dist_penalty=False):
+    Tq, B, D = q.shape
+    Tk = k.shape[0]
+    d = D // heads
+    if scale is None:
+        scale = d ** -0.5
+    if out is None:
+        out = torch.empty((Tq, B, D), dtype=q.dtype, device=q.device)
+    lse = torch.empty((B, heads, Tq), dtype=torch.float32, device=q.device)
+    if keep is not None:
+        L.require_cuda(keep)
+        assert keep.is_contiguous() and keep.numel() * keep.element_size() >= attn_keep_bytes(d, B, heads, Tq, Tk, causal, dist_penalty, p_drop)
+    rc = _lib().s2t_attn_fwd_keep(L.dt(q), d, B, heads, Tq, Tk, L.ptr(q), *_tb(q), L.ptr(k), *_tb(k), L.ptr(v), *_tb(v),
+                                  L.ptr(out), *_tb(out), L.ptr(lse), L.ptr(klen), int(causal), int(bool(dist_penalty)), float(scale),
+                                  float(p_drop), int(seed), L.ptr(keep), L.stream())
+    L.check(rc, "s2t_attn_fwd_keep")
+    return out, lse
+
+
+def attn_bwd_keep(q, k, v, o, do, lse, heads, dq, dk, dv, keep, klen=None, causal=False, scale=None, p_drop=0.0, seed=0, dist_penalty=False):
+    Tq, B, D = q.shape
+    Tk = k.shape[0]
+    d = D // heads
+    if scale is None:
+        scale = d ** -0.5
+    delta = torch.empty((B, heads, Tq), dtype=torch.float32, device=q.device)
+    if keep is not None:
+        L.require_cuda(keep)
+        assert keep.is_contiguous() and keep.numel() * keep.element_size() >= attn_keep_bytes(d, B, heads, Tq, Tk, causal, dist_penalty, p_drop)
+    rc = _lib().s2t_attn_bwd_keep(L.dt(q), d, B, heads, Tq, Tk, L.ptr(q), *_tb(q), L.ptr(k), *_tb(k), L.ptr(v), *_tb(v),
+                                  L.ptr(o), *_tb(o), L.ptr(do), *_tb(do), L.ptr(lse), L.ptr(delta),
+                                  L.ptr(dq), *_tb(dq), L.ptr(dk), *_tb(dk), L.ptr(dv), *_tb(dv),
+                                  L.ptr(klen), int(causal), int(bool(dist_penalty)), float(scale), float(p_drop), int(seed), L.ptr(keep), L.stream())
+    L.check(rc, "s2t_attn_bwd_keep")
+    return dq, dk, dv
+
+
 def attn_probs_avg(q, k, heads, klen=None, scale=None, heads_used=None):
     Tq, B, D = q.shape
     Tk = k.shape[0]
diff --git a/fbk_fairseq_st_amd/lib.py b/fbk_fairseq_st_amd/lib.py
--- a/fbk_fairseq_st_amd/lib.py
+++ b/fbk_fairseq_st_amd/lib.py
@@ -31,6 +31,10 @@
     "s2t_attn_fwd": [c_int] * 6 + [P, c_long, c_long] * 4 + [P, P, c_int, c_int, c_float, c_float, c_ull, P],
     "s2t_attn_bwd": [c_int] * 6 + [P, c_long, c_long] * 5 + [P, P] + [P, c_long, c_long] * 3 +
                     [P, c_int, c_int, c_float, c_float, c_ull, P],
+    "s2t_attn_keep_bytes": [c_int] * 7 + [c_float],
+    "s2t_attn_fwd_keep": [c_int] * 6 + [P, c_long, c_long] * 4 + [P, P, c_int, c_int, c_float, c_float, c_ull, P, P],
+    "s2t_attn_bwd_keep": [c_int] * 6 + [P, c_long, c_long] * 5 + [P, P] + [P, c_long, c_long] * 3 +
+                         [P, c_int, c_int, c_float, c_float, c_ull, P, P],
     "s2t_attn_probs_avg": [c_int] * 6 + [P, c_long, c_long] * 2 + [P, c_int, c_float, P, P],
     "s2t_layernorm_fwd": [c_int, P, P, P, P, P, P, c_int, c_int, c_float, P],
     "s2t_layernorm_bwd": [c_int, P, P, P, P, P, P, P, P, P, c_int, c_int, P, c_float, c_ull, P],
@@ -187,7 +191,7 @@
 
 FAST_PATH = os.path.join(_HERE, "_s2t_fastcall.so")
 _HOST_SIDE = ("s2t_host_batch_by_size", "s2t_host_ctc_uer")
-_SIZE_T_RESULT = ("s2t_gemm_relu_mask_bytes", "s2t_layer_ws_bytes", "s2t_layer_bwd_tmp_bytes", "s2t_decode_lds_bytes",
+_SIZE_T_RESULT = ("s2t_gemm_relu_mask_bytes", "s2t_attn_keep_bytes", "s2t_layer_ws_bytes", "s2t_layer_bwd_tmp_bytes", "s2t_decode_lds_bytes",
                   "s2t_ctc_loss_any_workspace")
 
 
diff --git a/include/s2t_hip.h b/include/s2t_hip.h
--- a/include/s2t_hip.h
+++ b/include/s2t_hip.h
@@ -66,6 +66,19 @@
                  const void* dO, long do_st, long do_sb, const float* LSE, float* Delta,
                  void* dQ, long dq_st, long dq_sb, void* dK, long dk_st, long dk_sb, void* dV, long dv_st, long dv_sb,
                  const int* klen, int causal, int dist_penalty, float scale, float p_drop, unsigned long long seed, void* stream);
+size_t s2t_attn_keep_bytes(int head_dim, int B, int H, int Tq, int Tk, int causal, int dist_penalty, float p_drop);
+int s2t_attn_fwd_keep(int dtype, int head_dim, int B, int H, int Tq, int Tk,
+                      const void* Q, long q_st, long q_sb, const void* K, long k_st, long k_sb,
+                      const void* V, long v_st, long v_sb, void* O, long o_st, long o_sb, float* LSE,
+                      const int* klen, int causal, int dist_penalty, float scale, float p_drop, unsigned long long seed,
+                      void* keep, void* stream);
+int s2t_attn_bwd_keep(int dtype, int head_dim, int B, int H, int Tq, int Tk,
+                      const void* Q, long q_st, long q_sb, const void* K, long k_st, long k_sb,
+                      const void* V, long v_st, long v_sb, const void* O, long o_st, long o_sb,
+                      const void* dO, long do_st, long do_sb, const float* LSE, float* Delta,
+                      void* dQ, long dq_st, long dq_sb, void* dK, long dk_st, long dk_sb, void* dV, long dv_st, long dv_sb,
+                      const int* klen, int causal, int dist_penalty, float scale, float p_drop, unsigned long long seed,
+                      const void* keep, void* stream);
 
 int s2t_layernorm_fwd(int dtype, const void* x, const float* gamma, const float* beta, void* y,
                       float* mean, float* rstd, int M, int D, float eps, void* stream);
```

Measured after the change: 6.720 million, median of 6. 1.01x the previous value.
